# Kolkir/feature-point-cnn

Measured on AMD Instinct MI355X. Metric: frames/sec (VGA 640x480) SuperPoint fwd+NMS+descriptors, higher is better.
Workload: dtype f32

## Files before the change

### feature-point-cnn_amd/csrc/block_mfma.h

```cpp
#pragma once
#include "conv_mfma.h"

namespace fpc {

#ifdef FPC_DIAG
#define FPC_STAMP(i)                                                                     \
  if (a.stamps && threadIdx.x == 0) {                                                    \
    unsigned long long t_;                                                               \
    asm volatile("s_memtime %0\n\ts_waitcnt lgkmcnt(0)" : "=s"(t_)::"memory");            \
    a.stamps[(size_t)blockIdx.x * 8 + (i)] = t_;                                         \
  }
#define FPC_RSTAMP(i)                                                                    \
  if (a.stamps && threadIdx.x == 0) {                                                    \
    unsigned long long t_;                                                               \
    asm volatile("s_memrealtime %0\n\ts_waitcnt lgkmcnt(0)" : "=s"(t_)::"memory");        \
    a.stamps[(size_t)blockIdx.x * 8 + (i)] = t_;                                         \
  }
#else
#define FPC_STAMP(i)
#define FPC_RSTAMP(i)
#endif

struct BlockArgs {
  const float* x;
  int csx, nchunk;
  int H, W;
  const float4* w1;
  const float* b1;
  int tapoff4[9];
  const float4* w2;
  const float* b2;
  int k8_h, k8_x;
  float* out;
  int cso, Ho, Wo, tiles_x, tiles_y, nstore, frame0;
  unsigned x_bytes;
#ifdef FPC_DIAG
  unsigned long long* stamps;
#endif
};

template <int TH, int TW, int S, int KC, int WM, int WN, int MB, int NB, int CMIDP>
struct BlockCfg {
  using C1 = ConvCfg<TH, TW, S, 3, KC, WM, WN, MB, NB>;
  static constexpr int ROWH4 = CMIDP / 4 + 1;
  static constexpr int H_BYTES = C1::M * ROWH4 * 16;
  static constexpr int LDS_BYTES = C1::LDS_BYTES > H_BYTES ? C1::LDS_BYTES : H_BYTES;
  static_assert(CMIDP % 8 == 0 && CMIDP <= C1::N, "mid channels must fit the workgroup's N");
};

template <int TH, int TW, int S, int KC, int WM, int WN, int MB, int NB, int CMIDP>
__global__ __launch_bounds__(WM* WN * 64, 2) void block_mfma_kernel(const BlockArgs a) {
  using C = ConvCfg<TH, TW, S, 3, KC, WM, WN, MB, NB>;
  using BC = BlockCfg<TH, TW, S, KC, WM, WN, MB, NB, CMIDP>;
  constexpr int NT = C::NT, HW = C::HW, HH = C::HH, ROW4 = C::ROW4, K8 = KC / 8, KC4 = KC / 4;
  constexpr int NV = HH * HW * KC4, ITER = (NV + NT - 1) / NT, ROWH4 = BC::ROWH4, NBT = WN * NB;
  extern __shared__ float4 lds4[];

  const int tid = threadIdx.x, lane = tid & 63, wave = tid >> 6;
  const int wm = wave / WN, wn = wave % WN;
  const int half = lane >> 5, l31 = lane & 31;
  const int tiles = a.tiles_x * a.tiles_y;
  const int bidx = fpc_xcd_tile_index();
  const int bl = bidx / tiles;
  const int b = a.frame0 + bl;
  const int t = bidx - bl * tiles;
  const int ty = t / a.tiles_x, tx = t - ty * a.tiles_x;

  FPC_STAMP(0)
#ifdef FPC_DIAG
  if (a.stamps && threadIdx.x == 0) {
    a.stamps[(size_t)blockIdx.x * 8 + 6] = __builtin_amdgcn_s_getreg(63492);
    a.stamps[(size_t)blockIdx.x * 8 + 7] = __builtin_amdgcn_s_getreg((31 << 11) | 20);
  }
#endif
  int abase[MB];
#pragma unroll
  for (int mb = 0; mb < MB; ++mb) {
    int m = (wm * MB + mb) * 32 + l31;
    m = m < TH * TW ? m : TH * TW - 1;
    const int py = m / TW, px = m - py * TW;
    abase[mb] = ((py * S) * HW + px * S) * ROW4 + half;
  }
  constexpr int stepstride = NBT * 64;
  const __amdgpu_buffer_rsrc_t wrsrc = __builtin_amdgcn_make_buffer_rsrc(
      const_cast<float4*>(a.w1), 0, (int)((unsigned)(a.nchunk * 9 * K8 + 2) * (unsigned)(stepstride * 16)), 0x00020000);
  const int wlane = ((wn * NB) * 64 + lane) * 16;
  int wstep = 0;
  auto wfrag = [&](int nb) {
    typedef float f32x4w __attribute__((ext_vector_type(4)));
    const f32x4w r = __builtin_bit_cast(f32x4w, __builtin_amdgcn_raw_buffer_load_b128(wrsrc, wlane + nb * 1024, wstep, 0));
    return make_float4(r.x, r.y, r.z, r.w);
  };

  const int iy0 = ty * TH * S - 1, ix0 = tx * TW * S - 1;
  typedef float f32x4v __attribute__((ext_vector_type(4)));
  f32x4v stage[ITER];
  const __amdgpu_buffer_rsrc_t xrsrc = __builtin_amdgcn_make_buffer_rsrc(const_cast<float*>(a.x), 0, (int)a.x_bytes, 0x00020000);
  const unsigned xbase = (unsigned)((b * a.H + iy0) * a.W + ix0) * (unsigned)(a.csx * 4);
  auto load_chunk = [&](int chunk) {
    const int wlim = chunk < a.nchunk ? a.W : 0;
#pragma unroll
    for (int i = 0; i < ITER; ++i) {
      const int e = tid + i * NT;
      const int pix = e / KC4, c4 = e - pix * KC4;
      const int hy = pix / HW, hx = pix - hy * HW;
      const int iy = iy0 + hy, ix = ix0 + hx;
      const bool ok = ((unsigned)iy < (unsigned)a.H) & ((unsigned)ix < (unsigned)wlim) & (hy < HH);
      unsigned off = xbase + (unsigned)(((hy * a.W + hx) * a.csx + chunk * KC + c4 * 4) * 4);
      asm volatile("" : "+v"(off));
      stage[i] = __builtin_bit_cast(f32x4v, __builtin_amdgcn_raw_buffer_load_b128(xrsrc, (int)(ok ? off : 0xfffffff0u), 0, 0));
    }
  };
  auto store_chunk = [&]() {
#pragma unroll
    for (int i = 0; i < ITER; ++i) {
      const int e = tid + i * NT;
      int pix = e / KC4, c4 = e - pix * KC4;
      if (NV % NT != 0) {
        const bool in = e < NV;
        pix = in ? pix : HH * HW - 1;
        c4 = in ? c4 : KC4;
      }
      *reinterpret_cast<f32x4v*>(&lds4[pix * ROW4 + c4]) = stage[i];
    }
  };

  f32x16 acc[MB][NB];
#pragma unroll
  for (int mb = 0; mb < MB; ++mb)
#pragma unroll
    for (int nb = 0; nb < NB; ++nb)
#pragma unroll
      for (int r = 0; r < 16; ++r) acc[mb][nb][r] = 0.f;

  load_chunk(0);
  float4 b0[NB], b1[NB];
#pragma unroll
  for (int nb = 0; nb < NB; ++nb) b0[nb] = wfrag(nb);
  wstep += stepstride * 16;
#pragma unroll
  for (int nb = 0; nb < NB; ++nb) b1[nb] = wfrag(nb);
  wstep += stepstride * 16;
  for (int chunk = 0; chunk < a.nchunk; ++chunk) {
    FPC_LDS_BARRIER();
    store_chunk();
    FPC_LDS_BARRIER();
    load_chunk(chunk + 1);
    if (chunk == 0) { FPC_STAMP(1) }
    float4 av[MB];
#pragma unroll
    for (int mb = 0; mb < MB; ++mb) av[mb] = lds4[abase[mb] + a.tapoff4[0]];
#pragma unroll
    for (int tap = 0; tap < 9; ++tap) {
      const int toff = a.tapoff4[tap];
      const int toffn = a.tapoff4[tap < 8 ? tap + 1 : 8];
#pragma unroll
      for (int k8 = 0; k8 < K8; ++k8) {
        float4 b2[NB], an[MB];
#pragma unroll
        for (int nb = 0; nb < NB; ++nb) b2[nb] = wfrag(nb);
        wstep += stepstride * 16;
#pragma unroll
        for (int mb = 0; mb < MB; ++mb)
          an[mb] = lds4[abase[mb] + (k8 + 1 < K8 ? toff + (k8 + 1) * 2 : toffn)];
        __builtin_amdgcn_sched_barrier(0);
#pragma unroll
        for (int j = 0; j < 4; ++j)
#pragma unroll
          for (int mb = 0; mb < MB; ++mb)
#pragma unroll
            for (int nb = 0; nb < NB; ++nb) {
              const float af = j == 0 ? av[mb].x : j == 1 ? av[mb].y : j == 2 ? av[mb].z : av[mb].w;
              const float bf = j == 0 ? b0[nb].x : j == 1 ? b0[nb].y : j == 2 ? b0[nb].z : b0[nb].w;
              acc[mb][nb] = __builtin_amdgcn_mfma_f32_32x32x2f32(af, bf, acc[mb][nb], 0, 0, 0);
            }
#pragma unroll
        for (int nb = 0; nb < NB; ++nb) {
          b0[nb] = b1[nb];
          b1[nb] = b2[nb];
        }
#pragma unroll
        for (int mb = 0; mb < MB; ++mb) av[mb] = an[mb];
      }
    }
  }

  FPC_STAMP(2)
  constexpr int KH = CMIDP / 8, RING = 4;
  const int nsteps2 = KH + a.k8_x;
  const float4* wq = a.w2 + (size_t)(wn * NB) * 64 + lane;
  float4 cb[RING][NB];
  auto load_b = [&](int slot, int step) {
    const float4* pw = wq + (size_t)min(step, nsteps2 + 1) * stepstride;
#pragma unroll
    for (int nb = 0; nb < NB; ++nb) cb[slot][nb] = pw[nb * 64];
  };
#pragma unroll
  for (int s_ = 0; s_ < RING - 1; ++s_) load_b(s_, s_);
  FPC_LDS_BARRIER();
  {
    float* hl = reinterpret_cast<float*>(lds4);
#pragma unroll
    for (int nb = 0; nb < NB; ++nb) {
      const int n = (wn * NB + nb) * 32 + l31;
      const float bias = a.b1[n];
#pragma unroll
      for (int mb = 0; mb < MB; ++mb)
#pragma unroll
        for (int r = 0; r < 16; ++r) {
          const int m = (wm * MB + mb) * 32 + (r & 3) + 8 * (r >> 2) + 4 * half;
          const float v = acc[mb][nb][r] + bias;
          if (n < CMIDP) hl[m * (ROWH4 * 4) + n] = v > 0.f ? v : 0.f;
          acc[mb][nb][r] = 0.f;
        }
    }
  }
  FPC_LDS_BARRIER();

  FPC_STAMP(3)
  int hbase[MB];
#pragma unroll
  for (int mb = 0; mb < MB; ++mb) hbase[mb] = ((wm * MB + mb) * 32 + l31) * ROWH4 + half;
  auto mfma_step = [&](const float4 (&av)[MB], int slot) {
#pragma unroll
    for (int j = 0; j < 4; ++j)
#pragma unroll
      for (int mb = 0; mb < MB; ++mb)
#pragma unroll
        for (int nb = 0; nb < NB; ++nb) {
          const float af = j == 0 ? av[mb].x : j == 1 ? av[mb].y : j == 2 ? av[mb].z : av[mb].w;
          const float bf = j == 0 ? cb[slot][nb].x : j == 1 ? cb[slot][nb].y : j == 2 ? cb[slot][nb].z : cb[slot][nb].w;
          acc[mb][nb] = __builtin_amdgcn_mfma_f32_32x32x2f32(af, bf, acc[mb][nb], 0, 0, 0);
        }
  };
  const float* xrow[MB];
#pragma unroll
  for (int mb = 0; mb < MB; ++mb) {
    int m = (wm * MB + mb) * 32 + l31;
    m = m < TH * TW ? m : TH * TW - 1;
    const int py = m / TW, px = m - py * TW;
    int y = (ty * TH + py) * S, x = (tx * TW + px) * S;
    y = y < a.H ? y : a.H - 1;
    x = x < a.W ? x : a.W - 1;
    xrow[mb] = a.x + ((size_t)(b * a.H + y) * a.W + x) * a.csx + half * 4;
  }
  typedef float f4v __attribute__((ext_vector_type(4)));
  auto ldx = [&](int mb, int k8) {
    const f4v v = *reinterpret_cast<const f4v*>(xrow[mb] + (k8 < a.k8_x ? k8 : 0) * 8);
    return make_float4(v.x, v.y, v.z, v.w);
  };
  float4 xa[4][MB];
  if (a.k8_x > 0) {
#pragma unroll
    for (int u = 0; u < 4; ++u)
#pragma unroll
      for (int mb = 0; mb < MB; ++mb) xa[u][mb] = ldx(mb, u);
  }
  {
    float4 av[MB];
#pragma unroll
    for (int mb = 0; mb < MB; ++mb) av[mb] = lds4[hbase[mb]];
#pragma unroll
    for (int k8 = 0; k8 < KH; ++k8) {
      float4 an[MB];
      load_b((k8 + RING - 1) % RING, k8 + RING - 1);
#pragma unroll
      for (int mb = 0; mb < MB; ++mb) an[mb] = lds4[hbase[mb] + (k8 + 1 < KH ? k8 + 1 : k8) * 2];
      __builtin_amdgcn_sched_barrier(0);
      mfma_step(av, k8 % RING);
#pragma unroll
      for (int mb = 0; mb < MB; ++mb) av[mb] = an[mb];
    }
  }

  for (int k8 = 0; k8 < a.k8_x; k8 += 8) {
    float4 xb[4][MB];
#pragma unroll
    for (int u = 0; u < 4; ++u) {
      load_b((KH + u + RING - 1) % RING, KH + k8 + u + RING - 1);
#pragma unroll
      for (int mb = 0; mb < MB; ++mb) xb[u][mb] = ldx(mb, k8 + 4 + u);
      __builtin_amdgcn_sched_barrier(0);
      mfma_step(xa[u], (KH + u) % RING);
    }
#pragma unroll
    for (int u = 0; u < 4; ++u) {
      load_b((KH + u + RING - 1) % RING, KH + k8 + 4 + u + RING - 1);
#pragma unroll
      for (int mb = 0; mb < MB; ++mb) xa[u][mb] = ldx(mb, k8 + 8 + u);
      __builtin_amdgcn_sched_barrier(0);
      mfma_step(xb[u], (KH + u) % RING);
    }
  }

  FPC_STAMP(4)
  FPC_LDS_BARRIER();
  {
    float* ol = reinterpret_cast<float*>(lds4);
#pragma unroll
    for (int nb = 0; nb < NB; ++nb) {
      const int n = (wn * NB + nb) * 32 + l31;
      const float bias = a.b2[n];
#pragma unroll
      for (int mb = 0; mb < MB; ++mb)
#pragma unroll
        for (int r = 0; r < 16; ++r) {
          const int m = (wm * MB + mb) * 32 + (r & 3) + 8 * (r >> 2) + 4 * half;
          if (n < CMIDP) ol[m * (ROWH4 * 4) + n] = acc[mb][nb][r] + bias;
        }
    }
  }
  FPC_LDS_BARRIER();
  {
    constexpr int C4 = CMIDP / 4;
    constexpr int NE = TH * TW * C4, EIT = (NE + NT - 1) / NT;
    const int oyb = ty * TH, oxb = tx * TW;
    const bool ident = a.k8_x == 0;
    float4 idv[EIT];
    if (ident) {
#pragma unroll
      for (int i = 0; i < EIT; ++i) {
        const int e = tid + i * NT;
        const int m = e / C4, c4 = e - m * C4;
        const int py = m / TW, px = m - py * TW;
        const int y = oyb + py, x = oxb + px;
        const bool ok = (NE % NT == 0 || e < NE) && y < a.Ho && x < a.Wo;
        idv[i] = *reinterpret_cast<const float4*>(a.x + (ok ? ((size_t)(b * a.Ho + y) * a.Wo + x) * a.csx + c4 * 4 : 0));
      }
    }
#pragma unroll
    for (int i = 0; i < EIT; ++i) {
      const int e = tid + i * NT;
      const int m = e / C4, c4 = e - m * C4;
      const int py = m / TW, px = m - py * TW;
      const int y = oyb + py, x = oxb + px;
      if ((NE % NT == 0 || e < NE) && y < a.Ho && x < a.Wo) {
        float4 v = lds4[m * ROWH4 + c4];
        if (ident) {
          v.x += idv[i].x;
          v.y += idv[i].y;
          v.z += idv[i].z;
          v.w += idv[i].w;
        }
        v.x = v.x > 0.f ? v.x : 0.f;
        v.y = v.y > 0.f ? v.y : 0.f;
        v.z = v.z > 0.f ? v.z : 0.f;
        v.w = v.w > 0.f ? v.w : 0.f;
        *reinterpret_cast<float4*>(a.out + ((size_t)(b * a.Ho + y) * a.Wo + x) * a.cso + c4 * 4) = v;
      }
    }
  }
  FPC_STAMP(5)
}


}
```

### feature-point-cnn_amd/csrc/conv_mfma.h

```cpp
#pragma once
#include <hip/hip_runtime.h>
#include <stdint.h>

namespace fpc {

__device__ __forceinline__ int fpc_xcd_tile_index() {
  const unsigned g = gridDim.x, b = blockIdx.x;
  return (g & 7u) == 0u ? (int)((b & 7u) * (g >> 3) + (b >> 3)) : (int)b;
}

typedef float f32x16 __attribute__((ext_vector_type(16)));

#define FPC_LDS_BARRIER() asm volatile("s_waitcnt lgkmcnt(0)\n\ts_barrier" ::: "memory")

struct ConvSub {
  const float4* wfrag;
  int ntaps;
  int tapoff4[9];
  int oy0, ox0;
};

struct ConvArgs {
  const float* in0;
  int cs0;
  int nchunk0;
  const float* in1;
  int cs1, nchunk1, s1, H1, W1;
  int H, W;
  int pad;
  const float* bias;
  const float* res;
  int csr;
  float* out;
  int cso;
  int OH, OW, oys, oxs;
  int Ho, Wo;
  int tiles_x, tiles_y;
  int nstore;
  int relu;
  int nbt;
  int frame0;
  ConvSub sub[4];
};

template <int TH, int TW, int S, int EXT, int KC, int WM, int WN, int MB, int NB>
struct ConvCfg {
  static constexpr int NT = WM * WN * 64;
  static constexpr int HW = (TW - 1) * S + EXT;
  static constexpr int HH = (TH - 1) * S + EXT;
  static constexpr int ROW4 = KC / 4 + 1;
  static constexpr int LDS_BYTES = HH * HW * ROW4 * 16;
  static constexpr int M = WM * MB * 32;
  static constexpr int N = WN * NB * 32;
  static_assert(TH * TW <= M && TH * TW > M - 32, "tile must fill the M blocks");
  static_assert(KC % 8 == 0, "KC must be a multiple of 8");
};

template <int TH, int TW, int S, int EXT, int KC, int WM, int WN, int MB, int NB>
__global__ __launch_bounds__(WM* WN * 64, 2) void conv_mfma_kernel(const ConvArgs a) {
  using C = ConvCfg<TH, TW, S, EXT, KC, WM, WN, MB, NB>;
  constexpr int NT = C::NT, HW = C::HW, HH = C::HH, ROW4 = C::ROW4, K8 = KC / 8, KC4 = KC / 4;
  constexpr int NV = HH * HW * KC4;
  constexpr int ITER = (NV + NT - 1) / NT;
  extern __shared__ float4 lds4[];

  const int tid = threadIdx.x;
  const int lane = tid & 63, wave = tid >> 6;
  const int wm = wave / WN, wn = wave % WN;
  const int half = lane >> 5, l31 = lane & 31;

  const int tiles = a.tiles_x * a.tiles_y;
  const int bidx = fpc_xcd_tile_index();
  const int bl = bidx / tiles;
  const int b = a.frame0 + bl;
  const int t = bidx - bl * tiles;
  const int ty = t / a.tiles_x, tx = t - ty * a.tiles_x;
  const int subi = gridDim.z - 1 - blockIdx.z;
  const ConvSub& sp = a.sub[subi];

  int abase[MB];
#pragma unroll
  for (int mb = 0; mb < MB; ++mb) {
    int m = (wm * MB + mb) * 32 + l31;
    m = m < TH * TW ? m : TH * TW - 1;
    const int py = m / TW, px = m - py * TW;
    abase[mb] = ((py * S) * HW + px * S) * ROW4 + half;
  }
  const int stepstride = a.nbt * 64;
  const __amdgpu_buffer_rsrc_t wrsrc = __builtin_amdgcn_make_buffer_rsrc(
      const_cast<float4*>(sp.wfrag), 0, (int)((unsigned)((a.nchunk0 * sp.ntaps + a.nchunk1) * K8 + 2) * (unsigned)(stepstride * 16)), 0x00020000);
  const int wlane = (((blockIdx.y * WN + wn) * NB) * 64 + lane) * 16;
  int wstep = 0;
  const float4* wp = sp.wfrag + (size_t)((blockIdx.y * WN + wn) * NB) * 64 + lane;
  auto wfrag = [&](int nb) {
    if constexpr (EXT == 1) {
      return wp[(wstep >> 4) + nb * 64];
    } else {
      typedef float f32x4w __attribute__((ext_vector_type(4)));
      const f32x4w r = __builtin_bit_cast(f32x4w, __builtin_amdgcn_raw_buffer_load_b128(wrsrc, wlane + nb * 1024, wstep, 0));
      return make_float4(r.x, r.y, r.z, r.w);
    }
  };

  const int iy0 = ty * TH * S - a.pad, ix0 = tx * TW * S - a.pad;
  float4 stage[ITER];
  auto load_chunk = [&](int chunk) {
    const bool second = chunk >= a.nchunk0;
    const float* src = second ? a.in1 : a.in0;
    const int cs = second ? a.cs1 : a.cs0;
    const int c0 = (second ? chunk - a.nchunk0 : chunk) * KC;
    const int sH = second ? a.H1 : a.H, sW = second ? a.W1 : a.W;
#pragma unroll
    for (int i = 0; i < ITER; ++i) {
      const int e = tid + i * NT;
      const int pix = e / KC4, c4 = e - pix * KC4;
      const int hy = pix / HW, hx = pix - hy * HW;
      int iy, ix;
      if (second) {
        iy = (ty * TH + hy) * a.s1;
        ix = (tx * TW + hx) * a.s1;
      } else {
        iy = iy0 + hy;
        ix = ix0 + hx;
      }
      const bool ok = (NV % NT == 0 || e < NV) && iy >= 0 && iy < sH && ix >= 0 && ix < sW;
      const size_t off = ok ? ((size_t)(b * sH + iy) * sW + ix) * cs + c0 + c4 * 4 : 0;
      float4 v = *reinterpret_cast<const float4*>(src + off);
      if (!ok) v = make_float4(0.f, 0.f, 0.f, 0.f);
      stage[i] = v;
    }
  };
  auto store_chunk = [&]() {
#pragma unroll
    for (int i = 0; i < ITER; ++i) {
      const int e = tid + i * NT;
      const int pix = e / KC4, c4 = e - pix * KC4;
      if (NV % NT == 0 || e < NV) lds4[pix * ROW4 + c4] = stage[i];
    }
  };

  f32x16 acc[MB][NB];
#pragma unroll
  for (int mb = 0; mb < MB; ++mb)
#pragma unroll
    for (int nb = 0; nb < NB; ++nb)
#pragma unroll
      for (int r = 0; r < 16; ++r) acc[mb][nb][r] = 0.f;

  const int nchunks = a.nchunk0 + a.nchunk1;
  const int ntaps = sp.ntaps;
  load_chunk(0);
  float4 b0[NB], b1[NB];
#pragma unroll
  for (int nb = 0; nb < NB; ++nb) b0[nb] = wfrag(nb);
  wstep += stepstride * 16;
#pragma unroll
  for (int nb = 0; nb < NB; ++nb) b1[nb] = wfrag(nb);
  wstep += stepstride * 16;

  for (int chunk = 0; chunk < nchunks; ++chunk) {
    if (chunk) __syncthreads();
    store_chunk();
    __syncthreads();
    if (chunk + 1 < nchunks) load_chunk(chunk + 1);
    for (int tap = 0; tap < ntaps; ++tap) {
      const int toff = sp.tapoff4[tap];
#pragma unroll
      for (int k8 = 0; k8 < K8; ++k8) {
        float4 b2[NB];
#pragma unroll
        for (int nb = 0; nb < NB; ++nb) b2[nb] = wfrag(nb);
        wstep += stepstride * 16;
        __builtin_amdgcn_sched_barrier(0);
        float4 av[MB];
#pragma unroll
        for (int mb = 0; mb < MB; ++mb) av[mb] = lds4[abase[mb] + toff + k8 * 2];
#pragma unroll
        for (int j = 0; j < 4; ++j)
#pragma unroll
          for (int mb = 0; mb < MB; ++mb)
#pragma unroll
            for (int nb = 0; nb < NB; ++nb) {
              const float af = j == 0 ? av[mb].x : j == 1 ? av[mb].y : j == 2 ? av[mb].z : av[mb].w;
              const float bf = j == 0 ? b0[nb].x : j == 1 ? b0[nb].y : j == 2 ? b0[nb].z : b0[nb].w;
              acc[mb][nb] = __builtin_amdgcn_mfma_f32_32x32x2f32(af, bf, acc[mb][nb], 0, 0, 0);
            }
#pragma unroll
        for (int nb = 0; nb < NB; ++nb) {
          b0[nb] = b1[nb];
          b1[nb] = b2[nb];
        }
      }
    }
  }

  const int oyb = ty * TH, oxb = tx * TW;
#pragma unroll
  for (int nb = 0; nb < NB; ++nb) {
    const int n = ((blockIdx.y * WN + wn) * NB + nb) * 32 + l31;
    const float bias = a.bias[n];
    const bool nok = n < a.nstore;
#pragma unroll
    for (int mb = 0; mb < MB; ++mb) {
#pragma unroll
      for (int r = 0; r < 16; ++r) {
        const int m = (wm * MB + mb) * 32 + (r & 3) + 8 * (r >> 2) + 4 * half;
        const int py = m / TW, px = m - py * TW;
        const int y = oyb + py, x = oxb + px;
        if (nok && m < TH * TW && y < a.Ho && x < a.Wo) {
          const size_t opix = (size_t)(b * a.OH + y * a.oys + sp.oy0) * a.OW + x * a.oxs + sp.ox0;
          float v = acc[mb][nb][r] + bias;
          if (a.res) v += a.res[opix * a.csr + n];
          if (a.relu) v = v > 0.f ? v : 0.f;
          a.out[opix * a.cso + n] = v;
        }
      }
    }
  }
}

#define CONV2_MARKER 0x7fffff00

template <int TH, int TW, int S, int EXT, int KC, int WM, int WN, int MB, int NB>
struct Conv2Cfg {
  using C = ConvCfg<TH, TW, S, EXT, KC, WM, WN, MB, NB>;
  static constexpr int ROWO4 = C::N / 4 + 1;
  static constexpr int OUT_BYTES = C::M * ROWO4 * 16;
  static constexpr int LDS_BYTES = C::LDS_BYTES > OUT_BYTES ? C::LDS_BYTES : OUT_BYTES;
};

template <int TH, int TW, int S, int EXT, int KC, int WM, int WN, int MB, int NB>
__global__ __launch_bounds__(WM* WN * 64, 2) void conv2_mfma_kernel(const ConvArgs a) {
  using C = ConvCfg<TH, TW, S, EXT, KC, WM, WN, MB, NB>;
  using C2 = Conv2Cfg<TH, TW, S, EXT, KC, WM, WN, MB, NB>;
  constexpr int NT = C::NT, HW = C::HW, HH = C::HH, ROW4 = C::ROW4, K8 = KC / 8, KC4 = KC / 4, N = C::N;
  constexpr int NV = HH * HW * KC4, ITER = (NV + NT - 1) / NT, ROWO4 = C2::ROWO4;
  extern __shared__ float4 lds4[];
  typedef float f32x4w __attribute__((ext_vector_type(4)));

  const int tid = threadIdx.x, lane = tid & 63, wave = tid >> 6;
  const int wm = wave / WN, wn = wave % WN;
  const int half = lane >> 5, l31 = lane & 31;
  const int tiles = a.tiles_x * a.tiles_y;
  const int bidx = fpc_xcd_tile_index();
  const int bl = bidx / tiles;
  const int b = a.frame0 + bl;
  const int t = bidx - bl * tiles;
  const int ty = t / a.tiles_x, tx = t - ty * a.tiles_x;
  const int subi = gridDim.z - 1 - blockIdx.z;
  const ConvSub& sp = a.sub[subi];

  int abase[MB];
#pragma unroll
  for (int mb = 0; mb < MB; ++mb) {
    int m = (wm * MB + mb) * 32 + l31;
    m = m < TH * TW ? m : TH * TW - 1;
    const int py = m / TW, px = m - py * TW;
    abase[mb] = ((py * S) * HW + px * S) * ROW4 + half;
  }
  const int stepstride = a.nbt * 64;
  const __amdgpu_buffer_rsrc_t wrsrc = __builtin_amdgcn_make_buffer_rsrc(
      const_cast<float4*>(sp.wfrag), 0, (int)((unsigned)(a.nchunk0 * sp.ntaps * K8 + 2) * (unsigned)(stepstride * 16)), 0x00020000);
  const int wlane = (((blockIdx.y * WN + wn) * NB) * 64 + lane) * 16;
  int wstep = 0;
  auto wfrag = [&](int nb) {
    const f32x4w r = __builtin_bit_cast(f32x4w, __builtin_amdgcn_raw_buffer_load_b128(wrsrc, wlane + nb * 1024, wstep, 0));
    return make_float4(r.x, r.y, r.z, r.w);
  };

  const int iy0 = ty * TH * S - a.pad, ix0 = tx * TW * S - a.pad;
  const __amdgpu_buffer_rsrc_t xrsrc = __builtin_amdgcn_make_buffer_rsrc(
      const_cast<float*>(a.in0) + (size_t)b * a.H * a.W * a.cs0, 0, a.H * a.W * a.cs0 * 4, 0x00020000);
  int eoff[ITER], eslot[ITER];
#pragma unroll
  for (int i = 0; i < ITER; ++i) {
    const int e = tid + i * NT;
    int pix = e / KC4, c4 = e - pix * KC4;
    const int hy = pix / HW, hx = pix - hy * HW;
    const int iy = iy0 + hy, ix = ix0 + hx;
    const bool ok = (NV % NT == 0 || e < NV) & ((unsigned)iy < (unsigned)a.H) & ((unsigned)ix < (unsigned)a.W);
    eoff[i] = ok ? ((iy * a.W + ix) * a.cs0 + c4 * 4) * 4 : CONV2_MARKER;
    if (NV % NT != 0) {
      const bool in = e < NV;
      pix = in ? pix : HH * HW - 1;
      c4 = in ? c4 : KC4;
    }
    eslot[i] = pix * ROW4 + c4;
  }
  f32x4w stage[ITER];
  auto load_chunk = [&](int chunk) {
    const int cbase = chunk < a.nchunk0 ? chunk * (KC * 4) : CONV2_MARKER;
#pragma unroll
    for (int i = 0; i < ITER; ++i) {
      int voff;
      asm("v_add_i32 %0, %1, %2 clamp" : "=v"(voff) : "v"(eoff[i]), "s"(cbase));
      stage[i] = __builtin_bit_cast(f32x4w, __builtin_amdgcn_raw_buffer_load_b128(xrsrc, voff, 0, 0));
    }
  };
  auto store_chunk = [&]() {
#pragma unroll
    for (int i = 0; i < ITER; ++i) *reinterpret_cast<f32x4w*>(&lds4[eslot[i]]) = stage[i];
  };

  f32x16 acc[MB][NB];
#pragma unroll
  for (int mb = 0; mb < MB; ++mb)
#pragma unroll
    for (int nb = 0; nb < NB; ++nb)
#pragma unroll
      for (int r = 0; r < 16; ++r) acc[mb][nb][r] = 0.f;

  const int nchunks = a.nchunk0, ntaps = sp.ntaps;
  load_chunk(0);
  float4 b0[NB], b1[NB];
#pragma unroll
  for (int nb = 0; nb < NB; ++nb) b0[nb] = wfrag(nb);
  wstep += stepstride * 16;
#pragma unroll
  for (int nb = 0; nb < NB; ++nb) b1[nb] = wfrag(nb);
  wstep += stepstride * 16;

  for (int chunk = 0; chunk < nchunks; ++chunk) {
    FPC_LDS_BARRIER();
    store_chunk();
    FPC_LDS_BARRIER();
    load_chunk(chunk + 1);
    float4 av[MB];
#pragma unroll
    for (int mb = 0; mb < MB; ++mb) av[mb] = lds4[abase[mb] + sp.tapoff4[0]];
    for (int tap = 0; tap < ntaps; ++tap) {
      const int toff = sp.tapoff4[tap];
      const int toffn = sp.tapoff4[tap + 1 < ntaps ? tap + 1 : tap];
#pragma unroll
      for (int k8 = 0; k8 < K8; ++k8) {
        float4 b2[NB], an[MB];
#pragma unroll
        for (int nb = 0; nb < NB; ++nb) b2[nb] = wfrag(nb);
        wstep += stepstride * 16;
#pragma unroll
        for (int mb = 0; mb < MB; ++mb) an[mb] = lds4[abase[mb] + (k8 + 1 < K8 ? toff + (k8 + 1) * 2 : toffn)];
        __builtin_amdgcn_sched_barrier(0);
#pragma unroll
        for (int j = 0; j < 4; ++j)
#pragma unroll
          for (int mb = 0; mb < MB; ++mb)
#pragma unroll
            for (int nb = 0; nb < NB; ++nb) {
              const float af = j == 0 ? av[mb].x : j == 1 ? av[mb].y : j == 2 ? av[mb].z : av[mb].w;
              const float bf = j == 0 ? b0[nb].x : j == 1 ? b0[nb].y : j == 2 ? b0[nb].z : b0[nb].w;
              acc[mb][nb] = __builtin_amdgcn_mfma_f32_32x32x2f32(af, bf, acc[mb][nb], 0, 0, 0);
            }
#pragma unroll
        for (int nb = 0; nb < NB; ++nb) {
          b0[nb] = b1[nb];
          b1[nb] = b2[nb];
        }
#pragma unroll
        for (int mb = 0; mb < MB; ++mb) av[mb] = an[mb];
      }
    }
  }

  constexpr int C4 = N / 4, NE = TH * TW * C4, EIT = (NE + NT - 1) / NT;
  const int oyb = ty * TH, oxb = tx * TW;
  const int nbase = blockIdx.y * N;
  const __amdgpu_buffer_rsrc_t orsrc = __builtin_amdgcn_make_buffer_rsrc(a.out + (size_t)b * a.OH * a.OW * a.cso, 0, a.OH * a.OW * a.cso * 4, 0x00020000);
  const __amdgpu_buffer_rsrc_t rrsrc = __builtin_amdgcn_make_buffer_rsrc(
      const_cast<float*>(a.res ? a.res : a.out) + (size_t)b * a.OH * a.OW * (a.res ? a.csr : a.cso), 0, a.res ? a.OH * a.OW * a.csr * 4 : 0, 0x00020000);
  int ooff[EIT], olds[EIT];
  f32x4w idv[EIT];
#pragma unroll
  for (int i = 0; i < EIT; ++i) {
    const int e = tid + i * NT;
    const int m = e / C4, c4 = e - m * C4;
    const int py = m / TW, px = m - py * TW;
    const int y = oyb + py, x = oxb + px;
    const bool ok = (NE % NT == 0 || e < NE) & (y < a.Ho) & (x < a.Wo);
    const int opix = (y * a.oys + sp.oy0) * a.OW + x * a.oxs + sp.ox0;
    ooff[i] = ok ? (opix * a.cso + nbase + c4 * 4) * 4 : CONV2_MARKER;
    olds[i] = (NE % NT == 0 || e < NE) ? m * ROWO4 + c4 : 0;
    idv[i] = __builtin_bit_cast(f32x4w, __builtin_amdgcn_raw_buffer_load_b128(rrsrc, ok ? (opix * a.csr + nbase + c4 * 4) * 4 : CONV2_MARKER, 0, 0));
  }
  FPC_LDS_BARRIER();
  {
    float* ol = reinterpret_cast<float*>(lds4);
#pragma unroll
    for (int nb = 0; nb < NB; ++nb) {
      const int nl = (wn * NB + nb) * 32 + l31;
      const float bias = a.bias[nbase + nl];
#pragma unroll
      for (int mb = 0; mb < MB; ++mb)
#pragma unroll
        for (int r = 0; r < 16; ++r) {
          const int m = (wm * MB + mb) * 32 + (r & 3) + 8 * (r >> 2) + 4 * half;
          ol[m * (ROWO4 * 4) + nl] = acc[mb][nb][r] + bias;
        }
    }
  }
  FPC_LDS_BARRIER();
  const float floor_ = a.relu ? 0.f : -3.0e38f;
#pragma unroll
  for (int i = 0; i < EIT; ++i) {
    f32x4w v = *reinterpret_cast<const f32x4w*>(&lds4[olds[i]]);
    v += idv[i];
    v.x = fmaxf(v.x, floor_);
    v.y = fmaxf(v.y, floor_);
    v.z = fmaxf(v.z, floor_);
    v.w = fmaxf(v.w, floor_);
    __builtin_amdgcn_raw_buffer_store_b128(__builtin_bit_cast(__attribute__((ext_vector_type(4))) unsigned, v), orsrc, ooff[i], 0, 0);
  }
}

}
```

### feature-point-cnn_amd/csrc/fpc_api.hip

```cpp
#include <hip/hip_runtime.h>

#include <dlfcn.h>

#include <algorithm>
#include <cmath>
#include <cstdio>
#include <cstdlib>
#include <cstring>
#include <memory>
#include <mutex>
#include <chrono>
#include <string>
#include <vector>

#include "../../include/fpc.h"
#include "block_mfma.h"
#include "block_bf16.h"
#include "convt_bf16.h"
#include "block_x3.h"
#include "stem_bf16.h"
#include "wblock_mfma.h"
#include "wblock16_mfma.h"
#include "wblock36_mfma.h"
#include "wblock36p_mfma.h"
#include "conv_mfma.h"
#include "kernels_misc.h"
#include "queue_map.h"
#include "match.h"
#include "match_frames.h"
#include "match_bank.h"
#include "match_bank_bf16.h"
#include "match_guided.h"
#include "match_guided_cells.h"
#include "match_guided_epipolar.h"
#include "match_guided_pose.h"
#include "ransac_homography.h"
#include "ransac_fundamental.h"
#include "pose_epipolar.h"
#include "pose_homography.h"
#include "match_bank_topk.h"
#include "pnp_ransac.h"
#include "sim3_ransac.h"
#include "landmarks.h"
#include "homography.h"
#include "weights.h"
#include "plan_options.h"

namespace fpc {

constexpr int BLOB_HEADER_FLOATS = 16;
constexpr uint32_t BLOB_MAGIC = 0x57435046u;

static thread_local std::string g_hip_err;

#define HIPCHECK(expr)                                                                   \
  do {                                                                                   \
    hipError_t e_ = (expr);                                                              \
    if (e_ != hipSuccess) {                                                              \
      g_hip_err = std::string(#expr) + ": " + hipGetErrorString(e_);                     \
      return FPC_E_HIP;                                                                  \
    }                                                                                    \
  } while (0)

template <auto Kernel, int Threads, int Lds, typename Args>
static void launch_as(const Args& a, dim3 grid, hipStream_t st) {
  hipLaunchKernelGGL(Kernel, grid, dim3(Threads), Lds, st, a);
}

template <typename Args>
struct Instance {
  const void* fn;
  int lds_bytes, threads;
  void (*launch)(const Args&, dim3, hipStream_t);
};
template <auto Kernel, typename Cfg, int Threads, typename Args>
static Instance<Args> instance_of() {
  return {(const void*)Kernel, Cfg::LDS_BYTES, Threads, launch_as<Kernel, Threads, Cfg::LDS_BYTES, Args>};
}

#define FPC_KINDS(X)                                                        \
  X(T816_3x3_K64_N64, 8, 16, 1, 3, 64, 4, 1, 1, 2)                          \
  X(T816_1x1_K64_N64, 8, 16, 1, 1, 64, 4, 1, 1, 2)                          \
  X(T620_3x3s2_K32_N128, 6, 20, 2, 3, 32, 2, 2, 2, 2)                       \
  X(T620_3x3_K64_N128, 6, 20, 1, 3, 64, 2, 2, 2, 2)                         \
  X(T620_1x1_K64_N128, 6, 20, 1, 1, 64, 2, 2, 2, 2)                         \
  X(T620_2x2_K64_N128, 6, 20, 1, 2, 64, 2, 2, 2, 2)                         \
  X(T320_2x2_K64_N128, 3, 20, 1, 2, 64, 1, 4, 2, 1)                         \
  X(T320_1x1_K64_N128, 3, 20, 1, 1, 64, 1, 4, 2, 1)                         \
  X(T620_3x3_K64_N96, 6, 20, 1, 3, 64, 4, 1, 1, 3)                          \
  X(T620_1x1_K64_N96, 6, 20, 1, 1, 64, 4, 1, 1, 3)                          \
  X(T620_3x3_K72_N96, 6, 20, 1, 3, 72, 4, 1, 1, 3)                          \
  X(T620_1x1_K72_N96, 6, 20, 1, 1, 72, 4, 1, 1, 3)

enum Kind {
#define X(name, ...) K_##name,
  FPC_KINDS(X)
#undef X
      K_COUNT
};

struct KindInfo : Instance<ConvArgs> {
  const char* name;
  const char* symbol;
  int TH, TW, S, EXT, KC, WM, WN, MB, NB;
};

static const KindInfo g_kinds[K_COUNT] = {
#define X(name, TH, TW, S, EXT, KC, WM, WN, MB, NB)                                                                                      \
  {instance_of<conv_mfma_kernel<TH, TW, S, EXT, KC, WM, WN, MB, NB>, ConvCfg<TH, TW, S, EXT, KC, WM, WN, MB, NB>, WM * WN * 64, ConvArgs>(), \
   #name, "conv_mfma_kernel<" #TH ", " #TW ", " #S ", " #EXT ", " #KC ", " #WM ", " #WN ", " #MB ", " #NB ">", TH, TW, S, EXT, KC, WM, WN, MB, NB},
    FPC_KINDS(X)
#undef X
};

#define FPC_LEAN_KINDS(X)                          \
  X(T320_2x2_K64_N128, 3, 20, 1, 2, 64, 1, 4, 2, 1) \
  X(T320_1x1_K64_N128, 3, 20, 1, 1, 64, 1, 4, 2, 1)
struct LeanKindInfo : Instance<ConvArgs> {
  Kind kind;
  const char* symbol;
};
static const LeanKindInfo g_lean_kinds[] = {
#define X(name, TH, TW, S, EXT, KC, WM, WN, MB, NB)                                                                                        \
  {instance_of<conv2_mfma_kernel<TH, TW, S, EXT, KC, WM, WN, MB, NB>, Conv2Cfg<TH, TW, S, EXT, KC, WM, WN, MB, NB>, WM * WN * 64, ConvArgs>(), \
   K_##name, "conv2_mfma_kernel<" #TH ", " #TW ", " #S ", " #EXT ", " #KC ", " #WM ", " #WN ", " #MB ", " #NB ">"},
    FPC_LEAN_KINDS(X)
#undef X
};
static const LeanKindInfo* lean_kind(Kind k) {
  for (const LeanKindInfo& l : g_lean_kinds)
    if (l.kind == k) return &l;
  return nullptr;
}

#define FPC_BLOCK_KINDS(X)                                   \
  X(B816_s1_K64_C64, 8, 16, 1, 64, 4, 1, 1, 2, 64)           \
  X(B1616_s1_K32_C64, 16, 16, 1, 32, 4, 1, 2, 2, 64)         \
  X(B620_s2_K32_C128, 6, 20, 2, 32, 2, 2, 2, 2, 128)         \
  X(B620_s1_K64_C128, 6, 20, 1, 64, 2, 2, 2, 2, 128)         \
  X(B620_s1_K64_C72, 6, 20, 1, 64, 4, 1, 1, 3, 72)           \
  X(B620_s1_K72_C72, 6, 20, 1, 72, 4, 1, 1, 3, 72)           \
  X(B320_s2_K32_C256, 3, 20, 2, 32, 1, 4, 2, 2, 256)         \
  X(B310_s2_K32_C256, 3, 10, 2, 32, 1, 4, 1, 2, 256)         \
  X(B320_s2_K32_C128, 3, 20, 2, 32, 1, 4, 2, 1, 128)         \
  X(B320_s1_K64_C256, 3, 20, 1, 64, 1, 4, 2, 2, 256)         \
  X(B416_s2_K32_C128, 4, 16, 2, 32, 1, 4, 2, 1, 128)

enum BKind {
#define X(name, ...) BK_##name,
  FPC_BLOCK_KINDS(X)
#undef X
      BK_COUNT
};

struct BKindInfo : Instance<BlockArgs> {
  const char* name;
  const char* symbol;
  int TH, TW, S, KC, WM, WN, MB, NB, CMIDP;
};

static const BKindInfo g_bkinds[BK_COUNT] = {
#define X(name, TH, TW, S, KC, WM, WN, MB, NB, CMIDP)                                                                                            \
  {instance_of<block_mfma_kernel<TH, TW, S, KC, WM, WN, MB, NB, CMIDP>, BlockCfg<TH, TW, S, KC, WM, WN, MB, NB, CMIDP>, WM * WN * 64, BlockArgs>(), \
   #name, "block_mfma_kernel<" #TH ", " #TW ", " #S ", " #KC ", " #WM ", " #WN ", " #MB ", " #NB ", " #CMIDP ">", TH, TW, S, KC, WM, WN, MB, NB, CMIDP},
    FPC_BLOCK_KINDS(X)
#undef X
};

#define FPC_WBLOCK_KINDS(X)     \
  X(W816_K32_C64, 32, 2, 64)    \
  X(W816_K32_C128, 32, 4, 128)  \
  X(W816_K32_C72, 32, 3, 72)    \
  X(W816_K24_C72, 24, 3, 72)
#define FPC_W16_KINDS(X) \
  X(W16_C64, 4, 8)       \
  X(W16_C128, 8, 8)      \
  X(W16_C128H, 8, 4)
#define FPC_W36_KINDS(X) \
  X(W36_C64_4x4, 1, 4, 4)  \
  X(W36_C64_2x8, 1, 2, 8)  \
  X(W36_C128_4x4, 2, 4, 4) \
  X(W36_C128_2x8, 2, 2, 8)

#define FPC_W36P_KINDS(X) \
  X(W36P_C64_4x4, 4, 4)   \
  X(W36P_C64_2x8, 2, 8)

#define FPC_W36PD_KINDS(X) \
  X(W36PD_C65_4x4, 4, 4)   \
  X(W36PD_C65_2x8, 2, 8)

#define FPC_W36D_KINDS(X) \
  X(W36_C65_4x4, 4, 4)    \
  X(W36_C65_2x8, 2, 8)

#define FPC_W36S_KINDS(X) \
  X(W36S_C128_4x4, 2, 4, 4)
#define FPC_W36PC_KINDS(X) \
  X(W36PC_C64_8x2, 8, 2)

enum WKind {
#define X(name, ...) WK_##name,
  FPC_WBLOCK_KINDS(X)
  FPC_W16_KINDS(X)
  FPC_W36_KINDS(X)
  FPC_W36D_KINDS(X)
  FPC_W36P_KINDS(X)
  FPC_W36PD_KINDS(X)
  FPC_W36S_KINDS(X)
  FPC_W36PC_KINDS(X)
#undef X
      WK_COUNT
};

struct WKindInfo : Instance<WBlockArgs> {
  const char* name;
  const char* symbol;
  int gen;
  int KC, NBT, CMID;
  int NCG;
  int TH;
  int TW;
  bool dust = false;
};

static const WKindInfo g_wkinds[WK_COUNT] = {
#define X(name, KC, NBT, CMID)                                                                            \
  {instance_of<wblock_mfma_kernel<KC, NBT, CMID>, WBlockCfg<KC, NBT, CMID>, 512, WBlockArgs>(), #name,                         \
   "wblock_mfma_kernel<" #KC ", " #NBT ", " #CMID ">", 1, KC, NBT, CMID, 0, 8, 16},
    FPC_WBLOCK_KINDS(X)
#undef X
#define X(name, NCG, TH)                                                                                  \
  {instance_of<wblock16_kernel<NCG, TH>, W16Cfg<NCG, TH>, 512, WBlockArgs>(), #name,                                           \
   "wblock16_kernel<" #NCG ", " #TH ">", 2, 16, NCG / 2, NCG * 16, NCG, TH, 16},
    FPC_W16_KINDS(X)
#undef X
#define X(name, NB, TYT, TXT)                                                                             \
  {instance_of<wblock36_kernel<NB, TYT, TXT>, W36Cfg<NB, TYT, TXT>, 256, WBlockArgs>(), #name,                                 \
   "wblock36_kernel<" #NB ", " #TYT ", " #TXT ">", 3, 16, 2 * NB, 64 * NB, 4 * NB, 4 * TYT, 4 * TXT},
    FPC_W36_KINDS(X)
#undef X
#define X(name, TYT, TXT)                                                                                 \
  {instance_of<wblock36_dust_kernel<TYT, TXT>, W36Cfg<1, TYT, TXT, true>, 256, WBlockArgs>(), #name,                           \
   "wblock36_dust_kernel<" #TYT ", " #TXT ">", 3, 16, 2, 64, 4, 4 * TYT, 4 * TXT, true},
    FPC_W36D_KINDS(X)
#undef X
#define X(name, TYT, TXT)                                                                                 \
  {instance_of<wblock36p_kernel<TYT, TXT>, W36PCfg<TYT, TXT>, 512, WBlockArgs>(), #name,                                       \
   "wblock36p_kernel<" #TYT ", " #TXT ", 3>", 3, 16, 2, 64, 4, 4 * TYT, 4 * TXT},
    FPC_W36P_KINDS(X)
#undef X
#define X(name, TYT, TXT)                                                                                 \
  {instance_of<wblock36p_dust_kernel<TYT, TXT>, W36PCfg<TYT, TXT, true>, 512, WBlockArgs>(), #name,                            \
   "wblock36p_dust_kernel<" #TYT ", " #TXT ", 3>", 3, 16, 2, 64, 4, 4 * TYT, 4 * TXT, true},
    FPC_W36PD_KINDS(X)
#undef X
#define X(name, NB, TYT, TXT)                                                                             \
  {instance_of<wblock36s_kernel<NB, TYT, TXT>, W36Cfg<NB, TYT, TXT>, 256, WBlockArgs>(), #name,                                \
   "wblock36s_kernel<" #NB ", " #TYT ", " #TXT ">", 3, 16, 2 * NB, 64 * NB, 4 * NB, 4 * TYT, 4 * TXT},
    FPC_W36S_KINDS(X)
#undef X
#define X(name, TYT, TXT)                                                                                 \
  {instance_of<wconv36p_kernel<TYT, TXT>, W36PCfg<TYT, TXT, false, true>, 512, WBlockArgs>(), #name,                           \
   "wconv36p_kernel<" #TYT ", " #TXT ", 3>", 3, 16, 2, 64, 4, 4 * TYT, 4 * TXT},
    FPC_W36PC_KINDS(X)
#undef X
};

static size_t conv_floats(size_t steps, int nbt) { return (steps + 2) * nbt * 64 * 4; }
static size_t conv_bf16_floats(size_t steps, int nbt, int planes) { return (steps + 2) * planes * nbt * 64 * 4; }
static size_t bias_floats(int nbt) { return (size_t)nbt * 32; }
static size_t w1_floats(const WKindInfo& k, int nchunk) {
  if (k.gen == 3) return (size_t)k.NCG * ((size_t)nchunk * 36 + (k.NCG == 8 ? W36Cfg<2, 4, 4>::WPAD : W36Cfg<1, 4, 4>::WPAD)) * 256;
  if (k.gen == 2) return (size_t)k.NCG * ((size_t)nchunk * 16 + W16Cfg<8>::WPAD) * 256;
  return conv_floats(((size_t)nchunk + 1) * 16 * (k.KC / 8), k.NBT);
}
static size_t w2_floats(const WKindInfo& k, int k8) {
  if (k.gen >= 2) return (size_t)k.NCG * ((size_t)k8 / 2 + W16Cfg<8>::WPAD) * 256;
  return conv_floats(k8, k.NBT);
}
static double wkind_mfma_flops(const WKindInfo& k, int tiles, int nchunk, int k8_1x1) {
  const double px = (double)k.TH * k.TW, n = k.NBT * 32.0;
  if (k.gen == 3) return 2.0 * tiles * n * (36.0 * (px / 16) * nchunk * k.KC + px * k8_1x1 * 8.0);
  return 2.0 * tiles * n * (16.0 * (px / 4) * nchunk * k.KC + px * k8_1x1 * 8.0);
}
static bool w36_fits(int , int H, int W, int cs_in, int cs_out) {
  return (unsigned long long)H * W * (unsigned long long)std::max(cs_in, cs_out) * sizeof(float) < (unsigned long long)W36_MARKER;
}
static int w36_frames_per_launch(int H, int W, int cs_in, int cs_out) {
  const unsigned long long fb = (unsigned long long)H * W * (unsigned long long)std::max(cs_in, cs_out) * sizeof(float);
  return (int)std::max<unsigned long long>(1, ((unsigned long long)W36_MARKER - 1) / fb);
}
static const unsigned long long W16_REACH = 0xfffffff0ull;
static int w16_frames_in_reach(int H, int W, int cs) {
  return (int)std::min<unsigned long long>(1u << 30, W16_REACH / ((unsigned long long)H * W * cs * sizeof(float)));
}
static int w36_conv_part(int cout, int tiles, int cus) {
  if (cout < 128) return 64;
  if (cout == 128) return 128;
  const double t2 = std::ceil((double)tiles * (cout / 128) / cus) * 1.0, t1 = std::ceil((double)tiles * (cout / 64) / cus) * 0.53;
  return t1 < t2 ? 64 : 128;
}
static WKind w36_kind(int cout, int H, int W, bool paired = false, bool conv82 = false) {
  const int t44 = ((H + 15) / 16) * ((W + 15) / 16), t28 = ((H + 7) / 8) * ((W + 31) / 32), t82 = ((H + 31) / 32) * ((W + 7) / 8);
  if (conv82 && cout == 64 && paired && t82 < std::min(t44, t28)) return WK_W36PC_C64_8x2;
  if (cout == 65 && paired) return t28 < t44 ? WK_W36PD_C65_2x8 : WK_W36PD_C65_4x4;
  if (cout == 65) return t28 < t44 ? WK_W36_C65_2x8 : WK_W36_C65_4x4;
  if (cout == 64 && paired) return t28 < t44 ? WK_W36P_C64_2x8 : WK_W36P_C64_4x4;
  if (cout == 64) return t28 < t44 ? WK_W36_C64_2x8 : WK_W36_C64_4x4;
  return t28 < t44 ? WK_W36_C128_2x8 : WK_W36_C128_4x4;
}

static WKind w36_stacked_kind(WKind wk) { return wk == WK_W36_C128_4x4 || wk == WK_W36_C128_2x8 ? WK_W36S_C128_4x4 : WK_COUNT; }
static int w36_stacked_rows(int Hf, int W, int frames, WKind sk, int tiles_now) {
  if (sk == WK_COUNT) return 0;
  const int th = g_wkinds[sk].TH, tw = g_wkinds[sk].TW;
  if (Hf % 4 != 0 || Hf < th) return 0;
  const int rows = (frames * Hf + th - 1) / th;
  return rows * ((W + tw - 1) / tw) < frames * tiles_now ? rows : 0;
}

#define FPC_BF16_KINDS(X)                                                                   \
  X(F816_s1_K64_C64, block_bf16_one_kernel, BlockBfCfg, 1, 8, 32, 1, 3, 64, 2, 2, 4, 1, 64) \
  X(F816_s1_K64_C128, block_bf16_kernel, BlockBfCfg, 1, 8, 16, 1, 3, 64, 1, 4, 4, 1, 128)   \
  X(F816_s1_K80_C80, block_bf16_one_kernel, BlockBfCfg, 1, 8, 16, 1, 3, 80, 4, 1, 1, 3, 80) \
  X(F816_s1_K128_C128, block_bf16_one_kernel, BlockBfCfg, 1, 8, 16, 1, 3, 128, 1, 4, 4, 1, 128) \
  X(F816_s1_K128_C80w, block_bf16_one_kernel, BlockBfCfg, 1, 8, 16, 1, 3, 128, 1, 4, 4, 1, 80) \
  X(F620_s2_K64_C128, block_bf16_one_kernel, BlockBfCfg, 1, 6, 20, 2, 3, 64, 2, 2, 2, 2, 128) \
  X(F320_s2_K128_C256, block_bf16_one_kernel, BlockBfCfg, 1, 3, 20, 2, 3, 128, 1, 4, 2, 2, 256) \
  X(F416_s1_K128_C256, block_bf16_two_kernel, BlockBfCfg, 1, 4, 16, 1, 3, 128, 1, 4, 2, 2, 256) \
  X(F816_ct_K64_C128, block_bf16_kernel, BlockBfCfg, 1, 8, 16, 1, 2, 64, 1, 4, 4, 1, 128)   \
  X(F816_ctf_K64_C128, convt_bf16_kernel, ConvTBfCfg, 1, 8, 16, 1, 2, 64, 2, 2, 2, 1, 128)  \
  X(S816_s1_K64_C64, block_x3_kernel, BlockX3Cfg, 3, 8, 16, 1, 3, 64, 2, 2, 2, 1, 64)       \
  X(S620_s2_K16_C128, block_x3_kernel, BlockX3Cfg, 3, 6, 20, 2, 3, 16, 2, 2, 2, 2, 128)     \
  X(S620_s1_K64_C128, block_x3_kernel, BlockX3Cfg, 3, 6, 20, 1, 3, 64, 2, 2, 2, 2, 128)     \
  X(S620_s1_K64_C80, block_x3_kernel, BlockX3Cfg, 3, 6, 20, 1, 3, 64, 4, 1, 1, 3, 80)       \
  X(S620_s1_K16_C80, block_x3_kernel, BlockX3Cfg, 3, 6, 20, 1, 3, 16, 4, 1, 1, 3, 80)       \
  X(S320_s2_K16_C256, block_x3_kernel, BlockX3Cfg, 3, 3, 20, 2, 3, 16, 1, 4, 2, 2, 256)     \
  X(S320_s1_K64_C256, block_x3_kernel, BlockX3Cfg, 3, 3, 20, 1, 3, 64, 1, 4, 2, 2, 256)     \
  X(S620_ct_K64_C128, block_x3_kernel, BlockX3Cfg, 3, 6, 20, 1, 2, 64, 2, 2, 2, 2, 128)     \
  X(S620_1x1_K64_C80, block_x3_kernel, BlockX3Cfg, 3, 6, 20, 1, 1, 64, 4, 1, 1, 3, 80)      \
  X(S320_1x1_K64_C256, block_x3_kernel, BlockX3Cfg, 3, 3, 20, 1, 1, 64, 1, 4, 2, 2, 256)     \
  X(H816_s1_K64_C64, block_h2_kernel, BlockH2Cfg, 2, 8, 16, 1, 3, 64, 2, 2, 2, 1, 64)     \
  X(H620_s2_K16_C128, block_h2_kernel, BlockH2Cfg, 2, 6, 20, 2, 3, 16, 2, 2, 2, 2, 128)     \
  X(H620_s1_K64_C128, block_h2_kernel, BlockH2Cfg, 2, 6, 20, 1, 3, 64, 2, 2, 2, 2, 128)     \
  X(H620_s1_K64_C80, block_h2_kernel, BlockH2Cfg, 2, 6, 20, 1, 3, 64, 4, 1, 1, 3, 80)     \
  X(H620_s1_K16_C80, block_h2_kernel, BlockH2Cfg, 2, 6, 20, 1, 3, 16, 4, 1, 1, 3, 80)     \
  X(H320_s2_K16_C256, block_h2_kernel, BlockH2Cfg, 2, 3, 20, 2, 3, 16, 1, 4, 2, 2, 256)     \
  X(H320_s1_K64_C256, block_h2_kernel, BlockH2Cfg, 2, 3, 20, 1, 3, 64, 1, 4, 2, 2, 256)     \
  X(H620_ct_K64_C128, block_h2_kernel, BlockH2Cfg, 2, 6, 20, 1, 2, 64, 2, 2, 2, 2, 128)     \
  X(H620_1x1_K64_C80, block_h2_kernel, BlockH2Cfg, 2, 6, 20, 1, 1, 64, 4, 1, 1, 3, 80)     \
  X(H320_1x1_K64_C256, block_h2_kernel, BlockH2Cfg, 2, 3, 20, 1, 1, 64, 1, 4, 2, 2, 256)

enum FKind {
#define X(name, ...) FK_##name,
  FPC_BF16_KINDS(X)
#undef X
      FK_COUNT
};

struct FKindInfo : Instance<BlockBfArgs> {
  const char* name;
  const char* symbol;
  int planes, TH, TW, S, EXT, KC, WM, WN, MB, NB, CMIDP;
};

static const FKindInfo g_fkinds[FK_COUNT] = {
#define X(name, KERN, CFG, PL, TH, TW, S, EXT, KC, WM, WN, MB, NB, CMIDP)                                                                  \
  {instance_of<KERN<TH, TW, S, EXT, KC, WM, WN, MB, NB, CMIDP>, CFG<TH, TW, S, EXT, KC, WM, WN, MB, NB, CMIDP>, WM * WN * 64, BlockBfArgs>(), \
   #name, #KERN "<" #TH ", " #TW ", " #S ", " #EXT ", " #KC ", " #WM ", " #WN ", " #MB ", " #NB ", " #CMIDP ">",                             \
   PL, TH, TW, S, EXT, KC, WM, WN, MB, NB, CMIDP},
    FPC_BF16_KINDS(X)
#undef X
};

template <typename Info, size_t N>
static int allow_dynamic_lds(const Info (&table)[N]) {
  for (const Info& k : table) HIPCHECK(hipFuncSetAttribute(k.fn, hipFuncAttributeMaxDynamicSharedMemorySize, k.lds_bytes));
  return FPC_OK;
}
#ifdef FPC_DIAG
template <typename Info, size_t N>
static void print_occupancy(const Info (&table)[N]) {
  for (const Info& k : table) {
    int nb = -1;
    hipOccupancyMaxActiveBlocksPerMultiprocessor(&nb, k.fn, k.threads, k.lds_bytes);
    hipFuncAttributes fa{};
    hipFuncGetAttributes(&fa, k.fn);
    fprintf(stderr, "[diag] %s: lds %d B, regs %d, scratch %zu, static lds %zu, occupancy %d blocks/CU\n", k.name, k.lds_bytes,
            fa.numRegs, fa.localSizeBytes, fa.sharedSizeBytes, nb);
  }
}
#endif

enum OpType { OP_STEM, OP_POOL, OP_CONV, OP_BLOCK, OP_WBLOCK, OP_BF16, OP_SOFTMAX, OP_NMS, OP_DESC,
              OP_VCONV0, OP_POOL2, OP_L2NORM };

struct Op {
  OpType type;
  std::string name;
  Kind kind = K_COUNT;
  ConvArgs args{};
  BKind bkind = BK_COUNT;
  BlockArgs bargs{};
  WKind wkind = WK_COUNT;
  int hash_bkind = -1, hash_wkind = -1;
  WBlockArgs wargs{};
  FKind fkind = FK_COUNT;
  BlockBfArgs fargs{};
  int phase = -1;
  int when = 0;
  bool shadow = false;
  bool wconv = false;
  int n0 = 0;
  bool plain_conv = false;
  bool lean = false;
  int ksize = 0;
  const float* pin = nullptr;
  float* pout = nullptr;
  int pH = 0, pW = 0, pC = 0;
  std::string prefix;
  int cin = 0, cout = 0;
  int grid_y = 1, grid_z = 1;
  double flops_per_frame = 0;
  double mfma_flops_per_frame = 0;
  bool fused_softmax_capable = false;
  double bytes_per_frame = 0;
  bool descriptor_branch = false;
};

struct Region {
  size_t off = 0, len = 0;
};

struct Timing {
  hipEvent_t start, stop;
  int op;
  int frames;
  int wkind = -1;
  double mfma_flops = -1.0;
};

using GuardZones = std::vector<std::pair<size_t, size_t>>;
struct Carver;
struct Slab {
  char* base = nullptr;
  size_t bytes = 0;
  GuardZones zones;
  explicit operator bool() const { return base != nullptr; }
  int allocate(hipStream_t st, Carver& cv);
  hipError_t release() {
    const hipError_t e = base ? hipFree(base) : hipSuccess;
    *this = Slab{};
    return e;
  }
};

}

using namespace fpc;

struct fpc_ctx {
  fpc_config cfg{};
  int H = 0, W = 0, B = 0, Hc = 0, Wc = 0;
  bool vgg = false;
  int D = 128;
  struct VTap { const char* name; const float* p; int cs, C, H, W; };
  std::vector<VTap> vtaps;
  size_t vconv0_off = 0;
  bool bf16 = false;
  bool split = false;
  bool split_f16 = false;
  int lgcs = 72;
  int cin = 3;
  int cap = 0, sort_cap = 0;
  PlanOptions opt;
  hipStream_t stream = nullptr;
  bool own_stream = false;
  hipStream_t upload = nullptr;
  bool queue_probe = true;
  int probe_rounds = 0;
  double placement_ms = 0.0;
  std::vector<std::pair<hipStream_t, int>> caller_stream_memo;
  std::vector<hipStream_t> aux;
  std::vector<hipEvent_t> ev_join;
  std::vector<hipStream_t> side;
  std::vector<hipEvent_t> ev_enc, ev_det;
  hipEvent_t ev_fork = nullptr;
  int small_reach = 1 << 30;
  int num_cus = 256;
  int fkind_blocks_per_cu[64] = {};
  bool logits_valid = false;
#ifdef FPC_DIAG
  unsigned long long* diag_stamps = nullptr;
  int diag_n = 0;
#endif
  bool weights_loaded = false;
  bool plan_error = false;

  Slab slab, bank_slab, topk_slab, pnp_slab, lm_slab;
  Slab* const slabs[5] = {&slab, &bank_slab, &topk_slab, &pnp_slab, &lm_slab};
  float *stem_out, *x0, *h4, *x1, *x2, *h8, *x3, *cat, *dh, *dproj, *d0, *lg;
  float *h16, *y16a, *y16b, *lo_h, *lo0, *desc_map, *desc_in_nhwc;
  float* prob;
  uint32_t *nmsmap, *cand;
  int32_t *ncand, *count, *xy, *status;
  float* rowmax = nullptr;
  uint32_t* range = nullptr;
  float *conf, *desc_out;
  unsigned long long* sort_scratch;
  int32_t* nms_aux = nullptr;
  unsigned long long *rowbest, *colbest;
  float* mf_norms = nullptr;
  unsigned long long *mf_top2 = nullptr, *mf_colbest = nullptr;
  float4* hf_pairs = nullptr;
  int32_t *hf_row = nullptr, *hf_np = nullptr;
  unsigned long long* hf_best = nullptr;
  int32_t *mgc_perm_q = nullptr, *mgc_perm_t = nullptr;
  int4* mgc_box = nullptr;
  BankArgs bank{};
  int bank_format = FPC_BANK_F32;
  BankBf16Args bank16{};
  BankTopkArgs topk{};
  float4* topk_pairs = nullptr;
  int32_t *topk_row = nullptr, *topk_np = nullptr;
  unsigned long long* topk_best = nullptr;
  float4* pnp_rec = nullptr;
  int32_t* pnp_np = nullptr;
  unsigned long long* pnp_best = nullptr;
  float4* lm_xyzw = nullptr;
  int pts_n = 0;
  bool pts_desc = false;

  float* u8stage = nullptr;
  char* ha_ws = nullptr;

  float* blob = nullptr;
  size_t blob_floats = 0;
  uint32_t* bcast_tag = nullptr;
  std::vector<float> host_blob;

  std::vector<Op> ops;
  StemArgs stem{};
  size_t stem_w_off = 0, stem_b_off = 0;
  struct ConvW {
    Region w[4], b, b2;
  };
  std::vector<ConvW> convw;

  bool timing = false;
  int timing_every = 0, timing_calls = 0;
  std::vector<Timing> timings;
  std::vector<hipEvent_t> event_pool;
  size_t events_used = 0;
};

namespace fpc {

static size_t align_up(size_t v, size_t a) { return (v + a - 1) / a * a; }

constexpr size_t GUARD_BYTES = 64 << 10;
constexpr size_t GUARD_TAIL = (size_t)0x80000000u + (4u << 20);
constexpr uint32_t GUARD_PATTERN = 0xA5C3F00Du;

struct Carver {
  size_t off = 0;
  size_t guard = 0;
  GuardZones zones;
  explicit Carver(const fpc_ctx* c) : guard(c->opt.guard_zones ? GUARD_BYTES : 0) {}
  template <typename T>
  size_t take(size_t n) {
    const size_t o = off;
    off = align_up(off + n * sizeof(T), 256);
    if (guard) {
      zones.push_back({off, guard});
      off += guard;
    }
    return o;
  }
  struct Bound { void* slot; size_t off; };
  std::vector<Bound> bound;
  template <typename T>
  void into(T** slot, size_t n) { bound.push_back({slot, take<T>(n)}); }
  void bind(char* slab) const {
    for (const Bound& b : bound) {
      char* p = slab + b.off;
      memcpy(b.slot, &p, sizeof p);
    }
  }
  void finish() {
    if (guard) {
      zones.push_back({off, GUARD_TAIL});
      off += GUARD_TAIL;
// ... 27 lines not shown
static int fill_guards(fpc_ctx* c) {
  HIPCHECK(hipDeviceSynchronize());
  fill_zones(c->stream, c->slab.base, c->slab.zones);
  if (!c->slab.zones.empty()) HIPCHECK(hipStreamSynchronize(c->stream));
  return FPC_OK;
}

int Slab::allocate(hipStream_t st, Carver& cv) {
  char* p = nullptr;
  HIPCHECK(hipMalloc((void**)&p, cv.off));
  hipError_t e = hipMemset(p, 0, cv.off);
  if (e == hipSuccess) e = hipDeviceSynchronize();
  fill_zones(st, p, cv.zones);
  if (e == hipSuccess) e = hipStreamSynchronize(st);
  if (e != hipSuccess) hipFree(p);
  HIPCHECK(e);
  base = p;
  bytes = cv.off;
  zones = std::move(cv.zones);
  cv.bind(p);
  return FPC_OK;
}


static int carve_results(fpc_ctx* c, Carver& cv) {
  const size_t B = c->B, HW = (size_t)c->H * c->W, cap = c->cap;
  const bool whole = c->vgg || c->cfg.descriptor_enabled != 0;
  cv.into(&c->prob, B * HW);
  cv.into(&c->nmsmap, B * HW); cv.into(&c->cand, B * HW);
  cv.into(&c->ncand, B); cv.into(&c->count, B);
  cv.into(&c->status, 4 + BLOB_HEADER_FLOATS);
  cv.into(&c->range, B * FPC_RANGE_WORDS);
  cv.into(&c->rowmax, B * (c->H / 8));
  cv.into(&c->xy, B * cap * 2); cv.into(&c->conf, B * cap);
  cv.into(&c->desc_out, whole ? B * cap * c->D : 64);
  cv.into(&c->sort_scratch, B * c->sort_cap);
  cv.into(&c->nms_aux, B * NMS_AUX_INTS);
  cv.into(&c->rowbest, cap); cv.into(&c->colbest, cap);
  cv.into(&c->mf_norms, whole ? (B + 1) * cap : 64);
  cv.into(&c->mf_top2, whole ? B * cap * 2 : 64);
  cv.into(&c->mf_colbest, whole ? B * cap : 64);
  cv.into(&c->hf_pairs, B * cap); cv.into(&c->hf_row, B * cap);
  cv.into(&c->hf_np, B); cv.into(&c->hf_best, B);
  cv.into(&c->mgc_perm_q, whole ? B * cap : 64); cv.into(&c->mgc_perm_t, whole ? B * cap : 64);
  cv.into(&c->mgc_box, whole ? 2 * B * ((cap + 63) / 64) : 64);
  cv.finish();
  c->slab.bytes = cv.off;
  c->slab.zones = cv.zones;
  if (hipMalloc((void**)&c->slab.base, c->slab.bytes) != hipSuccess) {
    g_hip_err = "hipMalloc(workspace " + std::to_string(c->slab.bytes >> 20) + " MiB) failed";
    return FPC_E_HIP;
  }
  HIPCHECK(hipMemset(c->slab.base, 0, c->slab.bytes));
  if (int grc = fill_guards(c)) return grc;
  cv.bind(c->slab.base);
  c->bcast_tag = reinterpret_cast<uint32_t*>(c->status + 4);
  return FPC_OK;
}

static Op& push_op(fpc_ctx* c, OpType type, const std::string& name) {
  Op op;
  op.type = type;
  op.name = name;
  c->ops.push_back(op);
  c->convw.push_back({});
  return c->ops.back();
}

static int finish_plan(fpc_ctx* c, size_t blob_floats) {
  push_op(c, OP_NMS, "nms+sort+border_crop");
  if (c->cfg.descriptor_enabled) push_op(c, OP_DESC, "descriptor_sample+l2norm");
  for (Op& op : c->ops)
    if (op.type == OP_SOFTMAX) op.bytes_per_frame = 4.0 * (65.0 * c->Hc * c->Wc + 2.0 * c->H * c->W);
  c->blob_floats = blob_floats;
  HIPCHECK(hipMalloc((void**)&c->blob, c->blob_floats * sizeof(float)));
  HIPCHECK(hipMemset(c->blob, 0, c->blob_floats * sizeof(float)));
  for (size_t i = 0; i < c->ops.size(); ++i) {
    Op& op = c->ops[i];
    const fpc_ctx::ConvW& cw = c->convw[i];
    const float *w1 = c->blob + cw.w[0].off, *w2 = c->blob + cw.w[1].off, *b1 = c->blob + cw.b.off, *b2 = c->blob + cw.b2.off;
    switch (op.type) {
      case OP_WBLOCK:
        op.wargs.w1 = reinterpret_cast<const float4*>(w1); op.wargs.b1 = b1;
        op.wargs.w2 = reinterpret_cast<const float4*>(w2); op.wargs.b2 = b2;
        op.wargs.dust = g_wkinds[op.wkind].dust ? c->blob + cw.w[2].off : nullptr;
        break;
      case OP_BF16:
        op.fargs.w1 = reinterpret_cast<const uint4*>(w1); op.fargs.b1 = b1;
        op.fargs.w2 = reinterpret_cast<const uint4*>(w2); op.fargs.b2 = b2;
        break;
      case OP_BLOCK:
        op.bargs.w1 = reinterpret_cast<const float4*>(w1); op.bargs.b1 = b1;
        op.bargs.w2 = reinterpret_cast<const float4*>(w2); op.bargs.b2 = b2;
        break;
      case OP_CONV:
        for (int z = 0; z < op.grid_z; ++z)
          op.args.sub[z].wfrag = reinterpret_cast<const float4*>(c->blob + cw.w[z].off);
        op.args.bias = b1;
        break;
      default:
        break;
    }
  }
  return FPC_OK;
}

static void reserve(size_t* blob_off, Region& r, size_t n) {
  r = {*blob_off, n};
  *blob_off += n;
}
static Op weight_op(OpType type, const std::string& name, const std::string& prefix, int cin, int cout, bool desc_branch) {
  Op op;
  op.type = type; op.name = name; op.prefix = prefix;
  op.cin = cin; op.cout = cout; op.descriptor_branch = desc_branch;
  return op;
}
static void push_op(fpc_ctx* c, const Op& op, const fpc_ctx::ConvW& cw) {
  c->ops.push_back(op);
  c->convw.push_back(cw);
}
static void mark_when(fpc_ctx* c, size_t i0, int when) {
  for (size_t k = i0; k < c->ops.size(); ++k) c->ops[k].when = when;
}
static unsigned x_bytes(const fpc_ctx* c, int H, int W, int csx, int elem) {
  return (unsigned)std::min<size_t>((size_t)c->B * H * W * csx * elem, 0xffffff00u);
}

struct ConvTTap { int dy, dx, ky, kx; };
static std::vector<ConvTTap> convt_phase_taps(int ph) {
  const int py = ph >> 1, px = ph & 1;
  std::vector<ConvTTap> taps;
  for (int iy = 0; iy < (py ? 2 : 1); ++iy)
    for (int ix = 0; ix < (px ? 2 : 1); ++ix)
      taps.push_back({py ? 1 - iy : 0, px ? 1 - ix : 0, py ? (iy == 0 ? 0 : 2) : 1, px ? (ix == 0 ? 0 : 2) : 1});
  return taps;
}

struct ConvSpec {
  std::string name;
  Kind kind;
  int ksize;
  const float* in0;
  int cs0, cin0, cin0_pad, H0, W0;
  const float* in1 = nullptr;
  int cs1 = 0, cin1 = 0, cin1_pad = 0, s1 = 1, H1 = 0, W1 = 0;
  const float* res = nullptr;
  int csr = 0;
  float* out;
  int cso, cout, nstore, Ho, Wo;
  int relu;
  bool desc_branch;
};

static bool conv_is_lean(const fpc_ctx* c, const Op& op) {
  const KindInfo& k = g_kinds[op.kind];
  const ConvArgs& a = op.args;
  return c->opt.conv_lean && lean_kind(op.kind) && a.nchunk1 == 0 && a.nstore == op.grid_y * (k.WN * k.NB * 32) && a.cso % 4 == 0 &&
         (!a.res || a.csr % 4 == 0);
}

static void add_conv(fpc_ctx* c, const ConvSpec& s, size_t* blob_off) {
  const KindInfo& k = g_kinds[s.kind];
  Op op;
  op.type = OP_CONV;
  op.name = s.name;
  op.kind = s.kind;
  op.descriptor_branch = s.desc_branch;
  ConvArgs& a = op.args;
  const int N = k.WN * k.NB * 32;
  const int nbt = (s.cout + N - 1) / N * (N / 32);
  op.grid_y = nbt * 32 / N;
  a.in0 = s.in0; a.cs0 = s.cs0; a.nchunk0 = s.cin0_pad / k.KC; a.H = s.H0; a.W = s.W0;
  a.in1 = s.in1; a.cs1 = s.cs1; a.nchunk1 = s.in1 ? s.cin1_pad / k.KC : 0; a.s1 = s.s1; a.H1 = s.H1; a.W1 = s.W1;
  a.pad = s.ksize == 3 ? 1 : 0;
  a.res = s.res; a.csr = s.csr;
  a.out = s.out; a.cso = s.cso; a.nstore = s.nstore; a.relu = s.relu; a.nbt = nbt;
  const int HWp = (k.TW - 1) * k.S + k.EXT, ROW4 = k.KC / 4 + 1;
  fpc_ctx::ConvW cw;
  const int K8 = k.KC / 8;
  if (s.ksize == 2) {
    op.grid_z = 4;
    a.Ho = s.H0;
    a.Wo = s.W0;
    a.OH = s.Ho;
    a.OW = s.Wo;
    a.oys = a.oxs = 2;
    double macs = 0;
    for (int ph = 0; ph < 4; ++ph) {
      ConvSub& sp = a.sub[ph];
      sp.oy0 = ph >> 1;
      sp.ox0 = ph & 1;
      sp.ntaps = 0;
      for (const ConvTTap& t : convt_phase_taps(ph)) sp.tapoff4[sp.ntaps++] = (t.dy * HWp + t.dx) * ROW4;
      reserve(blob_off, cw.w[ph], conv_floats((size_t)a.nchunk0 * sp.ntaps * K8, nbt));
      macs += (double)sp.ntaps;
    }
    op.flops_per_frame = 2.0 * macs * s.H0 * s.W0 * s.cin0 * s.cout;
    op.mfma_flops_per_frame = 2.0 * macs * ((s.H0 + k.TH - 1) / k.TH) * ((s.W0 + k.TW - 1) / k.TW) * (k.WM * k.MB * 32.0) * (a.nchunk0 * k.KC) * (nbt * 32.0);
  } else {
    a.Ho = a.OH = s.Ho;
    a.Wo = a.OW = s.Wo;
    a.oys = a.oxs = 1;
    ConvSub& sp = a.sub[0];
    sp.oy0 = sp.ox0 = 0;
    sp.ntaps = s.ksize * s.ksize;
    for (int ky = 0; ky < s.ksize; ++ky)
      for (int kx = 0; kx < s.ksize; ++kx) sp.tapoff4[ky * s.ksize + kx] = (ky * HWp + kx) * ROW4;
    reserve(blob_off, cw.w[0], conv_floats((size_t)(a.nchunk0 * sp.ntaps + a.nchunk1) * K8, nbt));
    op.flops_per_frame = 2.0 * s.Ho * s.Wo * s.cout * ((double)s.cin0 * sp.ntaps + s.cin1);
    op.mfma_flops_per_frame = 2.0 * ((s.Ho + k.TH - 1) / k.TH) * ((s.Wo + k.TW - 1) / k.TW) * (k.WM * k.MB * 32.0) * (nbt * 32.0) *
                              ((double)a.nchunk0 * k.KC * sp.ntaps + (double)a.nchunk1 * k.KC);
  }
  reserve(blob_off, cw.b, bias_floats(nbt));
  op.lean = conv_is_lean(c, op);
  a.tiles_x = (a.Wo + k.TW - 1) / k.TW;
  a.tiles_y = (a.Ho + k.TH - 1) / k.TH;
  op.bytes_per_frame = 4.0 * ((double)s.cin0 * s.H0 * s.W0 + (s.in1 ? (double)s.cin1 * s.H1 * s.W1 : 0.0) +
                              (s.res ? (double)s.cout * s.Ho * s.Wo : 0.0) + (double)s.cout * s.Ho * s.Wo);
  push_op(c, op, cw);
}

struct BlockSpec {
  std::string prefix;
  BKind kind;
  const float* x;
  int csx, cin, cin_pad, H, W;
  float* out;
  int cso, cout, cout_pad;
  bool proj, desc_branch;
};

static void tile_block(Op& o, BKind kind) {
  const BKindInfo& k = g_bkinds[kind];
  o.bkind = kind;
  BlockArgs& a = o.bargs;
  const int HWp = (k.TW - 1) * k.S + 3, ROW4 = k.KC / 4 + 1;
  for (int ky = 0; ky < 3; ++ky)
    for (int kx = 0; kx < 3; ++kx) a.tapoff4[ky * 3 + kx] = (ky * HWp + kx) * ROW4;
  a.tiles_x = (a.Wo + k.TW - 1) / k.TW;
  a.tiles_y = (a.Ho + k.TH - 1) / k.TH;
  o.mfma_flops_per_frame = 2.0 * a.tiles_x * a.tiles_y * (k.WM * k.MB * 32.0) * (k.WN * k.NB * 32.0) *
                           ((double)a.nchunk * k.KC * 9 + (a.k8_h + a.k8_x) * 8.0);
}

static void add_block(fpc_ctx* c, const BlockSpec& s, size_t* blob_off) {
  const BKindInfo& k = g_bkinds[s.kind];
  Op op = weight_op(OP_BLOCK, s.prefix + (s.proj ? " [conv1+bn1+relu+conv2+bn2+proj+relu]" : " [conv1+bn1+relu+conv2+bn2+identity+relu]"),
                    s.prefix, s.cin, s.cout, s.desc_branch);
  BlockArgs& a = op.bargs;
  const int nbt = k.WN * k.NB, K8 = k.KC / 8;
  a.x = s.x;
  a.csx = s.csx;
  a.x_bytes = x_bytes(c, s.H, s.W, s.csx, 4);
  a.nchunk = s.cin_pad / k.KC;
  a.H = s.H;
  a.W = s.W;
  a.k8_h = k.CMIDP / 8;
  a.k8_x = s.proj ? s.cin_pad / 8 : 0;
  if (a.k8_x % 8) { fprintf(stderr, "fpc: fused block %s: projection over %d channels is not a multiple of 64\n", s.prefix.c_str(), s.cin_pad); abort(); }
  a.out = s.out;
  a.cso = s.cso;
  a.Ho = s.H / k.S;
  a.Wo = s.W / k.S;
  a.nstore = s.cout_pad;
  tile_block(op, s.kind);
  fpc_ctx::ConvW cw;
  reserve(blob_off, cw.w[0], conv_floats((size_t)a.nchunk * 9 * K8, nbt));
  reserve(blob_off, cw.b, bias_floats(nbt));
  reserve(blob_off, cw.w[1], conv_floats(a.k8_h + a.k8_x, nbt));
  reserve(blob_off, cw.b2, bias_floats(nbt));
  op.flops_per_frame = 2.0 * a.Ho * a.Wo * s.cout * ((double)s.cin * 9 + s.cout + (s.proj ? s.cin : 0));
  op.bytes_per_frame = 4.0 * ((double)s.cin * s.H * s.W + (double)s.cout * a.Ho * a.Wo);
  push_op(c, op, cw);
}

static void retile_block(fpc_ctx* c, BKind small) {
  const BKindInfo &k0 = g_bkinds[c->ops.back().bkind], &k = g_bkinds[small];
  if (k.KC != k0.KC || k.WN * k.NB != k0.WN * k0.NB || k.S != k0.S || k.CMIDP != k0.CMIDP) { c->plan_error = true; return; }
  tile_block(c->ops.back(), small);
}
static void retile_last(fpc_ctx* c, BKind small) {
  if (!c->opt.latency_tiles || c->ops.empty() || c->ops.back().type != OP_BLOCK) return;
  retile_block(c, small);
}
static long block_rows(BKind k, int Ho, int Wo) {
  const BKindInfo& b = g_bkinds[k];
  return (long)((Ho + b.TH - 1) / b.TH) * ((Wo + b.TW - 1) / b.TW) * (b.WM * b.MB * 32);
}
static void retile_rows(fpc_ctx* c, BKind fit) {
  if (!c->opt.tiles_round6 || c->ops.empty() || c->ops.back().type != OP_BLOCK) return;
  Op& o = c->ops.back();
  if (block_rows(fit, o.bargs.Ho, o.bargs.Wo) >= block_rows(o.bkind, o.bargs.Ho, o.bargs.Wo)) return;
  const BKind had = o.bkind;
  retile_block(c, fit);
  if (!c->plan_error) c->ops.back().hash_bkind = had;
}

static void retile_last(fpc_ctx* c, Kind small) {
  if (!c->opt.latency_tiles || c->ops.empty() || c->ops.back().type != OP_CONV) return;
  const KindInfo &k0 = g_kinds[c->ops.back().kind], &k = g_kinds[small];
  if (k.KC != k0.KC || k.WN * k.NB != k0.WN * k0.NB || k.S != k0.S || k.EXT != k0.EXT) { c->plan_error = true; return; }
  Op& o = c->ops.back();
  o.kind = small;
  ConvArgs& a = o.args;
  const int HWp = (k.TW - 1) * k.S + k.EXT, HWp0 = (k0.TW - 1) * k0.S + k0.EXT, ROW4 = k.KC / 4 + 1;
  for (int z = 0; z < o.grid_z; ++z)
    for (int t = 0; t < a.sub[z].ntaps; ++t) {
      const int lin = a.sub[z].tapoff4[t] / ROW4, dy = lin / HWp0, dx = lin - dy * HWp0;
      a.sub[z].tapoff4[t] = (dy * HWp + dx) * ROW4;
    }
  a.tiles_x = (a.Wo + k.TW - 1) / k.TW;
  a.tiles_y = (a.Ho + k.TH - 1) / k.TH;
// ... 1020 lines not shown
  if (int rc = pk.put(op, pack_conv_bf16({s1}, co, nbt, k.KC, k.planes, &pk.range_bad), cw.w[0])) return rc;
  if (int rc = pk.fill(op, cw.b, co, [&](int n) { return b.f1.t[n]; })) return rc;
  if (int rc = pk.put(op, pack_conv_bf16(block_1x1_sources(b, ci, co, a.k16_h * 16, sc_in_w1 ? 0 : a.k16_x * 16), co, nbt, 16, k.planes, &pk.range_bad),
                      cw.w[1]))
    return rc;
  return pk.fill(op, cw.b2, co, [&](int n) { return b.bias[n]; });
}

static int pack_block(const Packer& pk, const Op& op, const fpc_ctx::ConvW& cw) {
  const BKindInfo& k = g_bkinds[op.bkind];
  const BlockArgs& a = op.bargs;
  const int ci = op.cin, co = op.cout, nbt = k.WN * k.NB;
  BlockWeights b;
  if (!load_block(pk, op.prefix, ci, co, a.k8_x > 0, &b)) return FPC_E_MISSING_KEY;
  PackSource s1{ci, a.nchunk * k.KC, 9, [&](int n, int c_, int t) { return (double)b.w1[((size_t)(n * ci + c_)) * 9 + t]; }, &b.f1.s};
  if (int rc = pk.put(op, pack_conv({s1}, co, nbt, k.KC), cw.w[0])) return rc;
  if (int rc = pk.fill(op, cw.b, co, [&](int n) { return b.f1.t[n]; })) return rc;
  if (int rc = pk.put(op, pack_conv(block_1x1_sources(b, ci, co, a.k8_h * 8, a.k8_x * 8), co, nbt, 8), cw.w[1])) return rc;
  return pk.fill(op, cw.b2, co, [&](int n) { return b.bias[n]; });
}

static int pack_conv_op(const Packer& pk, const Op& op, const fpc_ctx::ConvW& cw) {
  const TensorMap& m = pk.m;
  std::string* missing = pk.missing;
  const KindInfo& k = g_kinds[op.kind];
  const ConvArgs& a = op.args;
  const std::string& nm = op.name;
  const size_t dot = nm.find(".conv1+");
  const size_t dot2 = nm.find(".conv2+");
  const int cin0p = a.nchunk0 * k.KC, cin1p = a.nchunk1 * k.KC;
  Fold f, fp;
  std::vector<double> bias(a.nbt * 32, 0.0);
  if (nm == "descriptor.up_sample+bn+relu") {
    const float* w = pk.need("descriptor.up_sample.weight", {256, 128, 3, 3});
    const float* bct = pk.need("descriptor.up_sample.bias", {128});
    if (!w || !bct || !fold_bn(m, "descriptor.bn", 128, &f, missing)) return FPC_E_MISSING_KEY;
    for (int ph = 0; ph < 4; ++ph) {
      const std::vector<ConvTTap> taps = convt_phase_taps(ph);
      PackSource s{256, cin0p, (int)taps.size(),
                   [&](int n, int ci, int t) { return (double)w[((ci * 128 + n) * 3 + taps[t].ky) * 3 + taps[t].kx]; },
                   &f.s};
      if (int rc = pk.put(op, pack_conv({s}, 128, a.nbt, k.KC), cw.w[ph])) return rc;
    }
    for (int n = 0; n < 128; ++n) bias[n] = (double)bct[n] * f.s[n] + f.t[n];
  } else if (nm == "detector.layer.0.identity_downsample") {
    const float* w = pk.need("detector.layer.0.identity_downsample.0.weight", {65, 128, 1, 1});
    if (!w || !fold_bn(m, "detector.layer.0.identity_downsample.1", 65, &f, missing)) return FPC_E_MISSING_KEY;
    PackSource s{128, cin0p, 1, [&](int n, int ci, int) { return (double)w[n * 128 + ci]; }, &f.s};
    if (int rc = pk.put(op, pack_conv({s}, 65, a.nbt, k.KC), cw.w[0])) return rc;
    for (int n = 0; n < 65; ++n) bias[n] = f.t[n];
  } else if (dot != std::string::npos) {
    const std::string p = nm.substr(0, dot);
    auto it = m.find(p + ".conv1.weight");
    if (it == m.end() || it->second.shape.size() != 4 || it->second.shape[2] != 3) {
      if (missing->empty()) *missing = p + ".conv1.weight";
      return FPC_E_MISSING_KEY;
    }
    const int co = (int)it->second.shape[0], ci = (int)it->second.shape[1];
    const float* w = it->second.data;
    if (ci > cin0p || co > a.nbt * 32 || !w) {
      *missing = p + ".conv1.weight";
      return FPC_E_MISSING_KEY;
    }
    if (!fold_bn(m, p + ".bn1", co, &f, missing)) return FPC_E_MISSING_KEY;
    PackSource s{ci, cin0p, 9, [&](int n, int c_, int t) { return (double)w[((size_t)(n * ci + c_)) * 9 + t]; }, &f.s};
    if (int rc = pk.put(op, pack_conv({s}, co, a.nbt, k.KC), cw.w[0])) return rc;
    for (int n = 0; n < co; ++n) bias[n] = f.t[n];
  } else if (dot2 != std::string::npos) {
    const std::string p = nm.substr(0, dot2);
    auto it = m.find(p + ".conv2.weight");
    if (it == m.end() || it->second.shape.size() != 4 || !it->second.data) {
      if (missing->empty()) *missing = p + ".conv2.weight";
      return FPC_E_MISSING_KEY;
    }
    const int co = (int)it->second.shape[0];
    const float* w = it->second.data;
    if ((int)it->second.shape[1] != co || co > cin0p || co > a.nbt * 32) {
      *missing = p + ".conv2.weight";
      return FPC_E_MISSING_KEY;
    }
    if (!fold_bn(m, p + ".bn2", co, &f, missing)) return FPC_E_MISSING_KEY;
    std::vector<PackSource> srcs;
    srcs.push_back({co, cin0p, 1, [&, co](int n, int c_, int) { return (double)w[(size_t)n * co + c_]; }, &f.s});
    for (int n = 0; n < co; ++n) bias[n] = f.t[n];
    const float* wp = nullptr;
    int cip = 0;
    if (a.in1) {
      auto ip = m.find(p + ".identity_downsample.0.weight");
      if (ip == m.end() || ip->second.shape.size() != 4 || (int)ip->second.shape[0] != co || !ip->second.data ||
          (int)ip->second.shape[1] > cin1p) {
        if (missing->empty()) *missing = p + ".identity_downsample.0.weight";
        return FPC_E_MISSING_KEY;
      }
      wp = ip->second.data;
      cip = (int)ip->second.shape[1];
      if (!fold_bn(m, p + ".identity_downsample.1", co, &fp, missing)) return FPC_E_MISSING_KEY;
      srcs.push_back({cip, cin1p, 1, [&, cip](int n, int c_, int) { return (double)wp[(size_t)n * cip + c_]; }, &fp.s});
      for (int n = 0; n < co; ++n) bias[n] += fp.t[n];
    }
    if (int rc = pk.put(op, pack_conv(srcs, co, a.nbt, k.KC), cw.w[0])) return rc;
  } else {
    *missing = "internal: unknown op " + nm;
    return FPC_E_INVALID;
  }
  return pk.fill(op, cw.b, a.nbt * 32, [&](int n) { return bias[n]; });
}

static int pack_all_impl(fpc_ctx* c, const TensorMap& m, std::string* missing, bool& range_bad) {
  c->host_blob.assign(c->blob_floats, 0.f);
  const Packer pk{c, m, missing, range_bad};
  if (int rc = c->vgg ? pack_vgg_convs(pk) : pack_stem(pk)) return rc;
  for (size_t i = 0; i < c->ops.size(); ++i) {
    const Op& op = c->ops[i];
    if (c->vgg && op.type != OP_WBLOCK) continue;
    int rc = FPC_OK;
    switch (op.type) {
      case OP_WBLOCK: rc = pack_wblock(pk, op, c->convw[i]); break;
      case OP_BF16: rc = pack_fblock(pk, op, c->convw[i]); break;
      case OP_BLOCK: rc = pack_block(pk, op, c->convw[i]); break;
      case OP_CONV: rc = pack_conv_op(pk, op, c->convw[i]); break;
      default: break;
    }
    if (rc != FPC_OK) return rc;
  }
  return FPC_OK;
}

static hipEvent_t next_event(fpc_ctx* c) {
  if (c->events_used == c->event_pool.size()) {
    hipEvent_t e;
    hipEventCreate(&e);
    c->event_pool.push_back(e);
  }
  return c->event_pool[c->events_used++];
}

struct Sub {
  int f0, n;
  bool small = false;
  bool fuse_softmax = false;
  hipStream_t st;
  hipStream_t side = nullptr;
  hipEvent_t ev_enc = nullptr, ev_det = nullptr;
};

struct LaunchTimer {
  fpc_ctx* c;
  int op;
  hipStream_t st;
  int frames;
  hipEvent_t s{}, e{};
  int wkind = -1;
  double mfma_flops = -1.0;
  LaunchTimer(fpc_ctx* c_, int op_, hipStream_t st_, int frames_) : c(c_), op(op_), st(st_), frames(frames_) {
    if (c->timing) {
      s = next_event(c);
      e = next_event(c);
      hipEventRecord(s, st);
    }
  }
  ~LaunchTimer() {
    if (c->timing) {
      hipEventRecord(e, st);
      c->timings.push_back({s, e, op, frames, wkind, mfma_flops});
    }
  }
};

static int op_index(const fpc_ctx* c, OpType t) {
  for (size_t i = 0; i < c->ops.size(); ++i)
    if (c->ops[i].type == t) return (int)i;
  return -1;
}

template <typename Args>
static void diag_stamp(fpc_ctx* c, const Op& op, Args& a, int tiles) {
#ifdef FPC_DIAG
  a.stamps = nullptr;
  if (const char* e = getenv("FPC_STAMP_OP"))
    if (op.name.find(e) != std::string::npos) {
      if (!c->diag_stamps) hipHostMalloc((void**)&c->diag_stamps, (size_t)65536 * 8 * sizeof(unsigned long long));
      memset(c->diag_stamps, 0, (size_t)65536 * 8 * sizeof(unsigned long long));
      a.stamps = c->diag_stamps;
      c->diag_n = tiles;
    }
#endif
}

enum StemKind { STEM_PLAIN, STEM_POOL, STEM_POOL2, STEM_X3, STEM_X3_F16, STEM_BF16 };
static StemKind stem_kind(const fpc_ctx* c) {
  if (!(c->opt.fuse_stem_pool || c->cin == 1 || c->bf16)) return STEM_PLAIN;
  if (c->split_f16) return STEM_X3_F16;
  if (c->bf16) return STEM_BF16;
  if (c->split) return STEM_X3;
  return c->opt.stem2 ? STEM_POOL2 : STEM_POOL;
}

static const char* launch_stem(fpc_ctx* c, const Op& op, int i, const float* frames, const Sub* sb) {
  static const char* const symbol[] = {"stem_kernel", "stem_pool_kernel", "stem_pool2_kernel", "stem_pool_x3_kernel",
                                       "stem_pool_x3_kernel", "stem_bf16_kernel"};
  const StemKind kind = stem_kind(c);
  if (!sb) return symbol[kind];
  const int H = c->H, W = c->W, n = sb->n, f0 = sb->f0;
  const bool gray = c->cin == 1;
  if (kind == STEM_PLAIN) {
    LaunchTimer t(c, i, sb->st, n);
    StemArgs a = c->stem;
    a.in = frames + (size_t)f0 * 3 * H * W;
    a.out = c->stem_out + (size_t)f0 * (H / 2) * (W / 2) * 64;
    hipLaunchKernelGGL(stem_kernel, dim3(a.tiles_x * a.tiles_y * n), dim3(256), 0, sb->st, a);
    return symbol[kind];
  }
  float* x0 = c->bf16 ? reinterpret_cast<float*>(reinterpret_cast<unsigned short*>(c->x0) + (size_t)f0 * (H / 4) * (W / 4) * 64)
                      : c->x0 + (size_t)f0 * (H / 4) * (W / 4) * 64;
  if (!c->bf16) stem_border_clear_kernel<<<(n * (H / 4) + 7) / 8, 256, 0, sb->st>>>(reinterpret_cast<float4*>(x0), H / 4, W / 4, n * (H / 4));
  LaunchTimer t(c, i, sb->st, n);
  StemPoolArgs a{};
  a.in = frames + (size_t)f0 * c->cin * H * W;
  a.wfrag = c->stem.wfrag;
  a.bias = c->stem.bias;
  a.out = x0;
  a.H = H; a.W = W; a.Ho = H / 2; a.Wo = W / 2; a.Hp = H / 4; a.Wp = W / 4;
  a.tiles_x = c->stem.tiles_x; a.tiles_y = c->stem.tiles_y;
  a.range = c->range + (size_t)f0 * FPC_RANGE_WORDS;
  const dim3 grid(a.tiles_x * a.tiles_y * n);
  if (kind == STEM_X3 || kind == STEM_X3_F16 || kind == STEM_BF16) {
    StemX3Args x{};
    x.in = a.in; x.wfrag = reinterpret_cast<const uint4*>(a.wfrag); x.bias = a.bias; x.out = a.out;
    x.H = H; x.W = W; x.Ho = a.Ho; x.Wo = a.Wo; x.Hp = a.Hp; x.Wp = a.Wp; x.tiles_x = a.tiles_x; x.tiles_y = a.tiles_y;
    x.range_flag = c->split_f16 ? c->status + 1 : nullptr;
    diag_stamp(c, op, x, a.tiles_x * a.tiles_y * n);
    if (kind == STEM_X3_F16) {
      if (gray) hipLaunchKernelGGL((stem_pool_x3_kernel<1, 2>), grid, dim3(256), 0, sb->st, x);
      else hipLaunchKernelGGL((stem_pool_x3_kernel<3, 2>), grid, dim3(256), 0, sb->st, x);
    } else if (kind == STEM_BF16) {
      x.frames = n;
      x.tiles_x = (x.Wp + SB2_PW - 1) / SB2_PW;
      x.tiles_y = (x.Hp + SB2_PH - 1) / SB2_PH;
      const int T = x.tiles_x * x.tiles_y * n;
      const dim3 pg(std::min((T + 7) / 8 * 8, std::max(8, 2 * c->num_cus / 8 * 8)));
      if (gray) hipLaunchKernelGGL(stem_bf16_kernel<1>, pg, dim3(SB2_THREADS), StemB2Cfg<1>::LDS_BYTES, sb->st, x);
      else hipLaunchKernelGGL(stem_bf16_kernel<3>, pg, dim3(SB2_THREADS), StemB2Cfg<3>::LDS_BYTES, sb->st, x);
    } else {
      if (gray) hipLaunchKernelGGL((stem_pool_x3_kernel<1, 3>), grid, dim3(256), 0, sb->st, x);
      else hipLaunchKernelGGL((stem_pool_x3_kernel<3, 3>), grid, dim3(256), 0, sb->st, x);
    }
    return symbol[kind];
  }
  if (kind == STEM_POOL2) {
    if (gray) hipLaunchKernelGGL(stem_pool2_kernel<1>, grid, dim3(256), 0, sb->st, a);
    else hipLaunchKernelGGL(stem_pool2_kernel<3>, grid, dim3(256), 0, sb->st, a);
  } else {
    if (gray) hipLaunchKernelGGL(stem_pool_kernel<1>, grid, dim3(256), 0, sb->st, a);
    else hipLaunchKernelGGL(stem_pool_kernel<3>, grid, dim3(256), 0, sb->st, a);
  }
  return symbol[kind];
}

static void launch_pool(fpc_ctx* c, int i, const Sub& sb) {
  if (stem_kind(c) != STEM_PLAIN) return;
  const int H = c->H, W = c->W, n = sb.n, f0 = sb.f0;
  LaunchTimer t(c, i, sb.st, n);
  const size_t total = (size_t)n * (H / 4) * (W / 4) * 16;
  hipLaunchKernelGGL(maxpool_kernel, dim3((unsigned)((total + 255) / 256)), dim3(256), 0, sb.st,
                     reinterpret_cast<const float4*>(c->stem_out + (size_t)f0 * (H / 2) * (W / 2) * 64),
                     reinterpret_cast<float4*>(c->x0 + (size_t)f0 * (H / 4) * (W / 4) * 64), n, H / 2, W / 2, H / 4, W / 4);
}

static void launch_wblock(fpc_ctx* c, const Op& op, int i, const Sub& sb) {
  const int n = sb.n, f0 = sb.f0;
  LaunchTimer t(c, i, sb.st, n);
  WBlockArgs a = op.wargs;
  a.frame0 = f0;
  diag_stamp(c, op, a, a.tiles_x * a.tiles_y * n);
  a.total = a.tiles_x * a.tiles_y * n;
  a.xcd_order = c->opt.xcd_order ? 1 : 0;
  {
    const unsigned long long xb = (unsigned long long)(f0 + n) * a.H * a.W * a.csx * sizeof(float);
    a.x_bytes = xb > W16_REACH ? (unsigned)W16_REACH : (unsigned)xb;
  }
  int grid = (c->opt.persist_min_tiles > 0 && a.total >= c->opt.persist_min_tiles * c->num_cus) ? c->num_cus : a.total;
  if (g_wkinds[op.wkind].gen == 3) {
    const int fpl = w36_frames_per_launch(a.H, a.W, a.csx, a.cso);
    const float* x0 = a.x;
    float* o0 = a.out;
    const int Hf = a.H, tx_f = a.tiles_x, ty_f = a.tiles_y;
    const WKind sk = c->opt.tiles_round6 ? w36_stacked_kind(op.wkind) : WK_COUNT;
    double mf = 0.0;
    for (int g0 = 0; g0 < n; g0 += fpl) {
      const int gn = std::min(fpl, n - g0);
      a.frame0 = 0;
      a.x = x0 + (size_t)(f0 + g0) * Hf * a.W * a.csx;
      a.out = o0 + (size_t)(f0 + g0) * Hf * a.W * a.cso;
      a.x_bytes = (unsigned)((unsigned long long)gn * Hf * a.W * a.csx * sizeof(float));
      const int srows = w36_stacked_rows(Hf, a.W, gn, sk, tx_f * ty_f);
      const WKind lk = srows ? sk : op.wkind;
      a.H = srows ? gn * Hf : Hf;
      a.frame_h = srows ? Hf : 0;
      a.tiles_x = srows ? (a.W + g_wkinds[sk].TW - 1) / g_wkinds[sk].TW : tx_f;
      a.tiles_y = srows ? srows : ty_f;
      a.total = srows ? a.tiles_x * srows : tx_f * ty_f * gn;
      if (srows) t.wkind = sk;
      mf += srows ? wkind_mfma_flops(g_wkinds[sk], a.total, a.nchunk, a.k8_h + a.k8_x) : op.mfma_flops_per_frame * gn;
      const int cus_cap = c->opt.w36_cus > 0 ? std::min(c->num_cus, c->opt.w36_cus) : c->num_cus;
      const int cus8 = std::max(1, cus_cap / 8 / std::max(1, op.grid_y)), per_xcd = (a.total + 7) / 8;
      const int rounds = (per_xcd + cus8 - 1) / cus8;
      const int grid3 = 8 * std::min(cus8, (per_xcd + rounds - 1) / rounds);
      g_wkinds[lk].launch(a, dim3(std::min(a.total, grid3), op.grid_y), sb.st);
    }
    if (t.wkind >= 0) t.mfma_flops = mf;
    return;
  }
  g_wkinds[op.wkind].launch(a, dim3(std::min(a.total, grid), op.grid_y), sb.st);
}

static void launch_block(fpc_ctx* c, const Op& op, int i, const Sub& sb) {
  LaunchTimer t(c, i, sb.st, sb.n);
  BlockArgs a = op.bargs;
  a.frame0 = sb.f0;
  diag_stamp(c, op, a, a.tiles_x * a.tiles_y * sb.n);
  g_bkinds[op.bkind].launch(a, dim3(a.tiles_x * a.tiles_y * sb.n), sb.st);
}

static void launch_fblock(fpc_ctx* c, const Op& op, int i, const Sub& sb) {
  const int n = sb.n, f0 = sb.f0;
  LaunchTimer t(c, i, sb.st, n);
  BlockBfArgs a = op.fargs;
  a.frame0 = f0;
  a.range_flag = c->split_f16 ? c->status + 1 : nullptr;
  diag_stamp(c, op, a, a.tiles_x * a.tiles_y * n);
  if (g_fkinds[op.fkind].planes != 1) {
    g_fkinds[op.fkind].launch(a, dim3(a.tiles_x * a.tiles_y * n), sb.st);
    return;
  }
  a.total_tiles = a.tiles_x * a.tiles_y * n;
  if (sb.fuse_softmax && op.fused_softmax_capable) {
    const size_t HW = (size_t)c->H * c->W;
    hipMemsetAsync(c->ncand + f0, 0, sizeof(int32_t) * n, sb.st);
    a.softmax = 1;
    a.thresh = c->cfg.conf_thresh;
    a.nmsmap = c->nmsmap + f0 * HW;
    a.cand = c->cand + f0 * HW;
    a.ncand = c->ncand + f0;
  }
  const int g = std::min((a.total_tiles + 7) / 8 * 8, std::max(8, c->fkind_blocks_per_cu[op.fkind] * c->num_cus / op.grid_y / 8 * 8));
  g_fkinds[op.fkind].launch(a, dim3(g, op.grid_y), sb.st);
}

static void launch_conv(fpc_ctx* c, const Op& op, int i, const Sub& sb) {
  LaunchTimer t(c, i, sb.st, sb.n);
  ConvArgs a = op.args;
  a.frame0 = sb.f0;
  const dim3 grid(a.tiles_x * a.tiles_y * sb.n, op.grid_y, op.grid_z);
  if (op.lean) lean_kind(op.kind)->launch(a, grid, sb.st);
  else g_kinds[op.kind].launch(a, grid, sb.st);
}

static void launch_vconv0(fpc_ctx* c, const Op& op, int i, const float* frames, const Sub& sb) {
  LaunchTimer t(c, i, sb.st, sb.n);
  VggConv0Args a{};
  a.in = frames;
  a.w = c->blob + c->vconv0_off;
  a.out = op.pout;
  a.H = c->H; a.W = c->W; a.frame0 = sb.f0;
  hipLaunchKernelGGL(vgg_conv0_kernel, dim3((unsigned)((size_t)sb.n * c->H * c->W / 64)), dim3(256), 0, sb.st, a);
}
static void launch_pool2(fpc_ctx* c, const Op& op, int i, const Sub& sb) {
  LaunchTimer t(c, i, sb.st, sb.n);
  const size_t tot = (size_t)sb.n * (op.pH / 2) * (op.pW / 2) * (op.pC / 4);
  hipLaunchKernelGGL(maxpool2_kernel, dim3((unsigned)((tot + 255) / 256)), dim3(256), 0, sb.st,
                     reinterpret_cast<const float4*>(op.pin), reinterpret_cast<float4*>(op.pout), sb.n, op.pH, op.pW,
                     op.pC / 4, sb.f0);
}
static void launch_l2norm(fpc_ctx* c, const Op& op, int i, const Sub& sb) {
  LaunchTimer t(c, i, sb.st, sb.n);
  const size_t npix = (size_t)sb.n * c->Hc * c->Wc;
  hipLaunchKernelGGL(l2norm256_kernel, dim3((unsigned)((npix + 3) / 4)), dim3(256), 0, sb.st,
                     op.pout + (size_t)sb.f0 * c->Hc * c->Wc * 256, npix);
}

static void run_network(fpc_ctx* c, const float* frames, const Sub& sb0, int which, hipStream_t st) {
  Sub sb = sb0;
  sb.st = st;
  for (size_t i = 0; i < c->ops.size(); ++i) {
    const Op& op = c->ops[i];
    const int br = op.descriptor_branch ? 2 : (op.name.compare(0, 8, "detector") == 0 ? 1 : 0);
    if (br != which) continue;
    if (op.shadow) continue;
    if (op.when == 1 && !sb.small) continue;
    if (op.when == 2 && sb.small) continue;
    switch (op.type) {
      case OP_STEM: launch_stem(c, op, (int)i, frames, &sb); break;
      case OP_POOL: launch_pool(c, (int)i, sb); break;
      case OP_WBLOCK: launch_wblock(c, op, (int)i, sb); break;
      case OP_BLOCK: launch_block(c, op, (int)i, sb); break;
      case OP_BF16: launch_fblock(c, op, (int)i, sb); break;
      case OP_CONV: launch_conv(c, op, (int)i, sb); break;
      case OP_VCONV0: launch_vconv0(c, op, (int)i, frames, sb); break;
      case OP_POOL2: launch_pool2(c, op, (int)i, sb); break;
      case OP_L2NORM: launch_l2norm(c, op, (int)i, sb); break;
      default: break;
    }
  }
}

static Sub on(const Sub& sb, hipStream_t st) {
  Sub r = sb;
  r.st = st;
  return r;
}

static void run_softmax(fpc_ctx* c, const Sub& sb, bool dense_map = true) {
  const size_t HW = (size_t)c->H * c->W;
  hipMemsetAsync(c->ncand + sb.f0, 0, sizeof(int32_t) * sb.n, sb.st);
  LaunchTimer t(c, op_index(c, OP_SOFTMAX), sb.st, sb.n);
  const auto kern = c->bf16 ? softmax_d2s_kernel<true> : softmax_d2s_kernel<false>;
  hipLaunchKernelGGL(kern, dim3(sb.n * c->Hc), dim3(256), (size_t)12 * c->W * sizeof(float), sb.st,
                     c->lg + (size_t)sb.f0 * c->Hc * c->Wc * c->lgcs, c->lgcs, sb.n, c->Hc, c->Wc, c->cfg.conf_thresh,
                     dense_map ? c->prob + sb.f0 * HW : nullptr, c->nmsmap + sb.f0 * HW, c->cand + sb.f0 * HW, c->ncand + sb.f0,
                     c->rowmax + (size_t)sb.f0 * c->Hc);
}

static void run_nms(fpc_ctx* c, const Sub& sb) {
  LaunchTimer t(c, op_index(c, OP_NMS), sb.st, sb.n);
  const size_t HW = (size_t)c->H * c->W;
  const int n = sb.n, f0 = sb.f0;
  NmsArgs a{};
  a.nmsmap = c->nmsmap + f0 * HW; a.cand = c->cand + f0 * HW; a.ncand = c->ncand + f0;
  a.sort_scratch = c->sort_scratch + (size_t)f0 * c->sort_cap;
  a.sort_cap = c->sort_cap;
  const bool chunked = !c->opt.nms_one_workgroup;
  a.aux = chunked ? c->nms_aux + (size_t)f0 * NMS_AUX_INTS : nullptr;
  a.H = c->H; a.W = c->W; a.r = c->cfg.nms_dist; a.border = c->cfg.border_remove; a.cap = c->cap;
  a.count = c->count + f0; a.xy = c->xy + (size_t)f0 * c->cap * 2; a.conf = c->conf + (size_t)f0 * c->cap;
  a.status = c->status;
  a.max_rounds = c->H * c->W;
  const int G = c->opt.nms_g > 0 ? c->opt.nms_g : std::max(1, std::min(16, 512 / n));
  for (int pass = 0; pass < c->opt.nms_passes; ++pass) {
    if (c->cfg.nms_dist == 4)
      hipLaunchKernelGGL(nms_rounds_kernel<4>, dim3(G, n), dim3(NMS_ROUNDS_THREADS), 0, sb.st, a);
    else
      hipLaunchKernelGGL(nms_rounds_kernel<0>, dim3(G, n), dim3(NMS_ROUNDS_THREADS), 0, sb.st, a);
  }
  if (chunked) {
    const bool big = HW > 400000;
    const int GC = big ? 8 : 4;
    hipLaunchKernelGGL(nms_finish_kernel, dim3(n), dim3(NMS_FINISH_THREADS), 0, sb.st, a);
    if (big) {
      hipLaunchKernelGGL(nms_chunk_sort_kernel<4096>, dim3(GC, n), dim3(1024), 4096 * sizeof(unsigned long long), sb.st, a);
      hipLaunchKernelGGL(nms_merge_kernel<4096>, dim3(GC, n), dim3(1024), 4096 * sizeof(unsigned long long), sb.st, a);
    } else {
      hipLaunchKernelGGL(nms_chunk_sort_kernel<2048>, dim3(GC, n), dim3(1024), 2048 * sizeof(unsigned long long), sb.st, a);
      hipLaunchKernelGGL(nms_merge_kernel<2048>, dim3(GC, n), dim3(1024), 2048 * sizeof(unsigned long long), sb.st, a);
    }
  }
  hipLaunchKernelGGL(nms_sort_kernel, dim3(n), dim3(1024), chunked ? 0 : NMS_LDS_KEYS * sizeof(unsigned long long), sb.st, a);
}

static void run_desc(fpc_ctx* c, const Sub& sb, const float* dmap_nhwc) {
  LaunchTimer t(c, op_index(c, OP_DESC), sb.st, sb.n);
  const int by_xcd = sb.n >= 8;
  const int G = std::max(8, c->num_cus * 8 / 8 * 8);
  if (c->D == 256)
    hipLaunchKernelGGL(descriptor16_kernel<16>, dim3(G), dim3(256), 0, sb.st,
                       dmap_nhwc + (size_t)sb.f0 * c->Hc * c->Wc * 256, 256, c->Hc, c->Wc, c->H, c->W, c->count + sb.f0,
                       c->xy + (size_t)sb.f0 * c->cap * 2, c->cap, c->desc_out + (size_t)sb.f0 * c->cap * 256, sb.n, by_xcd);
  else if (c->bf16 && dmap_nhwc == c->desc_map)
    hipLaunchKernelGGL((descriptor16_kernel<8, true>), dim3(G), dim3(256), 0, sb.st,
                       reinterpret_cast<const float*>(reinterpret_cast<const unsigned short*>(dmap_nhwc) + (size_t)sb.f0 * c->Hc * c->Wc * 128),
                       128, c->Hc, c->Wc, c->H, c->W, c->count + sb.f0,
                       c->xy + (size_t)sb.f0 * c->cap * 2, c->cap, c->desc_out + (size_t)sb.f0 * c->cap * 128, sb.n, by_xcd);
  else
    hipLaunchKernelGGL(descriptor16_kernel<8>, dim3(G), dim3(256), 0, sb.st,
                       dmap_nhwc + (size_t)sb.f0 * c->Hc * c->Wc * 128, 128, c->Hc, c->Wc, c->H, c->W, c->count + sb.f0,
                       c->xy + (size_t)sb.f0 * c->cap * 2, c->cap, c->desc_out + (size_t)sb.f0 * c->cap * 128, sb.n, by_xcd);
}

template <typename F>
static int for_each_sub(fpc_ctx* c, int n, F&& body) {
  if (c->timing_every > 1) c->timing = c->timing_calls++ % c->timing_every == 0;
  int parts = std::min<int>((int)c->aux.size() + 1, std::max(1, n / c->opt.min_sub));
  if (parts > 1) HIPCHECK(hipEventRecord(c->ev_fork, c->stream));
  int f0 = 0;
  for (int p = 0; p < parts; ++p) {
    const int cnt = n / parts + (p < n % parts ? 1 : 0);
    Sub sb;
    sb.f0 = f0;
    sb.n = cnt;
    sb.small = n < 2 * c->opt.min_sub && n <= c->small_reach;
    sb.st = p == 0 ? c->stream : c->aux[p - 1];
    sb.side = c->side[p];
    if (sb.small && !c->aux.empty()) sb.side = c->aux[0];
    sb.ev_enc = c->ev_enc[p];
    sb.ev_det = c->ev_det[p];
    if (p) HIPCHECK(hipStreamWaitEvent(sb.st, c->ev_fork, 0));
    body(sb);
    if (p) {
      HIPCHECK(hipEventRecord(c->ev_join[p - 1], sb.st));
      HIPCHECK(hipStreamWaitEvent(c->stream, c->ev_join[p - 1], 0));
    }
    f0 += cnt;
  }
  HIPCHECK(hipGetLastError());
  return FPC_OK;
}

static void run_path(fpc_ctx* c, const float* frames, const Sub& sb0, bool de, int upto) {
  Sub sb = sb0;
  for (const Op& op : c->ops) sb.fuse_softmax |= upto && op.fused_softmax_capable;
  c->logits_valid = !sb.fuse_softmax;
  hipMemsetAsync(c->range + (size_t)sb.f0 * FPC_RANGE_WORDS, 0, sizeof(uint32_t) * FPC_RANGE_WORDS * sb.n, sb.st);
  run_network(c, frames, sb, 0, sb.st);
  if (de && upto && c->opt.nms_aside && !sb.small && sb.side) {
    run_network(c, frames, sb, 1, sb.st);
    if (!sb.fuse_softmax) run_softmax(c, sb, !upto);
    hipEventRecord(sb.ev_enc, sb.st);
    hipStreamWaitEvent(sb.side, sb.ev_enc, 0);
    run_nms(c, on(sb, sb.side));
    hipEventRecord(sb.ev_det, sb.side);
    run_network(c, frames, sb, 2, sb.st);
    hipStreamWaitEvent(sb.st, sb.ev_det, 0);
    run_desc(c, sb, c->desc_map);
    return;
  }
  if (!de || !(c->opt.split_heads || sb.small) || !sb.side) {
    run_network(c, frames, sb, 1, sb.st);
    if (!sb.fuse_softmax) run_softmax(c, sb, !upto);
    if (upto) run_nms(c, sb);
    if (de) {
      run_network(c, frames, sb, 2, sb.st);
      if (upto) run_desc(c, sb, c->desc_map);
    }
    return;
  }
  hipEventRecord(sb.ev_enc, sb.st);
  hipStreamWaitEvent(sb.side, sb.ev_enc, 0);
  const Sub det = on(sb, sb.side);
  run_network(c, frames, sb, 1, sb.side);
  if (!sb.fuse_softmax) run_softmax(c, det, !upto);
  if (upto) run_nms(c, det);
  hipEventRecord(sb.ev_det, sb.side);
  run_network(c, frames, sb, 2, sb.st);
  hipStreamWaitEvent(sb.st, sb.ev_det, 0);
  if (upto) run_desc(c, sb, c->desc_map);
}

}

extern "C" {

int fpc_abi_version(void) { return FPC_ABI_VERSION; }
int fpc_pack_layout_revision(void) { return FPC_PACK_LAYOUT_REVISION; }

#if defined(STEMB_SKIP_LOAD) || defined(STEMB_SKIP_K) || defined(STEMB_SKIP_TILE) || defined(STEMB_SKIP_POOL) || \
    defined(STEMB_SKIP_STORE) || defined(W16_YOUNG_PRIO) || defined(W16_PRIO_SPLIT) || defined(FPC_NO_PIN)
#error "ablation switches are not part of the library: see experiments/harness/"
#endif
const char* fpc_build_flags(void) {
  return "arch=gfx950"
#ifdef FPC_DIAG
         ";diag=1"
#else
         ";diag=0"
#endif
         ";ablations=none";
}

const char* fpc_strerror(int code) {
  switch (code) {
    case FPC_OK: return "ok";
    case FPC_E_INVALID: return "invalid argument or unsupported geometry";
    case FPC_E_NO_DEVICE: return "no usable HIP device (this library has no CPU fallback)";
    case FPC_E_HIP: return "HIP runtime error (see fpc_last_hip_error)";
    case FPC_E_NO_WEIGHTS: return "weights not loaded";
    case FPC_E_MISSING_KEY: return "checkpoint entry missing or of the wrong shape (see fpc_last_hip_error)";
    case FPC_E_CAPACITY: return "caller buffer too small";
    case FPC_E_NOT_CONVERGED: return "NMS round limit hit";
    case FPC_E_RANGE: return "value outside fp16's range in FPC_F32_SPLIT_F16 mode (use FPC_F32_SPLIT or FPC_F32)";
    case FPC_E_NONFINITE: return "a frame of the call holds a NaN or Inf pixel (see fpc_last_hip_error for which)";
    default: return "unknown error";
  }
}

const char* fpc_last_hip_error(void) { return g_hip_err.c_str(); }

int fpc_default_config(fpc_config* cfg) {
  if (!cfg) return FPC_E_INVALID;
  memset(cfg, 0, sizeof(*cfg));
  cfg->device = 0;
  cfg->height = 480;
  cfg->width = 640;
  cfg->max_batch = 1;
  cfg->cell = 8;
  cfg->nms_dist = 4;
  cfg->conf_thresh = 0.015f;
  cfg->border_remove = 4;
  cfg->descriptor_enabled = 1;
  cfg->max_keypoints = 0;
  return FPC_OK;
}

enum { SLOT_MAIN = 0, SLOT_AUX = 1, SLOT_SIDE = 100, SLOT_UPLOAD = 200 };

static int prepare_kernels(fpc_ctx* c, const fpc_config* cfg) {
  if (int rc = allow_dynamic_lds(g_kinds)) return rc;
  if (int rc = allow_dynamic_lds(g_lean_kinds)) return rc;
  if (int rc = allow_dynamic_lds(g_wkinds)) return rc;
  if (int rc = allow_dynamic_lds(g_bkinds)) return rc;
  if (int rc = allow_dynamic_lds(g_fkinds)) return rc;
  static_assert(FK_COUNT <= 64, "fpc_ctx::fkind_blocks_per_cu");
  for (int k = 0; k < FK_COUNT; ++k) {
    int nb = 0;
    HIPCHECK(hipOccupancyMaxActiveBlocksPerMultiprocessor(&nb, g_fkinds[k].fn, g_fkinds[k].threads, g_fkinds[k].lds_bytes));
    c->fkind_blocks_per_cu[k] = std::max(1, nb);
  }
  HIPCHECK(hipFuncSetAttribute((const void*)softmax_d2s_kernel<false>, hipFuncAttributeMaxDynamicSharedMemorySize,
                               12 * cfg->width * (int)sizeof(float)));
  HIPCHECK(hipFuncSetAttribute((const void*)softmax_d2s_kernel<true>, hipFuncAttributeMaxDynamicSharedMemorySize,
                               12 * cfg->width * (int)sizeof(float)));
  HIPCHECK(hipFuncSetAttribute((const void*)stem_bf16_kernel<1>, hipFuncAttributeMaxDynamicSharedMemorySize, StemB2Cfg<1>::LDS_BYTES));
  HIPCHECK(hipFuncSetAttribute((const void*)stem_bf16_kernel<3>, hipFuncAttributeMaxDynamicSharedMemorySize, StemB2Cfg<3>::LDS_BYTES));
  HIPCHECK(hipFuncSetAttribute((const void*)nms_sort_kernel, hipFuncAttributeMaxDynamicSharedMemorySize,
                               NMS_LDS_KEYS * (int)sizeof(unsigned long long)));
#ifdef FPC_DIAG
  print_occupancy(g_fkinds);
  print_occupancy(g_bkinds);
  print_occupancy(g_kinds);
#endif
  return FPC_OK;
}

int fpc_create(fpc_ctx** out, const fpc_config* cfg) {
  if (!out || !cfg) return FPC_E_INVALID;
  *out = nullptr;
  const int mult = (cfg->descriptor_enabled && cfg->arch != FPC_ARCH_VGG) ? 16 : 8;
  if (cfg->in_channels != 0 && cfg->in_channels != 1 && cfg->in_channels != 3) return FPC_E_INVALID;
  if (cfg->dtype < FPC_F32 || cfg->dtype > FPC_F32_SPLIT_F16) return FPC_E_INVALID;
  if (cfg->arch != FPC_ARCH_RESNET && cfg->arch != FPC_ARCH_VGG) return FPC_E_INVALID;
  if (cfg->arch == FPC_ARCH_VGG && (cfg->in_channels != 1 || cfg->dtype == FPC_BF16)) return FPC_E_INVALID;
  if (!(cfg->conf_thresh >= 0.f) || !(cfg->conf_thresh <= 3.0e38f)) return FPC_E_INVALID;
  if (cfg->cell != 8 || cfg->height < 16 || cfg->width < 16 || cfg->height % mult || cfg->width % mult ||
      cfg->max_batch < 1 || cfg->nms_dist < 0 || cfg->nms_dist > 64 || cfg->border_remove < 0 ||
      (long long)cfg->height * cfg->width >= (1ll << 30) ||
      (long long)cfg->max_batch * cfg->height * cfg->width >= (1ll << 28) ||
      cfg->width > 3328)
    return FPC_E_INVALID;
  int ndev = 0;
  if (hipGetDeviceCount(&ndev) != hipSuccess || ndev <= 0 || cfg->device < 0 || cfg->device >= ndev) {
    g_hip_err = "hipGetDeviceCount: no device";
    return FPC_E_NO_DEVICE;
  }
  HIPCHECK(hipSetDevice(cfg->device));
  std::unique_ptr<fpc_ctx> c(new fpc_ctx());
  {
    hipDeviceProp_t prop;
    HIPCHECK(hipGetDeviceProperties(&prop, cfg->device));
    c->num_cus = std::max(1, prop.multiProcessorCount);
  }
  c->cfg = *cfg;
  c->opt = resolve_plan_options(*cfg, [](const char* name) -> const char* { return getenv(name); });
  c->H = cfg->height;
  c->W = cfg->width;
  c->B = cfg->max_batch;
  c->Hc = c->H / 8;
  c->Wc = c->W / 8;
  c->cin = cfg->in_channels == 1 ? 1 : 3;
  c->vgg = cfg->arch == FPC_ARCH_VGG;
  c->D = c->vgg ? 256 : 128;
  c->bf16 = cfg->dtype == FPC_BF16;
  c->split = cfg->dtype == FPC_F32_SPLIT || cfg->dtype == FPC_F32_SPLIT_F16;
  c->split_f16 = cfg->dtype == FPC_F32_SPLIT_F16;
  c->lgcs = (c->bf16 || c->split) ? 80 : 72;
  const int r1 = cfg->nms_dist + 1;
  const int worst = ((c->H + r1 - 1) / r1) * ((c->W + r1 - 1) / r1);
  c->cap = cfg->max_keypoints > 0 ? cfg->max_keypoints : worst;
  c->sort_cap = 1;
  while (c->sort_cap < worst) c->sort_cap <<= 1;
  {
    const int prc = prepare_kernels(c.get(), cfg);
    if (prc != FPC_OK) return prc;
  }
  const bool qprobe = qmap::probe_mode() != 0;
  c->queue_probe = qprobe;
  const auto create_t0 = std::chrono::steady_clock::now();
  std::unique_lock<std::mutex> queue_lock(qmap::state().mu);
  const int probe_rounds0 = qmap::state().dev[cfg->device].rounds;
  c->stream = qmap::acquire(cfg->device, c.get(), SLOT_MAIN, true, qprobe, true);
  if (!c->stream) { qmap::release_owner(c.get()); g_hip_err = "hipStreamCreateWithFlags"; return FPC_E_HIP; }
  c->own_stream = true;
  {
    const int nsub = c->opt.nsub, nside = c->opt.nside;
    auto fail = [&](const char* what) {
      g_hip_err = what;
      queue_lock.unlock();
      fpc_destroy(c.release());
      return FPC_E_HIP;
    };
    if (hipEventCreateWithFlags(&c->ev_fork, hipEventDisableTiming) != hipSuccess) return fail("hipEventCreateWithFlags");
    for (int i = 1; i < nsub; ++i) {
      hipStream_t st = qmap::acquire(cfg->device, c.get(), SLOT_AUX + (i - 1), true, qprobe, true);
      hipEvent_t ev;
      if (!st) return fail("hipStreamCreateWithFlags");
      c->aux.push_back(st);
      if (hipEventCreateWithFlags(&ev, hipEventDisableTiming) != hipSuccess) return fail("hipEventCreateWithFlags");
      c->ev_join.push_back(ev);
    }
    for (int i = 0; i < nsub; ++i) {
      hipStream_t st = nullptr;
      hipEvent_t e1, e2;
      if (i < nside) {
        st = qmap::acquire(cfg->device, c.get(), SLOT_SIDE + i, false, qprobe, true);
        if (!st) return fail("hipStreamCreateWithFlags");
      }
      c->side.push_back(st);
      if (hipEventCreateWithFlags(&e1, hipEventDisableTiming) != hipSuccess) return fail("hipEventCreateWithFlags");
      c->ev_enc.push_back(e1);
      if (hipEventCreateWithFlags(&e2, hipEventDisableTiming) != hipSuccess) return fail("hipEventCreateWithFlags");
      c->ev_det.push_back(e2);
    }
    c->probe_rounds = qmap::state().dev[cfg->device].rounds - probe_rounds0;
    c->placement_ms = std::chrono::duration<double, std::milli>(std::chrono::steady_clock::now() - create_t0).count();
    queue_lock.unlock();
  }
  int rc = FPC_OK;
  if (rc == FPC_OK && getenv("FPC_TEST_FAIL_CREATE")) {
    g_hip_err = "FPC_TEST_FAIL_CREATE is set: fpc_create's failure path was asked for";
    rc = FPC_E_HIP;
  }
  if (rc == FPC_OK) rc = build_plan(c.get());
  if (rc == FPC_OK && c->plan_error) {
    g_hip_err = "no kernel instance for a layer of this dtype / arch combination";
    rc = FPC_E_INVALID;
  }
  if (rc != FPC_OK) {
    fpc_destroy(c.release());
    return rc;
  }
  *out = c.release();
  return FPC_OK;
}

void fpc_destroy(fpc_ctx* c) {
  if (!c) return;
  hipSetDevice(c->cfg.device);
  hipDeviceSynchronize();
  for (auto e : c->event_pool) hipEventDestroy(e);
  for (auto e : c->ev_join) hipEventDestroy(e);
  for (auto e : c->ev_enc) hipEventDestroy(e);
  for (auto e : c->ev_det) hipEventDestroy(e);
  if (c->ev_fork) hipEventDestroy(c->ev_fork);
  {
    std::lock_guard<std::mutex> queue_lock(qmap::state().mu);
    qmap::DeviceQueues& q = qmap::state().dev[c->cfg.device];
    auto give_back = [&](hipStream_t st, int slot) {
      if (!st) return;
      const qmap::Placed* p = qmap::find(c, slot);
      qmap::retire(q, st, p && p->st == st ? p->qclass : qmap::Q_UNKNOWN);
    };
    for (size_t i = 0; i < c->aux.size(); ++i) give_back(c->aux[i], SLOT_AUX + (int)i);
    for (size_t i = 0; i < c->side.size(); ++i) give_back(c->side[i], SLOT_SIDE + (int)i);
    give_back(c->upload, SLOT_UPLOAD);
    if (c->own_stream) give_back(c->stream, SLOT_MAIN);
    qmap::release_owner(c);
  }
  for (Slab* s : c->slabs) s->release();
  if (c->blob) hipFree(c->blob);
  if (c->u8stage) hipFree(c->u8stage);
  if (c->ha_ws) hipFree(c->ha_ws);
  delete c;
}

int fpc_load_weights(fpc_ctx* c, const fpc_tensor* tensors, int n) {
  if (!c || !tensors || n <= 0) return FPC_E_INVALID;
  TensorMap m;
  for (int i = 0; i < n; ++i) {
    if (!tensors[i].name || tensors[i].ndim < 0 || tensors[i].ndim > 4) return FPC_E_INVALID;
    HostTensor t;
    t.data = tensors[i].data;
    t.shape.assign(tensors[i].shape, tensors[i].shape + tensors[i].ndim);
    m[tensors[i].name] = t;
  }
  std::string missing;
  const int rc = pack_all(c, m, &missing);
  if (rc != FPC_OK) {
    g_hip_err = "checkpoint entry: " + missing;
    return rc;
  }
  HIPCHECK(hipSetDevice(c->cfg.device));
  HIPCHECK(hipMemcpy(c->blob, c->host_blob.data(), c->blob_floats * sizeof(float), hipMemcpyHostToDevice));
  c->weights_loaded = true;
  return FPC_OK;
}

size_t fpc_packed_size(const fpc_ctx* c) { return c ? c->blob_floats * sizeof(float) : 0; }
void* fpc_packed_device_ptr(fpc_ctx* c) { return c ? c->blob : nullptr; }

int fpc_export_packed(fpc_ctx* c, void* dst, size_t cap) {
  if (!c || !dst) return FPC_E_INVALID;
  if (!c->weights_loaded) return FPC_E_NO_WEIGHTS;
  if (cap < c->blob_floats * sizeof(float)) return FPC_E_CAPACITY;
  HIPCHECK(hipSetDevice(c->cfg.device));
  HIPCHECK(hipMemcpy(dst, c->blob, c->blob_floats * sizeof(float), hipMemcpyDeviceToHost));
  return FPC_OK;
}

int fpc_import_packed(fpc_ctx* c, const void* src, size_t n) {
  if (!c || !src) return FPC_E_INVALID;
  if (n != c->blob_floats * sizeof(float)) {
    g_hip_err = "packed weights: " + std::to_string(n) + " bytes, this context's plan packs " + std::to_string(c->blob_floats * sizeof(float));
    return FPC_E_INVALID;
  }
  if (!check_blob_header(c, static_cast<const uint32_t*>(src), &g_hip_err)) return FPC_E_INVALID;
  HIPCHECK(hipSetDevice(c->cfg.device));
  HIPCHECK(hipMemcpy(c->blob, src, n, hipMemcpyHostToDevice));
  c->weights_loaded = true;
  return FPC_OK;
}

int fpc_import_packed_device(fpc_ctx* c, const void* src_dev, size_t n) {
  if (!c || !src_dev) return FPC_E_INVALID;
  if (n != c->blob_floats * sizeof(float)) {
    g_hip_err = "packed weights: " + std::to_string(n) + " bytes, this context's plan packs " + std::to_string(c->blob_floats * sizeof(float));
    return FPC_E_INVALID;
  }
  HIPCHECK(hipSetDevice(c->cfg.device));
  uint32_t h[BLOB_HEADER_FLOATS];
  HIPCHECK(hipMemcpy(h, src_dev, sizeof(h), hipMemcpyDeviceToHost));
  if (!check_blob_header(c, h, &g_hip_err)) return FPC_E_INVALID;
  if (src_dev != (const void*)c->blob) {
    c->weights_loaded = false;
    HIPCHECK(hipMemcpy(c->blob, src_dev, n, hipMemcpyDeviceToDevice));
    HIPCHECK(hipDeviceSynchronize());
  }
  c->weights_loaded = true;
  return FPC_OK;
}

int fpc_mark_weights_loaded(fpc_ctx* c) {
  if (!c) return FPC_E_INVALID;
  uint32_t h[BLOB_HEADER_FLOATS];
  HIPCHECK(hipSetDevice(c->cfg.device));
  HIPCHECK(hipMemcpy(h, c->blob, sizeof(h), hipMemcpyDeviceToHost));
  if (!check_blob_header(c, h, &g_hip_err)) {
    c->weights_loaded = false;
    return FPC_E_INVALID;
  }
  c->weights_loaded = true;
  return FPC_OK;
}

uint64_t fpc_plan_hash(const fpc_ctx* c) { return c ? plan_hash(c) : 0; }

int fpc_tile_choice(int what, int H, int W, int frames, unsigned plan_flags) {
  const bool r6 = !(plan_flags & FPC_PLAN_TILES_ROUND5);
  if (H <= 0 || W <= 0 || frames <= 0) return FPC_E_INVALID;
  switch (what) {
    case 0: {
      const WKindInfo& k = g_wkinds[w36_kind(128, H, W)];
      return r6 ? w36_stacked_rows(H, W, frames, WK_W36S_C128_4x4, ((H + k.TH - 1) / k.TH) * ((W + k.TW - 1) / k.TW)) : 0;
    }
    case 1: { const WKindInfo& k = g_wkinds[w36_kind(64, H, W, true, r6)]; return 100 * k.TH + k.TW; }
    case 2: {
      const BKind k5 = BK_B320_s2_K32_C128, k6 = BK_B416_s2_K32_C128;
      const BKindInfo& k = g_bkinds[r6 && block_rows(k6, H, W) < block_rows(k5, H, W) ? k6 : k5];
      return 100 * k.TH + k.TW;
    }
  }
  return FPC_E_INVALID;
}

int fpc_check_guards(fpc_ctx* c, long long* bad_words) {
  if (!c || !bad_words) return FPC_E_INVALID;
  *bad_words = 0;
  if (!c->opt.guard_zones || c->slab.zones.empty()) return FPC_E_INVALID;
  HIPCHECK(hipSetDevice(c->cfg.device));
  HIPCHECK(hipDeviceSynchronize());
  unsigned long long* d = nullptr;
  HIPCHECK(hipMalloc((void**)&d, sizeof(*d)));
  {
    const hipError_t e0 = hipMemset(d, 0, sizeof(*d));
    if (e0 != hipSuccess) hipFree(d);
    HIPCHECK(e0);
  }
  for (const Slab* s : c->slabs) count_zones(c->stream, *s, d);
  unsigned long long h = 0;
  const hipError_t e1 = hipStreamSynchronize(c->stream);
  const hipError_t e2 = hipMemcpy(&h, d, sizeof(h), hipMemcpyDeviceToHost);
  hipFree(d);
  HIPCHECK(e1);
  HIPCHECK(e2);
  *bad_words = (long long)h;
  return FPC_OK;
}

namespace {
typedef int (*nccl_bcast_fn)(const void*, void*, size_t, int, int, void*, hipStream_t);
typedef int (*nccl_rank_fn)(void*, int*);
struct RcclApi {
  nccl_bcast_fn bcast = nullptr;
  nccl_rank_fn user_rank = nullptr;
  bool tried = false;
};
static RcclApi g_rccl;
static bool load_rccl() {
  if (g_rccl.tried) return g_rccl.bcast && g_rccl.user_rank;
  g_rccl.tried = true;
  void* h = nullptr;
  void* f = dlsym(RTLD_DEFAULT, "ncclBroadcast");
  if (!f) {
    h = dlopen("librccl.so.1", RTLD_NOW | RTLD_GLOBAL);
    if (!h) h = dlopen("librccl.so", RTLD_NOW | RTLD_GLOBAL);
    if (!h) return false;
    f = dlsym(h, "ncclBroadcast");
  }
  g_rccl.bcast = reinterpret_cast<nccl_bcast_fn>(f);
  void* r = h ? dlsym(h, "ncclCommUserRank") : dlsym(RTLD_DEFAULT, "ncclCommUserRank");
  g_rccl.user_rank = reinterpret_cast<nccl_rank_fn>(r);
  return g_rccl.bcast && g_rccl.user_rank;
}
}

int fpc_broadcast_weights(fpc_ctx* c, void* nccl_comm, int root) {
  if (!c || !nccl_comm || root < 0) return FPC_E_INVALID;
  if (!load_rccl()) {
    g_hip_err = "librccl.so (ncclBroadcast / ncclCommUserRank) could not be resolved";
    return FPC_E_HIP;
  }
  HIPCHECK(hipSetDevice(c->cfg.device));
  int rank = -1;
  if (g_rccl.user_rank(nccl_comm, &rank) != 0 || rank < 0) {
    g_hip_err = "ncclCommUserRank failed";
    return FPC_E_HIP;
  }
  const bool is_root = rank == root;
  uint32_t* tag_dev = c->bcast_tag;
  uint32_t tag[BLOB_HEADER_FLOATS];
  if (is_root) {
    fill_blob_header(c, tag);
    if (!c->weights_loaded) tag[8] = 0;
    hipMemcpyAsync(tag_dev, tag, sizeof(tag), hipMemcpyHostToDevice, c->stream);
  }
  int nrc = g_rccl.bcast(tag_dev, tag_dev, sizeof(tag),  1, root, nccl_comm, c->stream);
  hipError_t he = hipMemcpyAsync(tag, tag_dev, sizeof(tag), hipMemcpyDeviceToHost, c->stream);
  if (he == hipSuccess) he = hipStreamSynchronize(c->stream);
  if (nrc != 0 || he != hipSuccess) {
    g_hip_err = nrc ? "ncclBroadcast(tag) failed: ncclResult " + std::to_string(nrc) : std::string("tag copy: ") + hipGetErrorString(he);
    return FPC_E_HIP;
  }
  if (tag[0] != BLOB_MAGIC || tag[8] != 1) {
    g_hip_err = "the root rank holds no packed weights (load them on the root before fpc_broadcast_weights)";
    return FPC_E_NO_WEIGHTS;
  }
  const size_t root_bytes = (((size_t)tag[7] << 32) | tag[6]) * sizeof(float);
  std::string why;
  const bool match = check_blob_header(c, tag, &why);
  void* dst = c->blob;
  void* scratch = nullptr;
  bool slab_used = false;
  if (!match) {
    if (hipMalloc(&scratch, root_bytes) == hipSuccess) {
      dst = scratch;
    } else {
      (void)hipGetLastError();
      scratch = nullptr;
      if (root_bytes <= c->blob_floats * sizeof(float)) {
        c->weights_loaded = false;
      } else if (root_bytes <= c->slab.bytes) {
        dst = c->slab.base;
        slab_used = true;
      } else {
        g_hip_err = "no memory to take part in the weight broadcast (" + std::to_string(root_bytes) + " bytes: no scratch, and neither this "
                    "context's blob nor its workspace is that large); the other ranks of this communicator will wait for this one";
        return FPC_E_HIP;
      }
    }
  }
  nrc = g_rccl.bcast(dst, dst, root_bytes, 1, root, nccl_comm, c->stream);
  he = hipStreamSynchronize(c->stream);
  if (scratch) hipFree(scratch);
  if (slab_used) {
    hipMemsetAsync(c->slab.base, 0, std::min(c->slab.bytes, align_up(root_bytes, 256)), c->stream);
    hipStreamSynchronize(c->stream);
    if (c->opt.guard_zones) fill_guards(c);
  }
  if (nrc != 0 || he != hipSuccess) {
    if (match) c->weights_loaded = false;
    g_hip_err = nrc ? "ncclBroadcast(weights) failed: ncclResult " + std::to_string(nrc) : std::string("broadcast: ") + hipGetErrorString(he);
    return FPC_E_HIP;
  }
  if (!match) {
    g_hip_err = why;
    return FPC_E_INVALID;
  }
  c->weights_loaded = true;
  return FPC_OK;
}

int fpc_set_stream(fpc_ctx* c, void* s) {
  if (!c) return FPC_E_INVALID;
  if ((hipStream_t)s == c->stream) return FPC_OK;
  HIPCHECK(hipSetDevice(c->cfg.device));
  std::lock_guard<std::mutex> queue_lock(qmap::state().mu);
  if (c->own_stream && c->stream) {
    hipStreamSynchronize(c->stream);
    hipStreamDestroy(c->stream);
  }
  c->stream = (hipStream_t)s;
  c->own_stream = false;
  qmap::Placed* mainp = qmap::find(c, SLOT_MAIN);
  int k = qmap::Q_UNKNOWN;
  qmap::DeviceQueues& q = qmap::state().dev[c->cfg.device];
  bool memo_hit = false;
  for (const auto& m : c->caller_stream_memo)
    if (m.first == c->stream) { k = m.second; memo_hit = true; }
  if (!memo_hit && c->queue_probe && c->stream && !q.futile && q.anchor.size() >= 2) {
    hipStreamCaptureStatus cap = hipStreamCaptureStatusNone;
    const bool capturing = hipStreamIsCapturing(c->stream, &cap) != hipSuccess || cap != hipStreamCaptureStatusNone;
    if (!capturing && hipStreamQuery(c->stream) == hipSuccess) {
      k = qmap::classify(q, c->stream);
// ... 1292 lines not shown

extern "C++" template <class Source>
static int landmarks_launch(fpc_ctx* c, int n, const Source& src, const float* R, const float* t, const fpc_landmark_params* p,
                            float* xyz, uint8_t* kind, int32_t* counts, int S) {
  if (!R || !t || !xyz || !kind || !landmark_params_ok(p)) return FPC_E_INVALID;
  HIPCHECK(hipSetDevice(c->cfg.device));
  LmArgs a{};
  a.q_fx = p->q_fx; a.q_fy = p->q_fy; a.q_cx = p->q_cx; a.q_cy = p->q_cy;
  a.t_fx = p->t_fx; a.t_fy = p->t_fy; a.t_cx = p->t_cx; a.t_cy = p->t_cy;
  a.thr = p->reproj_threshold;
  const double s = std::sin((double)p->min_parallax_deg * (3.14159265358979323846 / 180.0));
  a.parallax = p->min_parallax_deg > 0.f ? s * s : POSE_PARALLEL;
  hipLaunchKernelGGL(landmarks_kernel<Source>, dim3(n), dim3(256), 0, c->stream, src, a, R, t, xyz, kind, counts, S);
  return launched();
}

int fpc_landmarks_pairs(fpc_ctx* c, int n, const float* q_xy, const float* t_xy, const float* t_xyz, const uint8_t* t_valid,
                        const int32_t* npairs, int stride, const float* R, const float* t, const fpc_landmark_params* p,
                        float* xyz, uint8_t* kind, int32_t* counts) {
  if (!c || !q_xy || !t_xy || !npairs || !explicit_ok(c, n, stride)) return FPC_E_INVALID;
  LmExplicit src{};
  src.q_xy = q_xy; src.t_xy = t_xy; src.t_xyz = t_xyz; src.t_valid = t_valid; src.npairs = npairs; src.stride = stride;
  return landmarks_launch(c, n, src, R, t, p, xyz, kind, counts, stride);
}

int fpc_landmarks_frames(fpc_ctx* c, int n, const int32_t* key_xy, const int32_t* nkey, const float* key_xyz,
                         const uint8_t* key_valid, const int32_t* match, const float* R, const float* t,
                         const fpc_landmark_params* p, float* xyz, uint8_t* kind, int32_t* counts) {
  if (!c || !key_xy || !nkey || !match || !frames_ok(c, n)) return FPC_E_INVALID;
  LmKey src{};
  src.q = LmFrames{c->xy, c->count, match, c->cap};
  src.key_xy = key_xy; src.nkey = nkey; src.key_xyz = key_xyz; src.key_valid = key_valid;
  return landmarks_launch(c, n, src, R, t, p, xyz, kind, counts, c->cap);
}

int fpc_landmarks_bank(fpc_ctx* c, int n, const int32_t* slot, const int32_t* match, const float* R, const float* t,
                       const fpc_landmark_params* p, float* xyz, uint8_t* kind, int32_t* counts) {
  if (!c || !bank_ok(c, n, slot, match)) return FPC_E_INVALID;
  LmBank src{};
  src.q = LmFrames{c->xy, c->count, match, c->cap};
  src.slot = slot; src.bank_xy = c->bank.xy; src.bank_count = c->bank.count;
  src.bank_lm = c->lm_xyzw;
  src.rows = c->bank.rows; src.slots = c->bank.slots;
  return landmarks_launch(c, n, src, R, t, p, xyz, kind, counts, c->cap);
}

int fpc_results(fpc_ctx* c, fpc_device_results* out) {
  if (!c || !out) return FPC_E_INVALID;
  out->count = c->count;
  out->n_candidates = c->ncand;
  out->xy = c->xy;
  out->conf = c->conf;
  out->desc = c->cfg.descriptor_enabled ? c->desc_out : nullptr;
  out->capacity = c->cap;
  out->desc_dim = c->D;
  return FPC_OK;
}

int fpc_get_counts(fpc_ctx* c, int n, int32_t* count, int32_t* ncand) {
  if (!c || n < 1 || n > c->B) return FPC_E_INVALID;
  HIPCHECK(hipSetDevice(c->cfg.device));
  HIPCHECK(hipStreamSynchronize(c->stream));
  int32_t st[2] = {0, 0};
  HIPCHECK(hipMemcpy(st, c->status, sizeof(st), hipMemcpyDeviceToHost));
  if (st[0]) return FPC_E_NOT_CONVERGED;
  if (st[1]) return FPC_E_RANGE;
  if (count) HIPCHECK(hipMemcpy(count, c->count, sizeof(int32_t) * n, hipMemcpyDeviceToHost));
  if (ncand) HIPCHECK(hipMemcpy(ncand, c->ncand, sizeof(int32_t) * n, hipMemcpyDeviceToHost));
  std::vector<uint32_t> rw((size_t)n * FPC_RANGE_WORDS);
  HIPCHECK(hipMemcpy(rw.data(), c->range, rw.size() * sizeof(uint32_t), hipMemcpyDeviceToHost));
  for (int b = 0; b < n; ++b)
    if (rw[(size_t)b * FPC_RANGE_WORDS + RANGE_BAD_INPUT]) {
      g_hip_err = "frame " + std::to_string(b) + " of the last call holds a NaN or Inf pixel";
      return FPC_E_NONFINITE;
    }
  return FPC_OK;
}

int fpc_output_range(fpc_ctx* c, int n, float* max_logit, float* max_desc, int32_t* nonfinite_input) {
  if (!c || n < 1 || n > c->B) return FPC_E_INVALID;
  HIPCHECK(hipSetDevice(c->cfg.device));
  HIPCHECK(hipStreamSynchronize(c->stream));
  std::vector<uint32_t> rw((size_t)n * FPC_RANGE_WORDS);
  HIPCHECK(hipMemcpy(rw.data(), c->range, rw.size() * sizeof(uint32_t), hipMemcpyDeviceToHost));
  std::vector<float> rm((size_t)n * c->Hc);
  if (max_logit) HIPCHECK(hipMemcpy(rm.data(), c->rowmax, rm.size() * sizeof(float), hipMemcpyDeviceToHost));
  for (int b = 0; b < n; ++b) {
    const uint32_t* w = rw.data() + (size_t)b * FPC_RANGE_WORDS;
    float f;
    if (max_logit) {
      f = 0.f;
      for (int i = 0; i < c->Hc; ++i) f = std::max(f, rm[(size_t)b * c->Hc + i]);
      max_logit[b] = f;
    }
    if (max_desc) { memcpy(&f, w + RANGE_MAX_DESC, 4); max_desc[b] = f; }
    if (nonfinite_input) nonfinite_input[b] = (int32_t)w[RANGE_BAD_INPUT];
  }
  return FPC_OK;
}

int fpc_get_keypoints(fpc_ctx* c, int frame, int cap, int32_t* xy, float* conf, float* desc) {
  if (!c || frame < 0 || frame >= c->B || cap < 0) return FPC_E_INVALID;
  HIPCHECK(hipSetDevice(c->cfg.device));
  HIPCHECK(hipStreamSynchronize(c->stream));
  int32_t k = 0;
  HIPCHECK(hipMemcpy(&k, c->count + frame, sizeof(k), hipMemcpyDeviceToHost));
  if (k > cap || k > c->cap) return FPC_E_CAPACITY;
  if (k == 0) return 0;
  if (xy) HIPCHECK(hipMemcpy(xy, c->xy + (size_t)frame * c->cap * 2, sizeof(int32_t) * 2 * k, hipMemcpyDeviceToHost));
  if (conf) HIPCHECK(hipMemcpy(conf, c->conf + (size_t)frame * c->cap, sizeof(float) * k, hipMemcpyDeviceToHost));
  if (desc) {
    if (!c->cfg.descriptor_enabled) return FPC_E_INVALID;
    HIPCHECK(hipMemcpy(desc, c->desc_out + (size_t)frame * c->cap * c->D, sizeof(float) * c->D * k, hipMemcpyDeviceToHost));
  }
  return k;
}

int fpc_set_timing(fpc_ctx* c, int enable) {
  if (!c) return FPC_E_INVALID;
  c->timing_every = enable > 0 ? enable : 0;
  c->timing_calls = 0;
  c->timing = enable != 0;
  c->timings.clear();
  c->events_used = 0;
  return FPC_OK;
}

int fpc_get_timings(fpc_ctx* c, int cap, const char** names, const char** kernels, float* ms, double* flops,
                    double* mfma_flops, double* bytes) {
  if (!c) return FPC_E_INVALID;
  const int n = (int)c->timings.size();
  for (int i = 0; i < n && i < cap; ++i) {
    const Timing& t = c->timings[i];
    float v = 0.f;
    if (hipEventElapsedTime(&v, t.start, t.stop) != hipSuccess) v = -1.f;
    const Op* op = t.op >= 0 ? &c->ops[t.op] : nullptr;
    if (names) names[i] = op ? op->name.c_str() : "?";
    if (kernels) {
      const char* k = "?";
      if (op) switch (op->type) {
          case OP_STEM: k = launch_stem(c, *op, t.op, nullptr, nullptr); break;
          case OP_POOL: k = "maxpool_kernel"; break;
          case OP_CONV: k = op->lean ? lean_kind(op->kind)->symbol : g_kinds[op->kind].symbol; break;
          case OP_BLOCK: k = g_bkinds[op->bkind].symbol; break;
          case OP_WBLOCK: k = g_wkinds[t.wkind >= 0 ? t.wkind : op->wkind].symbol; break;
          case OP_BF16: k = g_fkinds[op->fkind].symbol; break;
          case OP_SOFTMAX: k = "softmax_d2s_kernel"; break;
          case OP_NMS: k = c->opt.nms_one_workgroup ? "nms_rounds_kernel+nms_sort_kernel" : "nms_rounds_kernel+nms_finish_kernel+nms_chunk_sort_kernel+nms_merge_kernel"; break;
          case OP_DESC: k = "descriptor16_kernel"; break;
          case OP_VCONV0: k = "vgg_conv0_kernel"; break;
          case OP_POOL2: k = "maxpool2_kernel"; break;
          case OP_L2NORM: k = "l2norm256_kernel"; break;
        }
      kernels[i] = k;
    }
    if (ms) ms[i] = v;
    if (flops) flops[i] = op ? op->flops_per_frame * t.frames : 0.0;
    if (mfma_flops) mfma_flops[i] = !op ? 0.0 : t.mfma_flops >= 0 ? t.mfma_flops : op->mfma_flops_per_frame * t.frames;
    if (bytes) bytes[i] = op ? op->bytes_per_frame * t.frames : 0.0;
  }
  return n;
}

}
```

Baseline: 12350.

## Stack frames vertically so conv and block tiles span frame seams

Adds stacked variants of the residual-block and conv kernels. They treat a batch of frames as one tall image, so tiles no longer leave ragged partial tiles at each frame's bottom edge. For stride-2 blocks an extra zero row is placed at the seam in LDS, and the A-row bases skip past it for output rows after the seam. The host picks the stacked kernel only when it yields fewer padded rows than the per-frame tiling. This costs one extra LDS row, some seam index arithmetic, and new kernel instances to maintain.

Result: no change. 12400, median of 6 (+0.4%).

```diff
diff --git a/feature-point-cnn_amd/csrc/block_mfma.h b/feature-point-cnn_amd/csrc/block_mfma.h
--- a/feature-point-cnn_amd/csrc/block_mfma.h
+++ b/feature-point-cnn_amd/csrc/block_mfma.h
@@ -34,323 +34,34 @@
   float* out;
   int cso, Ho, Wo, tiles_x, tiles_y, nstore, frame0;
   unsigned x_bytes;
+  int frame_ho;
 #ifdef FPC_DIAG
   unsigned long long* stamps;
 #endif
 };
 
-template <int TH, int TW, int S, int KC, int WM, int WN, int MB, int NB, int CMIDP>
+template <int TH, int TW, int S, int KC, int WM, int WN, int MB, int NB, int CMIDP, bool STACK = false>
 struct BlockCfg {
   using C1 = ConvCfg<TH, TW, S, 3, KC, WM, WN, MB, NB>;
+  static constexpr int HHS = C1::HH + (STACK ? 1 : 0);
+  static constexpr int IN_BYTES = HHS * C1::HW * C1::ROW4 * 16;
   static constexpr int ROWH4 = CMIDP / 4 + 1;
   static constexpr int H_BYTES = C1::M * ROWH4 * 16;
-  static constexpr int LDS_BYTES = C1::LDS_BYTES > H_BYTES ? C1::LDS_BYTES : H_BYTES;
+  static constexpr int LDS_BYTES = IN_BYTES > H_BYTES ? IN_BYTES : H_BYTES;
+  static_assert(!STACK || S == 2, "the stacked walk: stride-2 blocks (pad 1: only the ky = 0 tap crosses a seam)");
   static_assert(CMIDP % 8 == 0 && CMIDP <= C1::N, "mid channels must fit the workgroup's N");
 };
 
 template <int TH, int TW, int S, int KC, int WM, int WN, int MB, int NB, int CMIDP>
 __global__ __launch_bounds__(WM* WN * 64, 2) void block_mfma_kernel(const BlockArgs a) {
-  using C = ConvCfg<TH, TW, S, 3, KC, WM, WN, MB, NB>;
-  using BC = BlockCfg<TH, TW, S, KC, WM, WN, MB, NB, CMIDP>;
-  constexpr int NT = C::NT, HW = C::HW, HH = C::HH, ROW4 = C::ROW4, K8 = KC / 8, KC4 = KC / 4;
-  constexpr int NV = HH * HW * KC4, ITER = (NV + NT - 1) / NT, ROWH4 = BC::ROWH4, NBT = WN * NB;
-  extern __shared__ float4 lds4[];
+  constexpr bool STACK = false;
+#include "block_mfma_body.h"
+}
 
-  const int tid = threadIdx.x, lane = tid & 63, wave = tid >> 6;
-  const int wm = wave / WN, wn = wave % WN;
-  const int half = lane >> 5, l31 = lane & 31;
-  const int tiles = a.tiles_x * a.tiles_y;
-  const int bidx = fpc_xcd_tile_index();
-  const int bl = bidx / tiles;
-  const int b = a.frame0 + bl;
-  const int t = bidx - bl * tiles;
-  const int ty = t / a.tiles_x, tx = t - ty * a.tiles_x;
-
-  FPC_STAMP(0)
-#ifdef FPC_DIAG
-  if (a.stamps && threadIdx.x == 0) {
-    a.stamps[(size_t)blockIdx.x * 8 + 6] = __builtin_amdgcn_s_getreg(63492);
-    a.stamps[(size_t)blockIdx.x * 8 + 7] = __builtin_amdgcn_s_getreg((31 << 11) | 20);
-  }
-#endif
-  int abase[MB];
-#pragma unroll
-  for (int mb = 0; mb < MB; ++mb) {
-    int m = (wm * MB + mb) * 32 + l31;
-    m = m < TH * TW ? m : TH * TW - 1;
-    const int py = m / TW, px = m - py * TW;
-    abase[mb] = ((py * S) * HW + px * S) * ROW4 + half;
-  }
-  constexpr int stepstride = NBT * 64;
-  const __amdgpu_buffer_rsrc_t wrsrc = __builtin_amdgcn_make_buffer_rsrc(
-      const_cast<float4*>(a.w1), 0, (int)((unsigned)(a.nchunk * 9 * K8 + 2) * (unsigned)(stepstride * 16)), 0x00020000);
-  const int wlane = ((wn * NB) * 64 + lane) * 16;
-  int wstep = 0;
-  auto wfrag = [&](int nb) {
-    typedef float f32x4w __attribute__((ext_vector_type(4)));
-    const f32x4w r = __builtin_bit_cast(f32x4w, __builtin_amdgcn_raw_buffer_load_b128(wrsrc, wlane + nb * 1024, wstep, 0));
-    return make_float4(r.x, r.y, r.z, r.w);
-  };
-
-  const int iy0 = ty * TH * S - 1, ix0 = tx * TW * S - 1;
-  typedef float f32x4v __attribute__((ext_vector_type(4)));
-  f32x4v stage[ITER];
-  const __amdgpu_buffer_rsrc_t xrsrc = __builtin_amdgcn_make_buffer_rsrc(const_cast<float*>(a.x), 0, (int)a.x_bytes, 0x00020000);
-  const unsigned xbase = (unsigned)((b * a.H + iy0) * a.W + ix0) * (unsigned)(a.csx * 4);
-  auto load_chunk = [&](int chunk) {
-    const int wlim = chunk < a.nchunk ? a.W : 0;
-#pragma unroll
-    for (int i = 0; i < ITER; ++i) {
-      const int e = tid + i * NT;
-      const int pix = e / KC4, c4 = e - pix * KC4;
-      const int hy = pix / HW, hx = pix - hy * HW;
-      const int iy = iy0 + hy, ix = ix0 + hx;
-      const bool ok = ((unsigned)iy < (unsigned)a.H) & ((unsigned)ix < (unsigned)wlim) & (hy < HH);
-      unsigned off = xbase + (unsigned)(((hy * a.W + hx) * a.csx + chunk * KC + c4 * 4) * 4);
-      asm volatile("" : "+v"(off));
-      stage[i] = __builtin_bit_cast(f32x4v, __builtin_amdgcn_raw_buffer_load_b128(xrsrc, (int)(ok ? off : 0xfffffff0u), 0, 0));
-    }
-  };
-  auto store_chunk = [&]() {
-#pragma unroll
-    for (int i = 0; i < ITER; ++i) {
-      const int e = tid + i * NT;
-      int pix = e / KC4, c4 = e - pix * KC4;
-      if (NV % NT != 0) {
-        const bool in = e < NV;
-        pix = in ? pix : HH * HW - 1;
-        c4 = in ? c4 : KC4;
-      }
-      *reinterpret_cast<f32x4v*>(&lds4[pix * ROW4 + c4]) = stage[i];
-    }
-  };
-
-  f32x16 acc[MB][NB];
-#pragma unroll
-  for (int mb = 0; mb < MB; ++mb)
-#pragma unroll
-    for (int nb = 0; nb < NB; ++nb)
-#pragma unroll
-      for (int r = 0; r < 16; ++r) acc[mb][nb][r] = 0.f;
-
-  load_chunk(0);
-  float4 b0[NB], b1[NB];
-#pragma unroll
-  for (int nb = 0; nb < NB; ++nb) b0[nb] = wfrag(nb);
-  wstep += stepstride * 16;
-#pragma unroll
-  for (int nb = 0; nb < NB; ++nb) b1[nb] = wfrag(nb);
-  wstep += stepstride * 16;
-  for (int chunk = 0; chunk < a.nchunk; ++chunk) {
-    FPC_LDS_BARRIER();
-    store_chunk();
-    FPC_LDS_BARRIER();
-    load_chunk(chunk + 1);
-    if (chunk == 0) { FPC_STAMP(1) }
-    float4 av[MB];
-#pragma unroll
-    for (int mb = 0; mb < MB; ++mb) av[mb] = lds4[abase[mb] + a.tapoff4[0]];
-#pragma unroll
-    for (int tap = 0; tap < 9; ++tap) {
-      const int toff = a.tapoff4[tap];
-      const int toffn = a.tapoff4[tap < 8 ? tap + 1 : 8];
-#pragma unroll
-      for (int k8 = 0; k8 < K8; ++k8) {
-        float4 b2[NB], an[MB];
-#pragma unroll
-        for (int nb = 0; nb < NB; ++nb) b2[nb] = wfrag(nb);
-        wstep += stepstride * 16;
-#pragma unroll
-        for (int mb = 0; mb < MB; ++mb)
-          an[mb] = lds4[abase[mb] + (k8 + 1 < K8 ? toff + (k8 + 1) * 2 : toffn)];
-        __builtin_amdgcn_sched_barrier(0);
-#pragma unroll
-        for (int j = 0; j < 4; ++j)
-#pragma unroll
-          for (int mb = 0; mb < MB; ++mb)
-#pragma unroll
-            for (int nb = 0; nb < NB; ++nb) {
-              const float af = j == 0 ? av[mb].x : j == 1 ? av[mb].y : j == 2 ? av[mb].z : av[mb].w;
-              const float bf = j == 0 ? b0[nb].x : j == 1 ? b0[nb].y : j == 2 ? b0[nb].z : b0[nb].w;
-              acc[mb][nb] = __builtin_amdgcn_mfma_f32_32x32x2f32(af, bf, acc[mb][nb], 0, 0, 0);
-            }
-#pragma unroll
-        for (int nb = 0; nb < NB; ++nb) {
-          b0[nb] = b1[nb];
-          b1[nb] = b2[nb];
-        }
-#pragma unroll
-        for (int mb = 0; mb < MB; ++mb) av[mb] = an[mb];
-      }
-    }
-  }
-
-  FPC_STAMP(2)
-  constexpr int KH = CMIDP / 8, RING = 4;
-  const int nsteps2 = KH + a.k8_x;
-  const float4* wq = a.w2 + (size_t)(wn * NB) * 64 + lane;
-  float4 cb[RING][NB];
-  auto load_b = [&](int slot, int step) {
-    const float4* pw = wq + (size_t)min(step, nsteps2 + 1) * stepstride;
-#pragma unroll
-    for (int nb = 0; nb < NB; ++nb) cb[slot][nb] = pw[nb * 64];
-  };
-#pragma unroll
-  for (int s_ = 0; s_ < RING - 1; ++s_) load_b(s_, s_);
-  FPC_LDS_BARRIER();
-  {
-    float* hl = reinterpret_cast<float*>(lds4);
-#pragma unroll
-    for (int nb = 0; nb < NB; ++nb) {
-      const int n = (wn * NB + nb) * 32 + l31;
-      const float bias = a.b1[n];
-#pragma unroll
-      for (int mb = 0; mb < MB; ++mb)
-#pragma unroll
-        for (int r = 0; r < 16; ++r) {
-          const int m = (wm * MB + mb) * 32 + (r & 3) + 8 * (r >> 2) + 4 * half;
-          const float v = acc[mb][nb][r] + bias;
-          if (n < CMIDP) hl[m * (ROWH4 * 4) + n] = v > 0.f ? v : 0.f;
-          acc[mb][nb][r] = 0.f;
-        }
-    }
-  }
-  FPC_LDS_BARRIER();
-
-  FPC_STAMP(3)
-  int hbase[MB];
-#pragma unroll
-  for (int mb = 0; mb < MB; ++mb) hbase[mb] = ((wm * MB + mb) * 32 + l31) * ROWH4 + half;
-  auto mfma_step = [&](const float4 (&av)[MB], int slot) {
-#pragma unroll
-    for (int j = 0; j < 4; ++j)
-#pragma unroll
-      for (int mb = 0; mb < MB; ++mb)
-#pragma unroll
-        for (int nb = 0; nb < NB; ++nb) {
-          const float af = j == 0 ? av[mb].x : j == 1 ? av[mb].y : j == 2 ? av[mb].z : av[mb].w;
-          const float bf = j == 0 ? cb[slot][nb].x : j == 1 ? cb[slot][nb].y : j == 2 ? cb[slot][nb].z : cb[slot][nb].w;
-          acc[mb][nb] = __builtin_amdgcn_mfma_f32_32x32x2f32(af, bf, acc[mb][nb], 0, 0, 0);
-        }
-  };
-  const float* xrow[MB];
-#pragma unroll
-  for (int mb = 0; mb < MB; ++mb) {
-    int m = (wm * MB + mb) * 32 + l31;
-    m = m < TH * TW ? m : TH * TW - 1;
-    const int py = m / TW, px = m - py * TW;
-    int y = (ty * TH + py) * S, x = (tx * TW + px) * S;
-    y = y < a.H ? y : a.H - 1;
-    x = x < a.W ? x : a.W - 1;
-    xrow[mb] = a.x + ((size_t)(b * a.H + y) * a.W + x) * a.csx + half * 4;
-  }
-  typedef float f4v __attribute__((ext_vector_type(4)));
-  auto ldx = [&](int mb, int k8) {
-    const f4v v = *reinterpret_cast<const f4v*>(xrow[mb] + (k8 < a.k8_x ? k8 : 0) * 8);
-    return make_float4(v.x, v.y, v.z, v.w);
-  };
-  float4 xa[4][MB];
-  if (a.k8_x > 0) {
-#pragma unroll
-    for (int u = 0; u < 4; ++u)
-#pragma unroll
-      for (int mb = 0; mb < MB; ++mb) xa[u][mb] = ldx(mb, u);
-  }
-  {
-    float4 av[MB];
-#pragma unroll
-    for (int mb = 0; mb < MB; ++mb) av[mb] = lds4[hbase[mb]];
-#pragma unroll
-    for (int k8 = 0; k8 < KH; ++k8) {
-      float4 an[MB];
-      load_b((k8 + RING - 1) % RING, k8 + RING - 1);
-#pragma unroll
-      for (int mb = 0; mb < MB; ++mb) an[mb] = lds4[hbase[mb] + (k8 + 1 < KH ? k8 + 1 : k8) * 2];
-      __builtin_amdgcn_sched_barrier(0);
-      mfma_step(av, k8 % RING);
-#pragma unroll
-      for (int mb = 0; mb < MB; ++mb) av[mb] = an[mb];
-    }
-  }
-
-  for (int k8 = 0; k8 < a.k8_x; k8 += 8) {
-    float4 xb[4][MB];
-#pragma unroll
-    for (int u = 0; u < 4; ++u) {
-      load_b((KH + u + RING - 1) % RING, KH + k8 + u + RING - 1);
-#pragma unroll
-      for (int mb = 0; mb < MB; ++mb) xb[u][mb] = ldx(mb, k8 + 4 + u);
-      __builtin_amdgcn_sched_barrier(0);
-      mfma_step(xa[u], (KH + u) % RING);
-    }
-#pragma unroll
-    for (int u = 0; u < 4; ++u) {
-      load_b((KH + u + RING - 1) % RING, KH + k8 + 4 + u + RING - 1);
-#pragma unroll
-      for (int mb = 0; mb < MB; ++mb) xa[u][mb] = ldx(mb, k8 + 8 + u);
-      __builtin_amdgcn_sched_barrier(0);
-      mfma_step(xb[u], (KH + u) % RING);
-    }
-  }
-
-  FPC_STAMP(4)
-  FPC_LDS_BARRIER();
-  {
-    float* ol = reinterpret_cast<float*>(lds4);
-#pragma unroll
-    for (int nb = 0; nb < NB; ++nb) {
-      const int n = (wn * NB + nb) * 32 + l31;
-      const float bias = a.b2[n];
-#pragma unroll
-      for (int mb = 0; mb < MB; ++mb)
-#pragma unroll
-        for (int r = 0; r < 16; ++r) {
-          const int m = (wm * MB + mb) * 32 + (r & 3) + 8 * (r >> 2) + 4 * half;
-          if (n < CMIDP) ol[m * (ROWH4 * 4) + n] = acc[mb][nb][r] + bias;
-        }
-    }
-  }
-  FPC_LDS_BARRIER();
-  {
-    constexpr int C4 = CMIDP / 4;
-    constexpr int NE = TH * TW * C4, EIT = (NE + NT - 1) / NT;
-    const int oyb = ty * TH, oxb = tx * TW;
-    const bool ident = a.k8_x == 0;
-    float4 idv[EIT];
-    if (ident) {
-#pragma unroll
-      for (int i = 0; i < EIT; ++i) {
-        const int e = tid + i * NT;
-        const int m = e / C4, c4 = e - m * C4;
-        const int py = m / TW, px = m - py * TW;
-        const int y = oyb + py, x = oxb + px;
-        const bool ok = (NE % NT == 0 || e < NE) && y < a.Ho && x < a.Wo;
-        idv[i] = *reinterpret_cast<const float4*>(a.x + (ok ? ((size_t)(b * a.Ho + y) * a.Wo + x) * a.csx + c4 * 4 : 0));
-      }
-    }
-#pragma unroll
-    for (int i = 0; i < EIT; ++i) {
-      const int e = tid + i * NT;
-      const int m = e / C4, c4 = e - m * C4;
-      const int py = m / TW, px = m - py * TW;
-      const int y = oyb + py, x = oxb + px;
-      if ((NE % NT == 0 || e < NE) && y < a.Ho && x < a.Wo) {
-        float4 v = lds4[m * ROWH4 + c4];
-        if (ident) {
-          v.x += idv[i].x;
-          v.y += idv[i].y;
-          v.z += idv[i].z;
-          v.w += idv[i].w;
-        }
-        v.x = v.x > 0.f ? v.x : 0.f;
-        v.y = v.y > 0.f ? v.y : 0.f;
-        v.z = v.z > 0.f ? v.z : 0.f;
-        v.w = v.w > 0.f ? v.w : 0.f;
-        *reinterpret_cast<float4*>(a.out + ((size_t)(b * a.Ho + y) * a.Wo + x) * a.cso + c4 * 4) = v;
-      }
-    }
-  }
-  FPC_STAMP(5)
+template <int TH, int TW, int S, int KC, int WM, int WN, int MB, int NB, int CMIDP>
+__global__ __launch_bounds__(WM* WN * 64, 2) void stacked_block_mfma_kernel(const BlockArgs a) {
+  constexpr bool STACK = true;
+#include "block_mfma_body.h"
 }
 
 
diff --git a/feature-point-cnn_amd/csrc/block_mfma_body.h b/feature-point-cnn_amd/csrc/block_mfma_body.h
--- /dev/null
+++ b/feature-point-cnn_amd/csrc/block_mfma_body.h
@@ -0,0 +1,315 @@
+  using C = ConvCfg<TH, TW, S, 3, KC, WM, WN, MB, NB>;
+  using BC = BlockCfg<TH, TW, S, KC, WM, WN, MB, NB, CMIDP, STACK>;
+  constexpr int NT = C::NT, HW = C::HW, HH = BC::HHS, ROW4 = C::ROW4, K8 = KC / 8, KC4 = KC / 4;
+  constexpr int NV = HH * HW * KC4, ITER = (NV + NT - 1) / NT, ROWH4 = BC::ROWH4, NBT = WN * NB;
+  extern __shared__ float4 lds4[];
+
+  const int tid = threadIdx.x, lane = tid & 63, wave = tid >> 6;
+  const int wm = wave / WN, wn = wave % WN;
+  const int half = lane >> 5, l31 = lane & 31;
+  const int tiles = a.tiles_x * a.tiles_y;
+  const int bidx = fpc_xcd_tile_index();
+  const int bl = bidx / tiles;
+  const int b = a.frame0 + bl;
+  const int t = bidx - bl * tiles;
+  const int ty = t / a.tiles_x, tx = t - ty * a.tiles_x;
+
+  FPC_STAMP(0)
+#ifdef FPC_DIAG
+  if (a.stamps && threadIdx.x == 0) {
+    a.stamps[(size_t)blockIdx.x * 8 + 6] = __builtin_amdgcn_s_getreg(63492);
+    a.stamps[(size_t)blockIdx.x * 8 + 7] = __builtin_amdgcn_s_getreg((31 << 11) | 20);
+  }
+#endif
+  int seam = TH;
+  if constexpr (STACK) {
+    const int in = (ty * TH) % a.frame_ho;
+    const int left = in ? a.frame_ho - in : 0;
+    seam = left < TH ? left : TH;
+  }
+  const int zrow = 2 * seam + 1;
+  int abase[MB];
+#pragma unroll
+  for (int mb = 0; mb < MB; ++mb) {
+    int m = (wm * MB + mb) * 32 + l31;
+    m = m < TH * TW ? m : TH * TW - 1;
+    const int py = m / TW, px = m - py * TW;
+    abase[mb] = ((py * S) * HW + px * S) * ROW4 + half;
+    if constexpr (STACK) abase[mb] += py >= seam ? HW * ROW4 : 0;
+  }
+  constexpr int stepstride = NBT * 64;
+  const __amdgpu_buffer_rsrc_t wrsrc = __builtin_amdgcn_make_buffer_rsrc(
+      const_cast<float4*>(a.w1), 0, (int)((unsigned)(a.nchunk * 9 * K8 + 2) * (unsigned)(stepstride * 16)), 0x00020000);
+  const int wlane = ((wn * NB) * 64 + lane) * 16;
+  int wstep = 0;
+  auto wfrag = [&](int nb) {
+    typedef float f32x4w __attribute__((ext_vector_type(4)));
+    const f32x4w r = __builtin_bit_cast(f32x4w, __builtin_amdgcn_raw_buffer_load_b128(wrsrc, wlane + nb * 1024, wstep, 0));
+    return make_float4(r.x, r.y, r.z, r.w);
+  };
+
+  const int iy0 = ty * TH * S - 1, ix0 = tx * TW * S - 1;
+  typedef float f32x4v __attribute__((ext_vector_type(4)));
+  f32x4v stage[ITER];
+  const __amdgpu_buffer_rsrc_t xrsrc = __builtin_amdgcn_make_buffer_rsrc(const_cast<float*>(a.x), 0, (int)a.x_bytes, 0x00020000);
+  const unsigned xbase = (unsigned)((b * a.H + iy0) * a.W + ix0) * (unsigned)(a.csx * 4);
+  auto load_chunk = [&](int chunk) {
+    const int wlim = chunk < a.nchunk ? a.W : 0;
+#pragma unroll
+    for (int i = 0; i < ITER; ++i) {
+      const int e = tid + i * NT;
+      const int pix = e / KC4, c4 = e - pix * KC4;
+      int hy = pix / HW;
+      const int hx = pix - hy * HW;
+      bool row_ok = hy < HH;
+      if constexpr (STACK) {
+        row_ok &= hy != zrow;
+        hy -= hy > zrow ? 1 : 0;
+      }
+      const int iy = iy0 + hy, ix = ix0 + hx;
+      const bool ok = ((unsigned)iy < (unsigned)a.H) & ((unsigned)ix < (unsigned)wlim) & row_ok;
+      unsigned off = xbase + (unsigned)(((hy * a.W + hx) * a.csx + chunk * KC + c4 * 4) * 4);
+      asm volatile("" : "+v"(off));
+      stage[i] = __builtin_bit_cast(f32x4v, __builtin_amdgcn_raw_buffer_load_b128(xrsrc, (int)(ok ? off : 0xfffffff0u), 0, 0));
+    }
+  };
+  auto store_chunk = [&]() {
+#pragma unroll
+    for (int i = 0; i < ITER; ++i) {
+      const int e = tid + i * NT;
+      int pix = e / KC4, c4 = e - pix * KC4;
+      if (NV % NT != 0) {
+        const bool in = e < NV;
+        pix = in ? pix : HH * HW - 1;
+        c4 = in ? c4 : KC4;
+      }
+      *reinterpret_cast<f32x4v*>(&lds4[pix * ROW4 + c4]) = stage[i];
+    }
+  };
+
+  f32x16 acc[MB][NB];
+#pragma unroll
+  for (int mb = 0; mb < MB; ++mb)
+#pragma unroll
+    for (int nb = 0; nb < NB; ++nb)
+#pragma unroll
+      for (int r = 0; r < 16; ++r) acc[mb][nb][r] = 0.f;
+
+  load_chunk(0);
+  float4 b0[NB], b1[NB];
+#pragma unroll
+  for (int nb = 0; nb < NB; ++nb) b0[nb] = wfrag(nb);
+  wstep += stepstride * 16;
+#pragma unroll
+  for (int nb = 0; nb < NB; ++nb) b1[nb] = wfrag(nb);
+  wstep += stepstride * 16;
+  for (int chunk = 0; chunk < a.nchunk; ++chunk) {
+    FPC_LDS_BARRIER();
+    store_chunk();
+    FPC_LDS_BARRIER();
+    load_chunk(chunk + 1);
+    if (chunk == 0) { FPC_STAMP(1) }
+    float4 av[MB];
+#pragma unroll
+    for (int mb = 0; mb < MB; ++mb) av[mb] = lds4[abase[mb] + a.tapoff4[0]];
+#pragma unroll
+    for (int tap = 0; tap < 9; ++tap) {
+      const int toff = a.tapoff4[tap];
+      const int toffn = a.tapoff4[tap < 8 ? tap + 1 : 8];
+#pragma unroll
+      for (int k8 = 0; k8 < K8; ++k8) {
+        float4 b2[NB], an[MB];
+#pragma unroll
+        for (int nb = 0; nb < NB; ++nb) b2[nb] = wfrag(nb);
+        wstep += stepstride * 16;
+#pragma unroll
+        for (int mb = 0; mb < MB; ++mb)
+          an[mb] = lds4[abase[mb] + (k8 + 1 < K8 ? toff + (k8 + 1) * 2 : toffn)];
+        __builtin_amdgcn_sched_barrier(0);
+#pragma unroll
+        for (int j = 0; j < 4; ++j)
+#pragma unroll
+          for (int mb = 0; mb < MB; ++mb)
+#pragma unroll
+            for (int nb = 0; nb < NB; ++nb) {
+              const float af = j == 0 ? av[mb].x : j == 1 ? av[mb].y : j == 2 ? av[mb].z : av[mb].w;
+              const float bf = j == 0 ? b0[nb].x : j == 1 ? b0[nb].y : j == 2 ? b0[nb].z : b0[nb].w;
+              acc[mb][nb] = __builtin_amdgcn_mfma_f32_32x32x2f32(af, bf, acc[mb][nb], 0, 0, 0);
+            }
+#pragma unroll
+        for (int nb = 0; nb < NB; ++nb) {
+          b0[nb] = b1[nb];
+          b1[nb] = b2[nb];
+        }
+#pragma unroll
+        for (int mb = 0; mb < MB; ++mb) av[mb] = an[mb];
+      }
+    }
+  }
+
+  FPC_STAMP(2)
+  constexpr int KH = CMIDP / 8, RING = 4;
+  const int nsteps2 = KH + a.k8_x;
+  const float4* wq = a.w2 + (size_t)(wn * NB) * 64 + lane;
+  float4 cb[RING][NB];
+  auto load_b = [&](int slot, int step) {
+    const float4* pw = wq + (size_t)min(step, nsteps2 + 1) * stepstride;
+#pragma unroll
+    for (int nb = 0; nb < NB; ++nb) cb[slot][nb] = pw[nb * 64];
+  };
+#pragma unroll
+  for (int s_ = 0; s_ < RING - 1; ++s_) load_b(s_, s_);
+  FPC_LDS_BARRIER();
+  {
+    float* hl = reinterpret_cast<float*>(lds4);
+#pragma unroll
+    for (int nb = 0; nb < NB; ++nb) {
+      const int n = (wn * NB + nb) * 32 + l31;
+      const float bias = a.b1[n];
+#pragma unroll
+      for (int mb = 0; mb < MB; ++mb)
+#pragma unroll
+        for (int r = 0; r < 16; ++r) {
+          const int m = (wm * MB + mb) * 32 + (r & 3) + 8 * (r >> 2) + 4 * half;
+          const float v = acc[mb][nb][r] + bias;
+          if (n < CMIDP) hl[m * (ROWH4 * 4) + n] = v > 0.f ? v : 0.f;
+          acc[mb][nb][r] = 0.f;
+        }
+    }
+  }
+  FPC_LDS_BARRIER();
+
+  FPC_STAMP(3)
+  int hbase[MB];
+#pragma unroll
+  for (int mb = 0; mb < MB; ++mb) hbase[mb] = ((wm * MB + mb) * 32 + l31) * ROWH4 + half;
+  auto mfma_step = [&](const float4 (&av)[MB], int slot) {
+#pragma unroll
+    for (int j = 0; j < 4; ++j)
+#pragma unroll
+      for (int mb = 0; mb < MB; ++mb)
+#pragma unroll
+        for (int nb = 0; nb < NB; ++nb) {
+          const float af = j == 0 ? av[mb].x : j == 1 ? av[mb].y : j == 2 ? av[mb].z : av[mb].w;
+          const float bf = j == 0 ? cb[slot][nb].x : j == 1 ? cb[slot][nb].y : j == 2 ? cb[slot][nb].z : cb[slot][nb].w;
+          acc[mb][nb] = __builtin_amdgcn_mfma_f32_32x32x2f32(af, bf, acc[mb][nb], 0, 0, 0);
+        }
+  };
+  const float* xrow[MB];
+#pragma unroll
+  for (int mb = 0; mb < MB; ++mb) {
+    int m = (wm * MB + mb) * 32 + l31;
+    m = m < TH * TW ? m : TH * TW - 1;
+    const int py = m / TW, px = m - py * TW;
+    int y = (ty * TH + py) * S, x = (tx * TW + px) * S;
+    y = y < a.H ? y : a.H - 1;
+    x = x < a.W ? x : a.W - 1;
+    xrow[mb] = a.x + ((size_t)(b * a.H + y) * a.W + x) * a.csx + half * 4;
+  }
+  typedef float f4v __attribute__((ext_vector_type(4)));
+  auto ldx = [&](int mb, int k8) {
+    const f4v v = *reinterpret_cast<const f4v*>(xrow[mb] + (k8 < a.k8_x ? k8 : 0) * 8);
+    return make_float4(v.x, v.y, v.z, v.w);
+  };
+  float4 xa[4][MB];
+  if (a.k8_x > 0) {
+#pragma unroll
+    for (int u = 0; u < 4; ++u)
+#pragma unroll
+      for (int mb = 0; mb < MB; ++mb) xa[u][mb] = ldx(mb, u);
+  }
+  {
+    float4 av[MB];
+#pragma unroll
+    for (int mb = 0; mb < MB; ++mb) av[mb] = lds4[hbase[mb]];
+#pragma unroll
+    for (int k8 = 0; k8 < KH; ++k8) {
+      float4 an[MB];
+      load_b((k8 + RING - 1) % RING, k8 + RING - 1);
+#pragma unroll
+      for (int mb = 0; mb < MB; ++mb) an[mb] = lds4[hbase[mb] + (k8 + 1 < KH ? k8 + 1 : k8) * 2];
+      __builtin_amdgcn_sched_barrier(0);
+      mfma_step(av, k8 % RING);
+#pragma unroll
+      for (int mb = 0; mb < MB; ++mb) av[mb] = an[mb];
+    }
+  }
+
+  for (int k8 = 0; k8 < a.k8_x; k8 += 8) {
+    float4 xb[4][MB];
+#pragma unroll
+    for (int u = 0; u < 4; ++u) {
+      load_b((KH + u + RING - 1) % RING, KH + k8 + u + RING - 1);
+#pragma unroll
+      for (int mb = 0; mb < MB; ++mb) xb[u][mb] = ldx(mb, k8 + 4 + u);
+      __builtin_amdgcn_sched_barrier(0);
+      mfma_step(xa[u], (KH + u) % RING);
+    }
+#pragma unroll
+    for (int u = 0; u < 4; ++u) {
+      load_b((KH + u + RING - 1) % RING, KH + k8 + 4 + u + RING - 1);
+#pragma unroll
+      for (int mb = 0; mb < MB; ++mb) xa[u][mb] = ldx(mb, k8 + 8 + u);
+      __builtin_amdgcn_sched_barrier(0);
+      mfma_step(xb[u], (KH + u) % RING);
+    }
+  }
+
+  FPC_STAMP(4)
+  FPC_LDS_BARRIER();
+  {
+    float* ol = reinterpret_cast<float*>(lds4);
+#pragma unroll
+    for (int nb = 0; nb < NB; ++nb) {
+      const int n = (wn * NB + nb) * 32 + l31;
+      const float bias = a.b2[n];
+#pragma unroll
+      for (int mb = 0; mb < MB; ++mb)
+#pragma unroll
+        for (int r = 0; r < 16; ++r) {
+          const int m = (wm * MB + mb) * 32 + (r & 3) + 8 * (r >> 2) + 4 * half;
+          if (n < CMIDP) ol[m * (ROWH4 * 4) + n] = acc[mb][nb][r] + bias;
+        }
+    }
+  }
+  FPC_LDS_BARRIER();
+  {
+    constexpr int C4 = CMIDP / 4;
+    constexpr int NE = TH * TW * C4, EIT = (NE + NT - 1) / NT;
+    const int oyb = ty * TH, oxb = tx * TW;
+    const bool ident = a.k8_x == 0;
+    float4 idv[EIT];
+    if (ident) {
+#pragma unroll
+      for (int i = 0; i < EIT; ++i) {
+        const int e = tid + i * NT;
+        const int m = e / C4, c4 = e - m * C4;
+        const int py = m / TW, px = m - py * TW;
+        const int y = oyb + py, x = oxb + px;
+        const bool ok = (NE % NT == 0 || e < NE) && y < a.Ho && x < a.Wo;
+        idv[i] = *reinterpret_cast<const float4*>(a.x + (ok ? ((size_t)(b * a.Ho + y) * a.Wo + x) * a.csx + c4 * 4 : 0));
+      }
+    }
+#pragma unroll
+    for (int i = 0; i < EIT; ++i) {
+      const int e = tid + i * NT;
+      const int m = e / C4, c4 = e - m * C4;
+      const int py = m / TW, px = m - py * TW;
+      const int y = oyb + py, x = oxb + px;
+      if ((NE % NT == 0 || e < NE) && y < a.Ho && x < a.Wo) {
+        float4 v = lds4[m * ROWH4 + c4];
+        if (ident) {
+          v.x += idv[i].x;
+          v.y += idv[i].y;
+          v.z += idv[i].z;
+          v.w += idv[i].w;
+        }
+        v.x = v.x > 0.f ? v.x : 0.f;
+        v.y = v.y > 0.f ? v.y : 0.f;
+        v.z = v.z > 0.f ? v.z : 0.f;
+        v.w = v.w > 0.f ? v.w : 0.f;
+        *reinterpret_cast<float4*>(a.out + ((size_t)(b * a.Ho + y) * a.Wo + x) * a.cso + c4 * 4) = v;
+      }
+    }
+  }
+  FPC_STAMP(5)
diff --git a/feature-point-cnn_amd/csrc/conv2_mfma_body.h b/feature-point-cnn_amd/csrc/conv2_mfma_body.h
--- /dev/null
+++ b/feature-point-cnn_amd/csrc/conv2_mfma_body.h
@@ -0,0 +1,190 @@
+  using C = ConvCfg<TH, TW, S, EXT, KC, WM, WN, MB, NB>;
+  using C2 = Conv2Cfg<TH, TW, S, EXT, KC, WM, WN, MB, NB, STACK>;
+  constexpr int NT = C::NT, HW = C::HW, HH = C2::HHS, ROW4 = C::ROW4, K8 = KC / 8, KC4 = KC / 4, N = C::N;
+  constexpr int NV = HH * HW * KC4, ITER = (NV + NT - 1) / NT, ROWO4 = C2::ROWO4;
+  extern __shared__ float4 lds4[];
+  typedef float f32x4w __attribute__((ext_vector_type(4)));
+
+  const int tid = threadIdx.x, lane = tid & 63, wave = tid >> 6;
+  const int wm = wave / WN, wn = wave % WN;
+  const int half = lane >> 5, l31 = lane & 31;
+  const int tiles = a.tiles_x * a.tiles_y;
+  const int bidx = fpc_xcd_tile_index();
+  const int bl = bidx / tiles;
+  const int b = a.frame0 + bl;
+  const int t = bidx - bl * tiles;
+  const int ty = t / a.tiles_x, tx = t - ty * a.tiles_x;
+  const int subi = gridDim.z - 1 - blockIdx.z;
+  const ConvSub& sp = a.sub[subi];
+  int seam = TH + 1;
+  if constexpr (STACK && EXT > 1) {
+    const int left = a.frame_h - (ty * TH) % a.frame_h;
+    seam = left <= TH ? left : TH + 1;
+  }
+
+  int abase[MB];
+#pragma unroll
+  for (int mb = 0; mb < MB; ++mb) {
+    int m = (wm * MB + mb) * 32 + l31;
+    m = m < TH * TW ? m : TH * TW - 1;
+    const int py = m / TW, px = m - py * TW;
+    abase[mb] = ((py * S) * HW + px * S) * ROW4 + half;
+    if constexpr (STACK && EXT > 1) abase[mb] += py >= seam ? HW * ROW4 : 0;
+  }
+  const int stepstride = a.nbt * 64;
+  const __amdgpu_buffer_rsrc_t wrsrc = __builtin_amdgcn_make_buffer_rsrc(
+      const_cast<float4*>(sp.wfrag), 0, (int)((unsigned)(a.nchunk0 * sp.ntaps * K8 + 2) * (unsigned)(stepstride * 16)), 0x00020000);
+  const int wlane = (((blockIdx.y * WN + wn) * NB) * 64 + lane) * 16;
+  int wstep = 0;
+  auto wfrag = [&](int nb) {
+    const f32x4w r = __builtin_bit_cast(f32x4w, __builtin_amdgcn_raw_buffer_load_b128(wrsrc, wlane + nb * 1024, wstep, 0));
+    return make_float4(r.x, r.y, r.z, r.w);
+  };
+
+  const int iy0 = ty * TH * S - a.pad, ix0 = tx * TW * S - a.pad;
+  const __amdgpu_buffer_rsrc_t xrsrc = __builtin_amdgcn_make_buffer_rsrc(
+      const_cast<float*>(a.in0) + (size_t)b * a.H * a.W * a.cs0, 0, a.H * a.W * a.cs0 * 4, 0x00020000);
+  int eoff[ITER], eslot[ITER];
+#pragma unroll
+  for (int i = 0; i < ITER; ++i) {
+    const int e = tid + i * NT;
+    int pix = e / KC4, c4 = e - pix * KC4;
+    const int hy = pix / HW, hx = pix - hy * HW;
+    int iy = iy0 + hy;
+    const int ix = ix0 + hx;
+    bool ok = (NV % NT == 0 || e < NV) & ((unsigned)ix < (unsigned)a.W);
+    if constexpr (STACK && EXT > 1) {
+      iy -= hy > seam ? 1 : 0;
+      ok &= hy != seam;
+    }
+    ok &= (unsigned)iy < (unsigned)a.H;
+    eoff[i] = ok ? ((iy * a.W + ix) * a.cs0 + c4 * 4) * 4 : CONV2_MARKER;
+    if (NV % NT != 0) {
+      const bool in = e < NV;
+      pix = in ? pix : HH * HW - 1;
+      c4 = in ? c4 : KC4;
+    }
+    eslot[i] = pix * ROW4 + c4;
+  }
+  f32x4w stage[ITER];
+  auto load_chunk = [&](int chunk) {
+    const int cbase = chunk < a.nchunk0 ? chunk * (KC * 4) : CONV2_MARKER;
+#pragma unroll
+    for (int i = 0; i < ITER; ++i) {
+      int voff;
+      asm("v_add_i32 %0, %1, %2 clamp" : "=v"(voff) : "v"(eoff[i]), "s"(cbase));
+      stage[i] = __builtin_bit_cast(f32x4w, __builtin_amdgcn_raw_buffer_load_b128(xrsrc, voff, 0, 0));
+    }
+  };
+  auto store_chunk = [&]() {
+#pragma unroll
+    for (int i = 0; i < ITER; ++i) *reinterpret_cast<f32x4w*>(&lds4[eslot[i]]) = stage[i];
+  };
+
+  f32x16 acc[MB][NB];
+#pragma unroll
+  for (int mb = 0; mb < MB; ++mb)
+#pragma unroll
+    for (int nb = 0; nb < NB; ++nb)
+#pragma unroll
+      for (int r = 0; r < 16; ++r) acc[mb][nb][r] = 0.f;
+
+  const int nchunks = a.nchunk0, ntaps = sp.ntaps;
+  load_chunk(0);
+  float4 b0[NB], b1[NB];
+#pragma unroll
+  for (int nb = 0; nb < NB; ++nb) b0[nb] = wfrag(nb);
+  wstep += stepstride * 16;
+#pragma unroll
+  for (int nb = 0; nb < NB; ++nb) b1[nb] = wfrag(nb);
+  wstep += stepstride * 16;
+
+  for (int chunk = 0; chunk < nchunks; ++chunk) {
+    FPC_LDS_BARRIER();
+    store_chunk();
+    FPC_LDS_BARRIER();
+    load_chunk(chunk + 1);
+    float4 av[MB];
+#pragma unroll
+    for (int mb = 0; mb < MB; ++mb) av[mb] = lds4[abase[mb] + sp.tapoff4[0]];
+    for (int tap = 0; tap < ntaps; ++tap) {
+      const int toff = sp.tapoff4[tap];
+      const int toffn = sp.tapoff4[tap + 1 < ntaps ? tap + 1 : tap];
+#pragma unroll
+      for (int k8 = 0; k8 < K8; ++k8) {
+        float4 b2[NB], an[MB];
+#pragma unroll
+        for (int nb = 0; nb < NB; ++nb) b2[nb] = wfrag(nb);
+        wstep += stepstride * 16;
+#pragma unroll
+        for (int mb = 0; mb < MB; ++mb) an[mb] = lds4[abase[mb] + (k8 + 1 < K8 ? toff + (k8 + 1) * 2 : toffn)];
+        __builtin_amdgcn_sched_barrier(0);
+#pragma unroll
+        for (int j = 0; j < 4; ++j)
+#pragma unroll
+          for (int mb = 0; mb < MB; ++mb)
+#pragma unroll
+            for (int nb = 0; nb < NB; ++nb) {
+              const float af = j == 0 ? av[mb].x : j == 1 ? av[mb].y : j == 2 ? av[mb].z : av[mb].w;
+              const float bf = j == 0 ? b0[nb].x : j == 1 ? b0[nb].y : j == 2 ? b0[nb].z : b0[nb].w;
+              acc[mb][nb] = __builtin_amdgcn_mfma_f32_32x32x2f32(af, bf, acc[mb][nb], 0, 0, 0);
+            }
+#pragma unroll
+        for (int nb = 0; nb < NB; ++nb) {
+          b0[nb] = b1[nb];
+          b1[nb] = b2[nb];
+        }
+#pragma unroll
+        for (int mb = 0; mb < MB; ++mb) av[mb] = an[mb];
+      }
+    }
+  }
+
+  constexpr int C4 = N / 4, NE = TH * TW * C4, EIT = (NE + NT - 1) / NT;
+  const int oyb = ty * TH, oxb = tx * TW;
+  const int nbase = blockIdx.y * N;
+  const __amdgpu_buffer_rsrc_t orsrc = __builtin_amdgcn_make_buffer_rsrc(a.out + (size_t)b * a.OH * a.OW * a.cso, 0, a.OH * a.OW * a.cso * 4, 0x00020000);
+  const __amdgpu_buffer_rsrc_t rrsrc = __builtin_amdgcn_make_buffer_rsrc(
+      const_cast<float*>(a.res ? a.res : a.out) + (size_t)b * a.OH * a.OW * (a.res ? a.csr : a.cso), 0, a.res ? a.OH * a.OW * a.csr * 4 : 0, 0x00020000);
+  int ooff[EIT], olds[EIT];
+  f32x4w idv[EIT];
+#pragma unroll
+  for (int i = 0; i < EIT; ++i) {
+    const int e = tid + i * NT;
+    const int m = e / C4, c4 = e - m * C4;
+    const int py = m / TW, px = m - py * TW;
+    const int y = oyb + py, x = oxb + px;
+    const bool ok = (NE % NT == 0 || e < NE) & (y < a.Ho) & (x < a.Wo);
+    const int opix = (y * a.oys + sp.oy0) * a.OW + x * a.oxs + sp.ox0;
+    ooff[i] = ok ? (opix * a.cso + nbase + c4 * 4) * 4 : CONV2_MARKER;
+    olds[i] = (NE % NT == 0 || e < NE) ? m * ROWO4 + c4 : 0;
+    idv[i] = __builtin_bit_cast(f32x4w, __builtin_amdgcn_raw_buffer_load_b128(rrsrc, ok ? (opix * a.csr + nbase + c4 * 4) * 4 : CONV2_MARKER, 0, 0));
+  }
+  FPC_LDS_BARRIER();
+  {
+    float* ol = reinterpret_cast<float*>(lds4);
+#pragma unroll
+    for (int nb = 0; nb < NB; ++nb) {
+      const int nl = (wn * NB + nb) * 32 + l31;
+      const float bias = a.bias[nbase + nl];
+#pragma unroll
+      for (int mb = 0; mb < MB; ++mb)
+#pragma unroll
+        for (int r = 0; r < 16; ++r) {
+          const int m = (wm * MB + mb) * 32 + (r & 3) + 8 * (r >> 2) + 4 * half;
+          ol[m * (ROWO4 * 4) + nl] = acc[mb][nb][r] + bias;
+        }
+    }
+  }
+  FPC_LDS_BARRIER();
+  const float floor_ = a.relu ? 0.f : -3.0e38f;
+#pragma unroll
+  for (int i = 0; i < EIT; ++i) {
+    f32x4w v = *reinterpret_cast<const f32x4w*>(&lds4[olds[i]]);
+    v += idv[i];
+    v.x = fmaxf(v.x, floor_);
+    v.y = fmaxf(v.y, floor_);
+    v.z = fmaxf(v.z, floor_);
+    v.w = fmaxf(v.w, floor_);
+    __builtin_amdgcn_raw_buffer_store_b128(__builtin_bit_cast(__attribute__((ext_vector_type(4))) unsigned, v), orsrc, ooff[i], 0, 0);
+  }
diff --git a/feature-point-cnn_amd/csrc/conv_mfma.h b/feature-point-cnn_amd/csrc/conv_mfma.h
--- a/feature-point-cnn_amd/csrc/conv_mfma.h
+++ b/feature-point-cnn_amd/csrc/conv_mfma.h
@@ -41,6 +41,7 @@
   int nbt;
   int frame0;
   ConvSub sub[4];
+  int frame_h;
 };
 
 template <int TH, int TW, int S, int EXT, int KC, int WM, int WN, int MB, int NB>
@@ -221,194 +222,27 @@
 
 #define CONV2_MARKER 0x7fffff00
 
-template <int TH, int TW, int S, int EXT, int KC, int WM, int WN, int MB, int NB>
+template <int TH, int TW, int S, int EXT, int KC, int WM, int WN, int MB, int NB, bool STACK = false>
 struct Conv2Cfg {
   using C = ConvCfg<TH, TW, S, EXT, KC, WM, WN, MB, NB>;
+  static constexpr int HHS = C::HH + (STACK && EXT > 1 ? 1 : 0);
+  static constexpr int IN_BYTES = HHS * C::HW * C::ROW4 * 16;
   static constexpr int ROWO4 = C::N / 4 + 1;
   static constexpr int OUT_BYTES = C::M * ROWO4 * 16;
-  static constexpr int LDS_BYTES = C::LDS_BYTES > OUT_BYTES ? C::LDS_BYTES : OUT_BYTES;
+  static constexpr int LDS_BYTES = IN_BYTES > OUT_BYTES ? IN_BYTES : OUT_BYTES;
+  static_assert(!STACK || (S == 1 && EXT <= 2), "the stacked walk: 1x1 and ConvTranspose phases (taps at dy = 0, 1)");
 };
 
 template <int TH, int TW, int S, int EXT, int KC, int WM, int WN, int MB, int NB>
 __global__ __launch_bounds__(WM* WN * 64, 2) void conv2_mfma_kernel(const ConvArgs a) {
-  using C = ConvCfg<TH, TW, S, EXT, KC, WM, WN, MB, NB>;
-  using C2 = Conv2Cfg<TH, TW, S, EXT, KC, WM, WN, MB, NB>;
-  constexpr int NT = C::NT, HW = C::HW, HH = C::HH, ROW4 = C::ROW4, K8 = KC / 8, KC4 = KC / 4, N = C::N;
-  constexpr int NV = HH * HW * KC4, ITER = (NV + NT - 1) / NT, ROWO4 = C2::ROWO4;
-  extern __shared__ float4 lds4[];
-  typedef float f32x4w __attribute__((ext_vector_type(4)));
-
-  const int tid = threadIdx.x, lane = tid & 63, wave = tid >> 6;
-  const int wm = wave / WN, wn = wave % WN;
-  const int half = lane >> 5, l31 = lane & 31;
-  const int tiles = a.tiles_x * a.tiles_y;
-  const int bidx = fpc_xcd_tile_index();
-  const int bl = bidx / tiles;
-  const int b = a.frame0 + bl;
-  const int t = bidx - bl * tiles;
-  const int ty = t / a.tiles_x, tx = t - ty * a.tiles_x;
-  const int subi = gridDim.z - 1 - blockIdx.z;
-  const ConvSub& sp = a.sub[subi];
-
-  int abase[MB];
-#pragma unroll
-  for (int mb = 0; mb < MB; ++mb) {
-    int m = (wm * MB + mb) * 32 + l31;
-    m = m < TH * TW ? m : TH * TW - 1;
-    const int py = m / TW, px = m - py * TW;
-    abase[mb] = ((py * S) * HW + px * S) * ROW4 + half;
-  }
-  const int stepstride = a.nbt * 64;
-  const __amdgpu_buffer_rsrc_t wrsrc = __builtin_amdgcn_make_buffer_rsrc(
-      const_cast<float4*>(sp.wfrag), 0, (int)((unsigned)(a.nchunk0 * sp.ntaps * K8 + 2) * (unsigned)(stepstride * 16)), 0x00020000);
-  const int wlane = (((blockIdx.y * WN + wn) * NB) * 64 + lane) * 16;
-  int wstep = 0;
-  auto wfrag = [&](int nb) {
-    const f32x4w r = __builtin_bit_cast(f32x4w, __builtin_amdgcn_raw_buffer_load_b128(wrsrc, wlane + nb * 1024, wstep, 0));
-    return make_float4(r.x, r.y, r.z, r.w);
-  };
-
-  const int iy0 = ty * TH * S - a.pad, ix0 = tx * TW * S - a.pad;
-  const __amdgpu_buffer_rsrc_t xrsrc = __builtin_amdgcn_make_buffer_rsrc(
-      const_cast<float*>(a.in0) + (size_t)b * a.H * a.W * a.cs0, 0, a.H * a.W * a.cs0 * 4, 0x00020000);
-  int eoff[ITER], eslot[ITER];
-#pragma unroll
-  for (int i = 0; i < ITER; ++i) {
-    const int e = tid + i * NT;
-    int pix = e / KC4, c4 = e - pix * KC4;
-    const int hy = pix / HW, hx = pix - hy * HW;
-    const int iy = iy0 + hy, ix = ix0 + hx;
-    const bool ok = (NV % NT == 0 || e < NV) & ((unsigned)iy < (unsigned)a.H) & ((unsigned)ix < (unsigned)a.W);
-    eoff[i] = ok ? ((iy * a.W + ix) * a.cs0 + c4 * 4) * 4 : CONV2_MARKER;
-    if (NV % NT != 0) {
-      const bool in = e < NV;
-      pix = in ? pix : HH * HW - 1;
-      c4 = in ? c4 : KC4;
-    }
-    eslot[i] = pix * ROW4 + c4;
-  }
-  f32x4w stage[ITER];
-  auto load_chunk = [&](int chunk) {
-    const int cbase = chunk < a.nchunk0 ? chunk * (KC * 4) : CONV2_MARKER;
-#pragma unroll
-    for (int i = 0; i < ITER; ++i) {
-      int voff;
-      asm("v_add_i32 %0, %1, %2 clamp" : "=v"(voff) : "v"(eoff[i]), "s"(cbase));
-      stage[i] = __builtin_bit_cast(f32x4w, __builtin_amdgcn_raw_buffer_load_b128(xrsrc, voff, 0, 0));
-    }
-  };
-  auto store_chunk = [&]() {
-#pragma unroll
-    for (int i = 0; i < ITER; ++i) *reinterpret_cast<f32x4w*>(&lds4[eslot[i]]) = stage[i];
-  };
-
-  f32x16 acc[MB][NB];
-#pragma unroll
-  for (int mb = 0; mb < MB; ++mb)
-#pragma unroll
-    for (int nb = 0; nb < NB; ++nb)
-#pragma unroll
-      for (int r = 0; r < 16; ++r) acc[mb][nb][r] = 0.f;
-
-  const int nchunks = a.nchunk0, ntaps = sp.ntaps;
-  load_chunk(0);
-  float4 b0[NB], b1[NB];
-#pragma unroll
-  for (int nb = 0; nb < NB; ++nb) b0[nb] = wfrag(nb);
-  wstep += stepstride * 16;
-#pragma unroll
-  for (int nb = 0; nb < NB; ++nb) b1[nb] = wfrag(nb);
-  wstep += stepstride * 16;
-
-  for (int chunk = 0; chunk < nchunks; ++chunk) {
-    FPC_LDS_BARRIER();
-    store_chunk();
-    FPC_LDS_BARRIER();
-    load_chunk(chunk + 1);
-    float4 av[MB];
-#pragma unroll
-    for (int mb = 0; mb < MB; ++mb) av[mb] = lds4[abase[mb] + sp.tapoff4[0]];
-    for (int tap = 0; tap < ntaps; ++tap) {
-      const int toff = sp.tapoff4[tap];
-      const int toffn = sp.tapoff4[tap + 1 < ntaps ? tap + 1 : tap];
-#pragma unroll
-      for (int k8 = 0; k8 < K8; ++k8) {
-        float4 b2[NB], an[MB];
-#pragma unroll
-        for (int nb = 0; nb < NB; ++nb) b2[nb] = wfrag(nb);
-        wstep += stepstride * 16;
-#pragma unroll
-        for (int mb = 0; mb < MB; ++mb) an[mb] = lds4[abase[mb] + (k8 + 1 < K8 ? toff + (k8 + 1) * 2 : toffn)];
-        __builtin_amdgcn_sched_barrier(0);
-#pragma unroll
-        for (int j = 0; j < 4; ++j)
-#pragma unroll
-          for (int mb = 0; mb < MB; ++mb)
-#pragma unroll
-            for (int nb = 0; nb < NB; ++nb) {
-              const float af = j == 0 ? av[mb].x : j == 1 ? av[mb].y : j == 2 ? av[mb].z : av[mb].w;
-              const float bf = j == 0 ? b0[nb].x : j == 1 ? b0[nb].y : j == 2 ? b0[nb].z : b0[nb].w;
-              acc[mb][nb] = __builtin_amdgcn_mfma_f32_32x32x2f32(af, bf, acc[mb][nb], 0, 0, 0);
-            }
-#pragma unroll
-        for (int nb = 0; nb < NB; ++nb) {
-          b0[nb] = b1[nb];
-          b1[nb] = b2[nb];
-        }
-#pragma unroll
-        for (int mb = 0; mb < MB; ++mb) av[mb] = an[mb];
-      }
-    }
-  }
-
-  constexpr int C4 = N / 4, NE = TH * TW * C4, EIT = (NE + NT - 1) / NT;
-  const int oyb = ty * TH, oxb = tx * TW;
-  const int nbase = blockIdx.y * N;
-  const __amdgpu_buffer_rsrc_t orsrc = __builtin_amdgcn_make_buffer_rsrc(a.out + (size_t)b * a.OH * a.OW * a.cso, 0, a.OH * a.OW * a.cso * 4, 0x00020000);
-  const __amdgpu_buffer_rsrc_t rrsrc = __builtin_amdgcn_make_buffer_rsrc(
-      const_cast<float*>(a.res ? a.res : a.out) + (size_t)b * a.OH * a.OW * (a.res ? a.csr : a.cso), 0, a.res ? a.OH * a.OW * a.csr * 4 : 0, 0x00020000);
-  int ooff[EIT], olds[EIT];
-  f32x4w idv[EIT];
-#pragma unroll
-  for (int i = 0; i < EIT; ++i) {
-    const int e = tid + i * NT;
-    const int m = e / C4, c4 = e - m * C4;
-    const int py = m / TW, px = m - py * TW;
-    const int y = oyb + py, x = oxb + px;
-    const bool ok = (NE % NT == 0 || e < NE) & (y < a.Ho) & (x < a.Wo);
-    const int opix = (y * a.oys + sp.oy0) * a.OW + x * a.oxs + sp.ox0;
-    ooff[i] = ok ? (opix * a.cso + nbase + c4 * 4) * 4 : CONV2_MARKER;
-    olds[i] = (NE % NT == 0 || e < NE) ? m * ROWO4 + c4 : 0;
-    idv[i] = __builtin_bit_cast(f32x4w, __builtin_amdgcn_raw_buffer_load_b128(rrsrc, ok ? (opix * a.csr + nbase + c4 * 4) * 4 : CONV2_MARKER, 0, 0));
-  }
-  FPC_LDS_BARRIER();
-  {
-    float* ol = reinterpret_cast<float*>(lds4);
-#pragma unroll
-    for (int nb = 0; nb < NB; ++nb) {
-      const int nl = (wn * NB + nb) * 32 + l31;
-      const float bias = a.bias[nbase + nl];
-#pragma unroll
-      for (int mb = 0; mb < MB; ++mb)
-#pragma unroll
-        for (int r = 0; r < 16; ++r) {
-          const int m = (wm * MB + mb) * 32 + (r & 3) + 8 * (r >> 2) + 4 * half;
-          ol[m * (ROWO4 * 4) + nl] = acc[mb][nb][r] + bias;
-        }
-    }
-  }
-  FPC_LDS_BARRIER();
-  const float floor_ = a.relu ? 0.f : -3.0e38f;
-#pragma unroll
-  for (int i = 0; i < EIT; ++i) {
-    f32x4w v = *reinterpret_cast<const f32x4w*>(&lds4[olds[i]]);
-    v += idv[i];
-    v.x = fmaxf(v.x, floor_);
-    v.y = fmaxf(v.y, floor_);
-    v.z = fmaxf(v.z, floor_);
-    v.w = fmaxf(v.w, floor_);
-    __builtin_amdgcn_raw_buffer_store_b128(__builtin_bit_cast(__attribute__((ext_vector_type(4))) unsigned, v), orsrc, ooff[i], 0, 0);
-  }
-}
-
-}
+  constexpr bool STACK = false;
+#include "conv2_mfma_body.h"
+}
+
+template <int TH, int TW, int S, int EXT, int KC, int WM, int WN, int MB, int NB>
+__global__ __launch_bounds__(WM* WN * 64, 2) void stacked_conv2_mfma_kernel(const ConvArgs a) {
+  constexpr bool STACK = true;
+#include "conv2_mfma_body.h"
+}
+
+}
diff --git a/feature-point-cnn_amd/csrc/fpc_api.hip b/feature-point-cnn_amd/csrc/fpc_api.hip
--- a/feature-point-cnn_amd/csrc/fpc_api.hip
+++ b/feature-point-cnn_amd/csrc/fpc_api.hip
@@ -166,6 +166,40 @@
     FPC_BLOCK_KINDS(X)
 #undef X
 };
+
+#define FPC_STACKED_CONV_KINDS(X)      \
+  X(8, 8, 1, 2, 64, 1, 4, 2, 1)        \
+  X(8, 8, 1, 1, 64, 1, 4, 2, 1)
+struct StackedConvInfo : Instance<ConvArgs> {
+  const char* symbol;
+  int TH, TW, S, EXT, KC, WM, WN, MB, NB;
+};
+static const StackedConvInfo g_stacked_convs[] = {
+#define X(TH, TW, S, EXT, KC, WM, WN, MB, NB)                                                                                                          \
+  {instance_of<stacked_conv2_mfma_kernel<TH, TW, S, EXT, KC, WM, WN, MB, NB>, Conv2Cfg<TH, TW, S, EXT, KC, WM, WN, MB, NB, true>, WM * WN * 64, ConvArgs>(), \
+   "stacked_conv2_mfma_kernel<" #TH ", " #TW ", " #S ", " #EXT ", " #KC ", " #WM ", " #WN ", " #MB ", " #NB ">", TH, TW, S, EXT, KC, WM, WN, MB, NB},
+    FPC_STACKED_CONV_KINDS(X)
+#undef X
+};
+#define FPC_STACKED_BLOCK_KINDS(X)     \
+  X(4, 8, 2, 32, 1, 4, 1, 2, 256)
+struct StackedBlockInfo : Instance<BlockArgs> {
+  const char* symbol;
+  int TH, TW, S, KC, WM, WN, MB, NB, CMIDP;
+};
+static const StackedBlockInfo g_stacked_blocks[] = {
+#define X(TH, TW, S, KC, WM, WN, MB, NB, CMIDP)                                                                                                              \
+  {instance_of<stacked_block_mfma_kernel<TH, TW, S, KC, WM, WN, MB, NB, CMIDP>, BlockCfg<TH, TW, S, KC, WM, WN, MB, NB, CMIDP, true>, WM * WN * 64, BlockArgs>(), \
+   "stacked_block_mfma_kernel<" #TH ", " #TW ", " #S ", " #KC ", " #WM ", " #WN ", " #MB ", " #NB ", " #CMIDP ">", TH, TW, S, KC, WM, WN, MB, NB, CMIDP},
+    FPC_STACKED_BLOCK_KINDS(X)
+#undef X
+};
+static const int STACKED_MIN_FRAMES = 5;
+static int stacked_tiles(int Hf, int W, int frames, int th, int tw, int m, long rows_now) {
+  if (frames < STACKED_MIN_FRAMES || th > Hf) return 0;
+  const int tiles = ((frames * Hf + th - 1) / th) * ((W + tw - 1) / tw);
+  return (long)tiles * m < rows_now ? tiles : 0;
+}
 
 #define FPC_WBLOCK_KINDS(X)     \
   X(W816_K32_C64, 32, 2, 64)    \
@@ -439,6 +473,7 @@
   int frames;
   int wkind = -1;
   double mfma_flops = -1.0;
+  const char* symbol = nullptr;
 };
 
 using GuardZones = std::vector<std::pair<size_t, size_t>>;
@@ -772,12 +807,12 @@
   bool desc_branch;
 };
 
-static bool conv_is_lean(const fpc_ctx* c, const Op& op) {
+static bool conv2_takes(const fpc_ctx* c, const Op& op) {
   const KindInfo& k = g_kinds[op.kind];
   const ConvArgs& a = op.args;
-  return c->opt.conv_lean && lean_kind(op.kind) && a.nchunk1 == 0 && a.nstore == op.grid_y * (k.WN * k.NB * 32) && a.cso % 4 == 0 &&
-         (!a.res || a.csr % 4 == 0);
-}
+  return c->opt.conv_lean && a.nchunk1 == 0 && a.nstore == op.grid_y * (k.WN * k.NB * 32) && a.cso % 4 == 0 && (!a.res || a.csr % 4 == 0);
+}
+static bool conv_is_lean(const fpc_ctx* c, const Op& op) { return lean_kind(op.kind) && conv2_takes(c, op); }
 
 static void add_conv(fpc_ctx* c, const ConvSpec& s, size_t* blob_off) {
   const KindInfo& k = g_kinds[s.kind];
@@ -2104,6 +2139,7 @@
   hipEvent_t s{}, e{};
   int wkind = -1;
   double mfma_flops = -1.0;
+  const char* symbol = nullptr;
   LaunchTimer(fpc_ctx* c_, int op_, hipStream_t st_, int frames_) : c(c_), op(op_), st(st_), frames(frames_) {
     if (c->timing) {
       s = next_event(c);
@@ -2114,7 +2150,7 @@
   ~LaunchTimer() {
     if (c->timing) {
       hipEventRecord(e, st);
-      c->timings.push_back({s, e, op, frames, wkind, mfma_flops});
+      c->timings.push_back({s, e, op, frames, wkind, mfma_flops, symbol});
     }
   }
 };
@@ -2266,10 +2302,46 @@
   g_wkinds[op.wkind].launch(a, dim3(std::min(a.total, grid), op.grid_y), sb.st);
 }
 
+static const StackedBlockInfo* stacked_block_kind(BKind bk, int Ho, int Wo, int n, int* tiles) {
+  const BKindInfo& k0 = g_bkinds[bk];
+  for (const StackedBlockInfo& s : g_stacked_blocks) {
+    if (s.KC != k0.KC || s.WN * s.NB != k0.WN * k0.NB || s.S != k0.S || s.CMIDP != k0.CMIDP) continue;
+    *tiles = stacked_tiles(Ho, Wo, n, s.TH, s.TW, s.WM * s.MB * 32, n * block_rows(bk, Ho, Wo));
+    if (*tiles) return &s;
+  }
+  return nullptr;
+}
+static const StackedBlockInfo* stacked_block(const fpc_ctx* c, const Op& op, int n, int* tiles) {
+  const BlockArgs& a = op.bargs;
+  if (!c->opt.tiles_round6 || c->vgg || a.H != 2 * a.Ho || a.W != 2 * a.Wo) return nullptr;
+  if ((unsigned long long)n * a.H * a.W * a.csx * sizeof(float) >= 0x7fffff00ull) return nullptr;
+  return stacked_block_kind(op.bkind, a.Ho, a.Wo, n, tiles);
+}
+
 static void launch_block(fpc_ctx* c, const Op& op, int i, const Sub& sb) {
   LaunchTimer t(c, i, sb.st, sb.n);
   BlockArgs a = op.bargs;
   a.frame0 = sb.f0;
+  int tiles = 0;
+  if (const StackedBlockInfo* s = stacked_block(c, op, sb.n, &tiles)) {
+    const int n = sb.n, HWp = (s->TW - 1) * s->S + 3, ROW4 = s->KC / 4 + 1;
+    a.x += (size_t)sb.f0 * a.H * a.W * a.csx;
+    a.out += (size_t)sb.f0 * a.Ho * a.Wo * a.cso;
+    a.x_bytes = (unsigned)((size_t)n * a.H * a.W * a.csx * sizeof(float));
+    a.frame0 = 0;
+    a.frame_ho = a.Ho;
+    a.H *= n;
+    a.Ho *= n;
+    for (int ky = 0; ky < 3; ++ky)
+      for (int kx = 0; kx < 3; ++kx) a.tapoff4[ky * 3 + kx] = (ky * HWp + kx) * ROW4;
+    a.tiles_x = (a.Wo + s->TW - 1) / s->TW;
+    a.tiles_y = (a.Ho + s->TH - 1) / s->TH;
+    t.symbol = s->symbol;
+    t.mfma_flops = 2.0 * tiles * (s->WM * s->MB * 32.0) * (s->WN * s->NB * 32.0) * ((double)a.nchunk * s->KC * 9 + (a.k8_h + a.k8_x) * 8.0);
+    diag_stamp(c, op, a, tiles);
+    s->launch(a, dim3(tiles), sb.st);
+    return;
+  }
   diag_stamp(c, op, a, a.tiles_x * a.tiles_y * sb.n);
   g_bkinds[op.bkind].launch(a, dim3(a.tiles_x * a.tiles_y * sb.n), sb.st);
 }
@@ -2299,10 +2371,57 @@
   g_fkinds[op.fkind].launch(a, dim3(g, op.grid_y), sb.st);
 }
 
+static const StackedConvInfo* stacked_conv_kind(Kind kd, int Ho, int Wo, int n, int* tiles) {
+  const KindInfo& k0 = g_kinds[kd];
+  for (const StackedConvInfo& s : g_stacked_convs) {
+    if (s.KC != k0.KC || s.WN * s.NB != k0.WN * k0.NB || s.S != k0.S || s.EXT != k0.EXT) continue;
+    const long rows_now = (long)n * ((Ho + k0.TH - 1) / k0.TH) * ((Wo + k0.TW - 1) / k0.TW) * (k0.WM * k0.MB * 32);
+    *tiles = stacked_tiles(Ho, Wo, n, s.TH, s.TW, s.WM * s.MB * 32, rows_now);
+    if (*tiles) return &s;
+  }
+  return nullptr;
+}
+static const StackedConvInfo* stacked_conv(const fpc_ctx* c, const Op& op, int n, int* tiles) {
+  const ConvArgs& a = op.args;
+  if (!c->opt.tiles_round6 || c->vgg || op.plain_conv || !conv2_takes(c, op)) return nullptr;
+  if (a.pad != 0 || a.Ho != a.H || a.Wo != a.W) return nullptr;
+  const unsigned long long in_b = (unsigned long long)n * a.H * a.W * a.cs0 * sizeof(float);
+  const unsigned long long out_b = (unsigned long long)n * a.OH * a.OW * std::max(a.cso, a.res ? a.csr : 0) * sizeof(float);
+  if (std::max(in_b, out_b) >= (unsigned long long)CONV2_MARKER) return nullptr;
+  return stacked_conv_kind(op.kind, a.Ho, a.Wo, n, tiles);
+}
+
 static void launch_conv(fpc_ctx* c, const Op& op, int i, const Sub& sb) {
   LaunchTimer t(c, i, sb.st, sb.n);
   ConvArgs a = op.args;
   a.frame0 = sb.f0;
+  int tiles = 0;
+  if (const StackedConvInfo* s = stacked_conv(c, op, sb.n, &tiles)) {
+    const KindInfo& k0 = g_kinds[op.kind];
+    const int n = sb.n, HWp = (s->TW - 1) * s->S + s->EXT, HWp0 = (k0.TW - 1) * k0.S + k0.EXT, ROW4 = s->KC / 4 + 1;
+    a.in0 += (size_t)sb.f0 * a.H * a.W * a.cs0;
+    a.out += (size_t)sb.f0 * a.OH * a.OW * a.cso;
+    if (a.res) a.res += (size_t)sb.f0 * a.OH * a.OW * a.csr;
+    a.frame0 = 0;
+    a.frame_h = a.H;
+    a.H *= n;
+    a.Ho *= n;
+    a.OH *= n;
+    double taps = 0;
+    for (int z = 0; z < op.grid_z; ++z) {
+      taps += a.sub[z].ntaps;
+      for (int tp = 0; tp < a.sub[z].ntaps; ++tp) {
+        const int lin = a.sub[z].tapoff4[tp] / ROW4, dy = lin / HWp0, dx = lin - dy * HWp0;
+        a.sub[z].tapoff4[tp] = (dy * HWp + dx) * ROW4;
+      }
+    }
+    a.tiles_x = (a.Wo + s->TW - 1) / s->TW;
+    a.tiles_y = (a.Ho + s->TH - 1) / s->TH;
+    t.symbol = s->symbol;
+    t.mfma_flops = 2.0 * taps * tiles * (s->WM * s->MB * 32.0) * ((double)a.nchunk0 * s->KC) * (a.nbt * 32.0);
+    s->launch(a, dim3(tiles, op.grid_y, op.grid_z), sb.st);
+    return;
+  }
   const dim3 grid(a.tiles_x * a.tiles_y * sb.n, op.grid_y, op.grid_z);
   if (op.lean) lean_kind(op.kind)->launch(a, grid, sb.st);
   else g_kinds[op.kind].launch(a, grid, sb.st);
@@ -2559,6 +2678,8 @@
   if (int rc = allow_dynamic_lds(g_lean_kinds)) return rc;
   if (int rc = allow_dynamic_lds(g_wkinds)) return rc;
   if (int rc = allow_dynamic_lds(g_bkinds)) return rc;
+  if (int rc = allow_dynamic_lds(g_stacked_convs)) return rc;
+  if (int rc = allow_dynamic_lds(g_stacked_blocks)) return rc;
   if (int rc = allow_dynamic_lds(g_fkinds)) return rc;
   static_assert(FK_COUNT <= 64, "fpc_ctx::fkind_blocks_per_cu");
   for (int k = 0; k < FK_COUNT; ++k) {
@@ -2817,6 +2938,9 @@
       const BKindInfo& k = g_bkinds[r6 && block_rows(k6, H, W) < block_rows(k5, H, W) ? k6 : k5];
       return 100 * k.TH + k.TW;
     }
+    case 4: { int t = 0; return r6 && stacked_block_kind(BK_B310_s2_K32_C256, H, W, frames, &t) ? t : 0; }
+    case 5: { int t = 0; return r6 && stacked_conv_kind(K_T320_2x2_K64_N128, H, W, frames, &t) ? t : 0; }
+    case 6: { int t = 0; return r6 && stacked_conv_kind(K_T320_1x1_K64_N128, H, W, frames, &t) ? t : 0; }
   }
   return FPC_E_INVALID;
 }
@@ -4415,7 +4539,7 @@
           case OP_POOL2: k = "maxpool2_kernel"; break;
           case OP_L2NORM: k = "l2norm256_kernel"; break;
         }
-      kernels[i] = k;
+      kernels[i] = t.symbol ? t.symbol : k;
     }
     if (ms) ms[i] = v;
     if (flops) flops[i] = op ? op->flops_per_frame * t.frames : 0.0;
```
